# zerohd4869/MM-DFN

Hardware: AMD Instinct MI355X
Metric: utterances/sec (fwd+bwd), IEMOCAP-shaped batch (higher is better)
Workload: dtype f32; 1 GPU; cfg2 (BASELINE configs[1]): B=16 dialogues/GPU, L=110, dims 100/100/512, 2 GCN layers, P=2, dropout 0.50; utterances_per_gpu=1760, parallelism=dp1

## Files before the change

### include/mmdfn_hip.h

```cpp
#ifndef MMDFN_HIP_H
#define MMDFN_HIP_H

#include <stdint.h>

#ifdef __cplusplus
extern "C" {
#endif

int64_t mmdfn_riders_bytes(void);

int mmdfn_abi_version(void);

int mmdfn_propagate(const float* tiles, const float* cross, const float* H, float* out,
                    const int32_t* dia_len, const int32_t* row_start, const int64_t* tile_base,
                    int B, int M, int N, int d, int ldh, int ldo, int max_len, int transpose,
                    void* stream);

int mmdfn_tile_outer(const float* X, const float* Y, float* dtiles, float* dcross,
                     const int32_t* dia_len, const int32_t* row_start, const int64_t* tile_base,
                     int B, int M, int N, int d, int ldx, int ldy, int max_len, int accumulate,
                     void* stream);

int mmdfn_adj_build(const float* feats, float* unit, float* norm, float* cosg, float* cdot,
                    float* rdeg, float* tiles, float* cross,
                    const int32_t* dia_len, const int32_t* row_start, const int64_t* tile_base,
                    int B, int M, int N, int D, int max_len, float modal_weight, void* stream);

int mmdfn_adj_build_bwd(const float* dtiles, const float* dcross,
                        const float* unit, const float* norm, const float* cosg, const float* cdot,
                        const float* rdeg, const float* tiles, const float* cross,
                        float* wsym, float* etile, float* ecross, float* ddeg, float* dunit,
                        float* dfeats, const float* addend,
                        const int32_t* dia_len, const int32_t* row_start, const int64_t* tile_base,
                        int B, int M, int N, int D, int max_len, float modal_weight, void* stream);

int mmdfn_gru_seq_fwd(int ngroups, const float* const* gi, const float* const* w_hh,
                      const float* const* b_hh, float* const* y, float* const* gates,
                      const int* rows, const int* T, int H, void* riders, void* stream);

int mmdfn_gru_seq_bwd(int ngroups, const float* const* dy, const float* const* y,
                      const float* const* gates, const float* const* w_hh,
                      float* const* dgi, float* const* dgh,
                      const int* rows, const int* T, int H, void* riders, void* stream);

int mmdfn_gru_seq_fwd_seg(int ngroups, const float* const* gi, const float* const* w_hh,
                          const float* const* b_hh, float* const* y, float* const* gates,
                          const int* rows, const int* T, int H, const int32_t* const* rank, const int* P,
                          const int* BP, const int* tdir, const float* const* ytab, void* stream);
int mmdfn_gru_seq_bwd_seg(int ngroups, const float* const* dy, const float* const* y,
                          const float* const* gates, const float* const* w_hh,
                          float* const* dgi, float* const* dgh, const int* rows, const int* T, int H,
                          const int32_t* const* rank, const int* P, const int* BP, const int* tdir,
                          float* const* dhinit, int32_t* const* kout, void* stream);
int mmdfn_gru_tab_reduce(const float* dy, const int32_t* kout, const float* dhinit, float* dyt, int rows, int T,
                         int H, int dir, void* stream);

int mmdfn_lstm_pointwise_fwd(const float* G, const float* c_prev, float* h_out, float* c_out,
                             int64_t R, int H, void* stream);
int mmdfn_lstm_pointwise_bwd(const float* G, const float* c_prev, const float* c_new,
                             const float* dh, const float* dc_next, float* dG, float* dc_prev,
                             int64_t R, int H, void* stream);

int mmdfn_gcnii_combine_fwd(const float* P, const float* S2, const float* q, const float* mask,
                            float* out, float theta, float alpha, int64_t R, int d, void* stream);
int mmdfn_gcnii_combine_bwd(const float* P, const float* S2, const float* mask, const float* dout,
                            float* dP, float* dS2, float theta, float alpha, int64_t R, int d,
                            void* stream);

int mmdfn_party_gather(int Mn, const float* const* X, const float* qmask, const float* bias, float* S,
                       int32_t* rank, int L, int B, int P, int H, void* stream);
int mmdfn_party_gather_bwd(int Mn, const float* dS, const int32_t* rank, float* const* dX,
                           const float* const* addend, int L, int B, int P, int H, void* stream);
int mmdfn_party_gather_bwd_colsum(int Mn, const float* dS, const int32_t* rank, float* const* dX,
                                  const float* const* addend, int L, int B, int P, int H, float* workspace, void* stream);

int mmdfn_keep_flags(float* out, int64_t n, float keep, void* state, void* stream);
int mmdfn_keep_flags_stage(float* out, int64_t n, float keep, void* state, void* riders, void* stream);
int mmdfn_keep_flags_flush(void* riders, void* stream);
int mmdfn_gru_seq_fwd_takes_flags(int ngroups, const int* rows);
int64_t mmdfn_colsum_workspace(int H);
int mmdfn_colsum(const float* A, int64_t R, int H, int lda, float* out, float* workspace, void* stream);
int mmdfn_colsum_partial(const float* A, int64_t R, int H, int lda, float* workspace, void* stream);
int mmdfn_party_combine(int Mn, const float* const* base, const float* E, const int32_t* rank,
                        const int64_t* flat_idx, float* out, const float* weights,
                        int L, int B, int P, int N, int H, void* stream);
int mmdfn_party_combine_bwd(int Mn, const float* dout, const int32_t* rank, const int64_t* flat_idx,
                            float* const* dbase, float* dE, const float* weights,
                            int L, int B, int P, int N, int H, void* stream);
int mmdfn_party_combine_bwd_dst(int Mn, const float* dout, const int32_t* rank, const int64_t* inv, float* const* dbase,
                                float* dE, const float* weights, int L, int B, int P, int N, int H, void* stream);


int mmdfn_mask_scale(int ngroups, const float* const* x, const float* const* mask, float* const* out,
                     const int64_t* n, float scale, void* stream);

int mmdfn_linear(const float* X, const float* W, const float* bias, float* Y, int R, int K, int N,
                 int ldx, int ldy, int act, int accumulate, void* stream);
int mmdfn_linear2(const float* X, const float* W, const float* W2, int N1, const float* bias, const float* bias2,
                  float* Y, int R, int K, int N, int ldx, int ldy, int act, int accumulate, void* stream);

int64_t mmdfn_weight_planes_workspace(int N, int K);
int mmdfn_cut_weight_planes(int n, const float* const* w1, const float* const* w2, const int* n1, const int* ld,
                            const int* N, const int* K, const int* mode, void* const* planes, void* stream);
int mmdfn_linear_planes(const float* X, const void* planes, const float* bias, const float* bias2, int n1, float* Y, int R,
                        int K, int N, int ldx, int ldy, int act, int accumulate, void* stream);
int mmdfn_linear_planes_group(int n, const float* const* X, const void* const* planes, const float* const* bias,
                              const float* const* bias2, const int* n1, float* const* Y, const int* R, const int* K,
                              const int* N, const int* ldx, const int* ldy, int act, int accumulate,
                              const float* const* mask, float mask_scale, void* stream);
int mmdfn_linear_planes_group_in(int n, const float* const* X, const void* const* planes, const float* const* bias,
                                 const float* const* bias2, const int* n1, float* const* Y, const int* R, const int* K,
                                 const int* N, const int* ldx, const int* ldy, int act, int accumulate,
                                 const float* const* mask, float mask_scale, const float* const* xmask,
                                 float* const* xdrop, float xscale, void* stream);
int mmdfn_linear_planes_group_party(int n, const float* const* X, const void* const* planes, const float* const* bias,
                                    const float* const* bias2, const int* n1, float* const* Y, const int* R, const int* K,
                                    const int* N, const int* ldx, const int* ldy, int act, int accumulate,
                                    const float* const* mask, float mask_scale, const float* const* xmask,
                                    float* const* xdrop, float xscale, const int* party, const float* qmask, float* S,
                                    int32_t* rank, int L, int B, int P, int Mn, void* stream);

int mmdfn_linear_group_supported(int R, int K, int N);
int mmdfn_linear_group(int n, const float* const* X, const float* const* W, const float* const* W2, const int* N1,
                       const float* const* bias, const float* const* bias2, float* const* Y, const int* R,
                       const int* K, const int* N, const int* ldx, const int* ldw, const int* ldy,
                       const int* kmajor, const int* accumulate, int act, void* stream);
int mmdfn_linear_group_addend(int n, const float* const* X, const float* const* W, const float* const* W2, const int* N1,
                              const float* const* bias, const float* const* bias2, float* const* Y, const float* const* Z,
                              const int* ldz, const int* R, const int* K, const int* N, const int* ldx, const int* ldw,
                              const int* ldy, const int* kmajor, const int* accumulate, int act, void* stream);
int mmdfn_linear_group_seg2(int n, const float* const* X, const float* const* W, const float* const* W2, const int* N1,
                            const float* const* bias, const float* const* bias2, float* const* Y, const float* const* Z,
                            const int* ldz, const int* R, const int* K, const int* N, const int* ldx, const int* ldw,
                            const int* ldy, const int* kmajor, const int* accumulate, const float* const* X2,
                            const float* const* Wk2, const int* K2, const int* ldx2, const int* ldw2, int act, void* stream);

int mmdfn_softmax_scale_fwd(const float* z, const float* c, float* att, float* out, int R, int W, void* stream);
int mmdfn_softmax_scale_bwd(const float* att, const float* c, const float* dout, float* dz, float* dc, int R, int W,
                            void* stream);
int mmdfn_mfn_mem_fwd(const float* u, const float* v1, const float* v2, const float* mem, float* out, float* saved,
                      int64_t n, void* stream);
int mmdfn_mfn_mem_bwd(const float* saved, const float* mem, const float* dout, float* du, float* dv1, float* dv2,
                      float* dmem, int64_t n, void* stream);
int mmdfn_gated_pair_fwd(const float* xm, const float* xn, const float* w, const float* b, const float* pm,
                         const float* pn, float* out, float* zs, int R, int D, int C, void* stream);
int mmdfn_gated_pair_bwd(const float* xm, const float* xn, const float* w, const float* pm, const float* pn,
                         const float* zs, const float* dout, float* dxm, float* dxn, float* dpm, float* dpn,
                         float* dpre, int R, int D, int C, void* stream);
int mmdfn_rowscale_colsum(const float* s, const float* xm, const float* xn, float* out, int R, int D, void* stream);

int mmdfn_gemm_tn_splits(int R, int M, int N);
int mmdfn_gemm_tn(const float* A, const float* B, float* C, float* colsum, float* workspace,
                  int R, int M, int N, int lda, int ldb, int ldc, int splits, void* stream);

int64_t mmdfn_gemm_tn_grouped_workspace(int n, const int* R, const int* M, const int* N);
int mmdfn_gemm_tn_grouped(int n, const float* const* A, const float* const* B, float* const* C, float* const* colsum,
                          const int* R, const int* M, const int* N, const int* lda, const int* ldb, const int* ldc,
                          const int* bshift, float* workspace, void* stream);

int mmdfn_gcn_input_fwd(const float* x, const float* mx, const float* W0, const float* b0, const float* m0, float* xd,
                        float* h0, float* cur0, int R, int F, int H, int ldxd, float mscale, void* stream);
int mmdfn_gcn_input_bwd(const float* dcur0, const float* m0, const float* dh0, const float* h0, const float* W0,
                        const float* dxd, const float* mx, float* dpre, float* dx, int R, int F, int H, int lddxd,
                        float mscale, void* stream);
int mmdfn_lstm_gate_fwd(const float* q, const float* h, const float* c, const float* Wih, const float* Whh,
                        const float* bsum, const float* bsum2, float* gates, float* h_out, float* c_out, int R, int H,
                        void* stream);
int mmdfn_lstm_gate_fwd_ld(const float* q, const float* h, const float* c, const float* Wih, const float* Whh,
                           const float* bsum, const float* bsum2, float* gates, float* h_out, float* c_out, int R, int H,
                           int ldh, void* stream);
int64_t mmdfn_lstm_gate_planes_workspace(int H);
int mmdfn_lstm_gate_cut_weights(const float* Wih, const float* Whh, float* planes, int H, void* stream);
int mmdfn_lstm_gate_takes_planes(int R, int H);
int mmdfn_lstm_gate_fwd_pre(const float* q, const float* h, const float* c, const float* Wih, const float* Whh,
                            const float* bsum, const float* bsum2, float* gates, float* h_out, float* c_out, int R, int H,
                            int ldh, const float* planes, void* stream);
int mmdfn_lstm_gate_bwd(const float* gates, const float* c_prev, const float* c_new, const float* dh_a, const float* dh_b,
                        const float* dc_next, const float* Wih, const float* Whh, const float* dres, float* dG,
                        float* dc_prev, float* dq, float* dh_prev, int R, int H, int has_h, int lddres, void* stream);
int mmdfn_gcnii_layer_fwd(const float* hi, const float* h0, const float* W, const float* q, const float* m, float* out,
                          float* gmask, float theta, float alpha, int R, int H, int ldo, float mscale, void* stream);

int mmdfn_prop_layer_fwd(const float* tiles, const float* cross, const float* zin, int ldz, const int32_t* dia_len,
                         const int32_t* row_start, const int64_t* tile_base, int B, int M, int N, int max_len,
                         const float* h0, const float* W, const float* q, const float* m, float* hi, float* out,
                         float* gmask, float theta, float alpha, int H, int ldo, float mscale, void* stream);
int mmdfn_gcnii_layer_bwd(const float* dout, const float* gmask, const float* W, float* dP, float* dhi, float* dh0,
                          float theta, float alpha, int R, int H, int lddo, int acc_h0, void* stream);
int mmdfn_gcnii_layer_bwd_ld(const float* dout, const float* gmask, const float* W, float* dP, float* dhi, float* dh0,
                             float theta, float alpha, int R, int H, int lddo, int acc_h0, int lddhi, void* stream);

int64_t mmdfn_gemm_tn_batch_workspace(int nseg, const int* R, const int* out, int nout, const int* M, const int* N);
int mmdfn_gemm_tn_batch(int nseg, const float* const* A, const float* const* B, const int* R, const int* lda,
                        const int* ldb, const int* bshift, const int* out, int nout, float* const* C,
                        float* const* colsum, float* const* colsum2, const int* M, const int* N, const int* ldc,
                        const int* accumulate, float* workspace, void* riders, void* stream);
int mmdfn_gemm_tn_batch_ext(int nseg, const float* const* A, const float* const* B, const int* R, const int* lda,
                            const int* ldb, const int* bshift, const int* out, int nout, float* const* C,
                            float* const* colsum, float* const* colsum2, const int* M, const int* N, const int* ldc,
                            const int* accumulate, float* workspace, int next, const float* const* ext_part,
                            const float* const* ext_colpart, float* const* ext_C, float* const* ext_colsum, const int* ext_M,
                            const int* ext_N, const int* ext_ldc, const int* ext_splits, const int* ext_accumulate,
                            void* riders, void* stream);

int mmdfn_wgrad_riders_stage(int nseg, const float* const* A, const float* const* B, const int* R, const int* lda,
                             const int* ldb, const int* bshift, const int* out, int nout, float* const* C,
                             float* const* colsum, float* const* colsum2, const int* M, const int* N, const int* ldc,
                             const int* accumulate, float* workspace, void* riders, void* stream);
int mmdfn_wgrad_riders_staged(void* riders);
int mmdfn_gru_seq_bwd_idle_cus(int ngroups, const int* rows);
int mmdfn_gru_seq_bwd_step_ns(int ngroups, const int* rows);
int mmdfn_wgrad_riders_flush(void* riders, void* stream);
int mmdfn_wgrad_riders_drain(void* riders, void* stream, int discard);

int mmdfn_adam_step(float* p, const float* g, float* m, float* v, int64_t n, float lr, float beta1,
                    float beta2, float eps, float weight_decay, int step, void* stream);

int mmdfn_head_fwd(const float* F, const float* mask, const float* W, const float* bias, float* logp, int64_t N, int Wd,
                   int C, int ldf, int split, float mscale, void* stream);
int64_t mmdfn_head_bwd_workspace(int Wd, int C);
int mmdfn_head_bwd(const float* dlogp, const float* logp, const float* F, const float* mask, const float* W, float* dF,
                   float* dW, float* db, float* workspace, int64_t N, int Wd, int C, int ldf, int lddf, int split,
                   float mscale, void* stream);
int mmdfn_head_bwd_groups(void);
int mmdfn_head_bwd_partial(const float* dlogp, const float* logp, const float* F, const float* mask, const float* W, float* dF,
                           float* workspace, int64_t N, int Wd, int C, int ldf, int lddf, int split, float mscale,
                           void* stream);
int mmdfn_head_fwd_act(const float* F, const float* mask, const float* W, const float* bias, float* logp, int64_t N, int Wd,
                       int C, int ldf, int split, float mscale, int relu, void* stream);
int mmdfn_head_bwd_act(const float* dlogp, const float* logp, const float* F, const float* mask, const float* W, float* dF,
                       float* dW, float* db, float* workspace, int64_t N, int Wd, int C, int ldf, int lddf, int split,
                       float mscale, int relu, void* stream);
int mmdfn_head_bwd_partial_act(const float* dlogp, const float* logp, const float* F, const float* mask, const float* W,
                               float* dF, float* workspace, int64_t N, int Wd, int C, int ldf, int lddf, int split, float mscale,
                               int relu, void* stream);

int mmdfn_lmf_bwd_width(int O, int R);
int mmdfn_lmf_fwd(float* P, const float* factor_a, const float* factor_v, const float* factor_t, int64_t rank_stride_a,
                  int64_t rank_stride_v, int64_t rank_stride_t, const float* w, const float* bias, float* out, int64_t N, int O,
                  int R, int ldp, int ldo, void* stream);
int mmdfn_lmf_bwd(const float* g, const float* P, const float* w, float* D, int64_t N, int O, int R, int ldg, int ldp, int ldd,
                  void* stream);

int64_t mmdfn_tfn_workspace(int64_t N, int Ha, int Hv, int Ht, int O, int which);
int mmdfn_tfn_fwd(const float* ha, const float* hv, const float* ht, int ldha, int ldhv, int ldht, const float* W1, int64_t ldw,
                  const float* b1, void* state, void* used, int64_t counters, float keep, float scale, float* out,
                  float* workspace, int64_t N, int Ha, int Hv, int Ht, int O, int relu, void* stream);
int mmdfn_tfn_bwd_input(const float* dy, const float* y1, int relu, const float* W1, int64_t ldw, const float* ha,
                        const float* hv, const float* ht, int ldha, int ldhv, int ldht, void* used, float keep, float scale,
                        float* dpre, float* dha, float* dhv, float* dht, float* workspace, int64_t N, int Ha, int Hv, int Ht,
                        int O, void* stream);
int mmdfn_tfn_bwd_weight(const float* dpre, const float* ha, const float* hv, const float* ht, int ldha, int ldhv, int ldht,
                         void* used, float keep, float scale, float* dW1, int64_t N, int Ha, int Hv, int Ht, int O,
                         void* stream);
int mmdfn_tfn_keep_flags(void* used, float keep, float* out, int64_t N, int64_t K, int64_t row0, int64_t rows, void* stream);

int mmdfn_focal_loss_fwd(const float* logp, const int64_t* target, const float* alpha, float* loss, float* coef,
                         int64_t N, int C, float gamma, int size_average, void* stream);
int mmdfn_focal_loss_fwd_grad(const float* logp, const int64_t* target, const float* alpha, float* loss, float* coef,
                              float* dlogp_unit, int64_t N, int C, float gamma, int size_average, void* stream);
int mmdfn_focal_loss_bwd(const float* coef, const int64_t* target, const float* dloss, float* dlogp, int64_t N, int C,
                         void* stream);
int mmdfn_focal_loss_fwd_ignore(const float* logp, const int64_t* target, const float* alpha, float* loss, float* coef,
                                float* scale_out, int64_t N, int C, float gamma, int size_average, int64_t ignore_index,
                                void* stream);
int mmdfn_focal_loss_bwd_ignore(const float* coef, const int64_t* target, const float* dloss, const float* scale,
                                float* dlogp, int64_t N, int C, int64_t ignore_index, void* stream);

#ifdef __cplusplus
}
#endif
#endif
```

### mm_dfn_amd/_hip.py

```python
import ctypes
import os

import torch

from . import build as _build

_P = ctypes.c_void_p
_I = ctypes.c_int
_F = ctypes.c_float
_L = ctypes.c_int64

SIGNATURES = {
    "mmdfn_abi_version": [],
    "mmdfn_propagate": [_P, _P, _P, _P, _P, _P, _P, _I, _I, _I, _I, _I, _I, _I, _I, _P],
    "mmdfn_tile_outer": [_P, _P, _P, _P, _P, _P, _P, _I, _I, _I, _I, _I, _I, _I, _I, _P],
    "mmdfn_adj_build": [_P] * 8 + [_P, _P, _P] + [_I] * 5 + [_F, _P],
    "mmdfn_adj_build_bwd": [_P] * 16 + [_P, _P, _P] + [_I] * 5 + [_F, _P],
    "mmdfn_riders_bytes": [],
    "mmdfn_gru_seq_fwd": [_I, _P, _P, _P, _P, _P, _P, _P, _I, _P, _P],
    "mmdfn_gru_seq_bwd": [_I, _P, _P, _P, _P, _P, _P, _P, _P, _I, _P, _P],
    "mmdfn_gru_seq_fwd_seg": [_I, _P, _P, _P, _P, _P, _P, _P, _I, _P, _P, _P, _P, _P, _P],
    "mmdfn_gru_seq_bwd_seg": [_I, _P, _P, _P, _P, _P, _P, _P, _P, _I, _P, _P, _P, _P, _P, _P, _P],
    "mmdfn_gru_tab_reduce": [_P, _P, _P, _P, _I, _I, _I, _I, _P],
    "mmdfn_lstm_pointwise_fwd": [_P, _P, _P, _P, _L, _I, _P],
    "mmdfn_lstm_pointwise_bwd": [_P, _P, _P, _P, _P, _P, _P, _L, _I, _P],
    "mmdfn_gcnii_combine_fwd": [_P, _P, _P, _P, _P, _F, _F, _L, _I, _P],
    "mmdfn_gcnii_combine_bwd": [_P, _P, _P, _P, _P, _P, _F, _F, _L, _I, _P],
    "mmdfn_gcn_input_fwd": [_P] * 8 + [_I] * 4 + [_F, _P],
    "mmdfn_gcn_input_bwd": [_P] * 9 + [_I] * 4 + [_F, _P],
    "mmdfn_lstm_gate_fwd": [_P] * 10 + [_I] * 2 + [_P],
    "mmdfn_lstm_gate_fwd_ld": [_P] * 10 + [_I] * 3 + [_P],
    "mmdfn_lstm_gate_fwd_pre": [_P] * 10 + [_I] * 3 + [_P, _P],
    "mmdfn_lstm_gate_planes_workspace": [_I],
    "mmdfn_lstm_gate_cut_weights": [_P, _P, _P, _I, _P],
    "mmdfn_lstm_gate_takes_planes": [_I, _I],
    "mmdfn_lstm_gate_bwd": [_P] * 13 + [_I] * 4 + [_P],
    "mmdfn_gcnii_layer_fwd": [_P] * 7 + [_F, _F, _I, _I, _I, _F, _P],
    "mmdfn_prop_layer_fwd": [_P, _P, _P, _I, _P, _P, _P, _I, _I, _I, _I, _P, _P, _P, _P, _P, _P, _P, _F, _F, _I, _I, _F, _P],
    "mmdfn_gcnii_layer_bwd": [_P] * 6 + [_F, _F, _I, _I, _I, _I, _P],
    "mmdfn_gcnii_layer_bwd_ld": [_P] * 6 + [_F, _F, _I, _I, _I, _I, _I, _P],
    "mmdfn_linear": [_P, _P, _P, _P, _I, _I, _I, _I, _I, _I, _I, _P],
    "mmdfn_linear2": [_P, _P, _P, _I, _P, _P, _P, _I, _I, _I, _I, _I, _I, _I, _P],
    "mmdfn_weight_planes_workspace": [_I, _I],
    "mmdfn_cut_weight_planes": [_I, _P, _P, _P, _P, _P, _P, _P, _P, _P],
    "mmdfn_linear_planes": [_P, _P, _P, _P, _I, _P, _I, _I, _I, _I, _I, _I, _I, _P],
    "mmdfn_linear_planes_group": [_I, _P, _P, _P, _P, _P, _P, _P, _P, _P, _P, _P, _I, _I, _P, _F, _P],
    "mmdfn_linear_planes_group_in": [_I, _P, _P, _P, _P, _P, _P, _P, _P, _P, _P, _P, _I, _I, _P, _F, _P, _P, _F, _P],
    "mmdfn_linear_planes_group_party": [_I, _P, _P, _P, _P, _P, _P, _P, _P, _P, _P, _P, _I, _I, _P, _F, _P, _P, _F,
                                        _P, _P, _P, _P, _I, _I, _I, _I, _P],
    "mmdfn_linear_group_supported": [_I, _I, _I],
    "mmdfn_linear_group": [_I] + [_P] * 15 + [_I, _P],
    "mmdfn_linear_group_addend": [_I] + [_P] * 17 + [_I, _P],
    "mmdfn_linear_group_seg2": [_I] + [_P] * 22 + [_I, _P],
    "mmdfn_softmax_scale_fwd": [_P, _P, _P, _P, _I, _I, _P],
    "mmdfn_softmax_scale_bwd": [_P, _P, _P, _P, _P, _I, _I, _P],
    "mmdfn_mfn_mem_fwd": [_P] * 6 + [_L, _P],
    "mmdfn_mfn_mem_bwd": [_P] * 7 + [_L, _P],
    "mmdfn_gated_pair_fwd": [_P] * 8 + [_I, _I, _I, _P],
    "mmdfn_gated_pair_bwd": [_P] * 12 + [_I, _I, _I, _P],
    "mmdfn_rowscale_colsum": [_P, _P, _P, _P, _I, _I, _P],
    "mmdfn_gemm_tn_splits": [_I, _I, _I],
    "mmdfn_gemm_tn": [_P, _P, _P, _P, _P, _I, _I, _I, _I, _I, _I, _I, _P],
    "mmdfn_gemm_tn_grouped_workspace": [_I, _P, _P, _P],
    "mmdfn_gemm_tn_grouped": [_I, _P, _P, _P, _P, _P, _P, _P, _P, _P, _P, _P, _P, _P],
    "mmdfn_gemm_tn_batch_workspace": [_I, _P, _P, _I, _P, _P],
    "mmdfn_gemm_tn_batch": [_I, _P, _P, _P, _P, _P, _P, _P, _I, _P, _P, _P, _P, _P, _P, _P, _P, _P, _P],
    "mmdfn_wgrad_riders_stage": [_I, _P, _P, _P, _P, _P, _P, _P, _I, _P, _P, _P, _P, _P, _P, _P, _P, _P, _P],
    "mmdfn_wgrad_riders_staged": [_P],
    "mmdfn_wgrad_riders_flush": [_P, _P],
    "mmdfn_wgrad_riders_drain": [_P, _P, _I],
    "mmdfn_gru_seq_bwd_idle_cus": [_I, _P],
    "mmdfn_gru_seq_bwd_step_ns": [_I, _P],
    "mmdfn_gemm_tn_batch_ext": [_I, _P, _P, _P, _P, _P, _P, _P, _I, _P, _P, _P, _P, _P, _P, _P, _P,
                                _I, _P, _P, _P, _P, _P, _P, _P, _P, _P, _P, _P],
    "mmdfn_head_bwd_groups": [],
    "mmdfn_head_bwd_partial": [_P, _P, _P, _P, _P, _P, _P, _L, _I, _I, _I, _I, _I, _F, _P],
    "mmdfn_colsum_partial": [_P, _L, _I, _I, _P, _P],
    "mmdfn_head_fwd": [_P, _P, _P, _P, _P, _L, _I, _I, _I, _I, _F, _P],
    "mmdfn_head_bwd_workspace": [_I, _I],
    "mmdfn_head_bwd": [_P] * 9 + [_L, _I, _I, _I, _I, _I, _F, _P],
    "mmdfn_head_fwd_act": [_P, _P, _P, _P, _P, _L, _I, _I, _I, _I, _F, _I, _P],
    "mmdfn_head_bwd_act": [_P] * 9 + [_L, _I, _I, _I, _I, _I, _F, _I, _P],
    "mmdfn_head_bwd_partial_act": [_P, _P, _P, _P, _P, _P, _P, _L, _I, _I, _I, _I, _I, _F, _I, _P],
    "mmdfn_lmf_bwd_width": [_I, _I],
    "mmdfn_lmf_fwd": [_P, _P, _P, _P, _L, _L, _L, _P, _P, _P, _L, _I, _I, _I, _I, _P],
    "mmdfn_lmf_bwd": [_P, _P, _P, _P, _L, _I, _I, _I, _I, _I, _P],
    "mmdfn_tfn_workspace": [_L, _I, _I, _I, _I, _I],
    "mmdfn_tfn_fwd": [_P, _P, _P, _I, _I, _I, _P, _L, _P, _P, _P, _L, _F, _F, _P, _P, _L, _I, _I, _I, _I, _I, _P],
    "mmdfn_tfn_bwd_input": [_P, _P, _I, _P, _L, _P, _P, _P, _I, _I, _I, _P, _F, _F, _P, _P, _P, _P, _P, _L, _I, _I, _I, _I, _P],
    "mmdfn_tfn_bwd_weight": [_P, _P, _P, _P, _I, _I, _I, _P, _F, _F, _P, _L, _I, _I, _I, _I, _P],
    "mmdfn_tfn_keep_flags": [_P, _F, _P, _L, _L, _L, _L, _P],
    "mmdfn_focal_loss_fwd": [_P, _P, _P, _P, _P, _L, _I, _F, _I, _P],
    "mmdfn_focal_loss_bwd": [_P, _P, _P, _P, _L, _I, _P],
    "mmdfn_focal_loss_fwd_grad": [_P, _P, _P, _P, _P, _P, _L, _I, _F, _I, _P],
    "mmdfn_focal_loss_fwd_ignore": [_P, _P, _P, _P, _P, _P, _L, _I, _F, _I, _L, _P],
    "mmdfn_focal_loss_bwd_ignore": [_P, _P, _P, _P, _P, _L, _I, _L, _P],
    "mmdfn_adam_step": [_P, _P, _P, _P, _L, _F, _F, _F, _F, _F, _I, _P],
    "mmdfn_party_gather": [_I, _P, _P, _P, _P, _P, _I, _I, _I, _I, _P],
    "mmdfn_party_gather_bwd": [_I, _P, _P, _P, _P, _I, _I, _I, _I, _P],
    "mmdfn_party_gather_bwd_colsum": [_I, _P, _P, _P, _P, _I, _I, _I, _I, _P, _P],
    "mmdfn_party_combine": [_I, _P, _P, _P, _P, _P, _P, _I, _I, _I, _I, _I, _P],
    "mmdfn_party_combine_bwd": [_I, _P, _P, _P, _P, _P, _P, _I, _I, _I, _I, _I, _P],
    "mmdfn_party_combine_bwd_dst": [_I, _P, _P, _P, _P, _P, _P, _I, _I, _I, _I, _I, _P],
    "mmdfn_mask_scale": [_I, _P, _P, _P, _P, _F, _P],
    "mmdfn_keep_flags": [_P, _L, _F, _P, _P],
    "mmdfn_keep_flags_stage": [_P, _L, _F, _P, _P, _P],
    "mmdfn_keep_flags_flush": [_P, _P],
    "mmdfn_gru_seq_fwd_takes_flags": [_I, _P],
    "mmdfn_colsum_workspace": [_I],
    "mmdfn_colsum": [_P, _L, _I, _I, _P, _P, _P],
}

ABI_VERSION = 21


class HipLibraryError(RuntimeError):
    pass


_libs = {}
_tuning = os.environ.get("MMDFN_TUNING_LIB", "0") == "1"


def set_tuning(flag):
    global _tuning
    prev, _tuning = _tuning, bool(flag)
    return prev


def lib():
    handle = _libs.get(_tuning)
    if handle is not None:
        return handle
    tuning = _tuning
    path = _build.TUNING_LIBPATH if tuning else _build.LIBPATH
    if _build.is_stale(tuning):
        try:
            _build.build(verbose=False, tuning=tuning)
        except Exception as e:
            raise HipLibraryError(
                "%s is missing or stale (source digest mismatch) and could not be rebuilt (%s): run `python -m "
                "mm_dfn_amd.build` (needs hipcc); the MI355X path has no CPU fallback" % (path, e)) from e
    handle = ctypes.CDLL(path)
    for name, argtypes in SIGNATURES.items():
        try:
            fn = getattr(handle, name)
        except AttributeError as e:
            raise HipLibraryError("%s lacks symbol %s (stale build?)" % (os.path.basename(path), name)) from e
        fn.argtypes = argtypes
        fn.restype = ctypes.c_int64 if name.endswith(("_workspace", "_bytes")) else ctypes.c_int
    if handle.mmdfn_abi_version() != ABI_VERSION:
        raise HipLibraryError("%s ABI version mismatch" % os.path.basename(path))
    _libs[tuning] = handle
    return handle


def riders_context():
    return ctypes.create_string_buffer(int(lib().mmdfn_riders_bytes()))


def ptr(t):
    if t is None:
        return None
    return ctypes.c_void_p(t.data_ptr())


def stream():
    return ctypes.c_void_p(torch.cuda.current_stream().cuda_stream)


def check(rc, what):
    if rc != 0:
        raise HipLibraryError("%s failed with code %d" % (what, rc))


def require_cuda(*tensors):
    for t in tensors:
        if t is not None and not t.is_cuda:
            raise HipLibraryError("the MM-DFN HIP path needs tensors on an MI355X device (got %s); "
                                  "there is no CPU fallback" % t.device)


def ptr_array(tensors):
    return (ctypes.c_void_p * len(tensors))(*[None if t is None else t.data_ptr() for t in tensors])


def int_array(values):
    return (ctypes.c_int * len(values))(*[int(v) for v in values])


def long_array(values):
    return (ctypes.c_int64 * len(values))(*[int(v) for v in values])


def float_array(values):
    return (ctypes.c_float * len(values))(*[float(v) for v in values])


def require_f32(*tensors):
    for t in tensors:
        if t is not None and t.dtype != torch.float32:
            raise HipLibraryError("the MM-DFN HIP kernels are fp32 (got %s)" % t.dtype)
```

### mm_dfn_amd/csrc/gcn_small.hip

```cpp
#include "mmdfn_internal.h"
#include "../../include/mmdfn_hip.h"
#include <stdlib.h>

namespace {

constexpr int GS_SR = 32;
constexpr int GS_NW = 8;
constexpr int GS_MAXL = 128;
constexpr int GS_SA = 132;

#ifdef MMDFN_TUNING
#define GS_STOP(K) do { if (stop == (K)) return; } while (0)
#else
#define GS_STOP(K) do { } while (0)
#endif

__global__ __launch_bounds__(64 * GS_NW) void prop_layer_strip_fwd_kernel(
    const float* __restrict__ tiles, const float* __restrict__ cross, const float* __restrict__ zin, int ldz,
    const int32_t* __restrict__ dia_len, const int32_t* __restrict__ row_start, const int64_t* __restrict__ tile_base,
    int B, int M, int N, int NS, const float* __restrict__ h0, const float* __restrict__ W, const float* __restrict__ q,
    const float* __restrict__ mk, float* __restrict__ hi_out, float* __restrict__ out, float* __restrict__ gmask,
    float theta, float alpha, int H, int ldo, float ms, int S2, int stop) {
    extern __shared__ __attribute__((aligned(16))) float smem[];
    const int bid = blockIdx.x;
    const int yq = bid >> 3;
    const int per = M * NS;
    const int i = (yq / per) * 8 + (bid & 7);
    if (i >= B) return;
    const int rem = yq % per;
    const int m = rem / NS;
    const int st = rem - m * NS;
    const int L = dia_len[i];
    const int r0 = st * GS_SR;
    if (r0 >= L) return;
    GS_STOP(9);
    const int ld = (L + 3) & ~3;
    const int Lp = (L + 15) & ~15;
    const int nt = Lp >> 4;
    const int rs = row_start[i];
    const int64_t toff = tile_base[i] + (int64_t)m * L * ld;
    const int K2 = 2 * H;
    const int nkc2 = (K2 + 15) >> 4;
    const int nct = (H + 15) >> 4;

    float* As = smem;
    float* A2 = As + GS_SR * GS_SA;
    float* cw = A2 + GS_SR * S2;

    const int tid = threadIdx.x;
    const int lane = tid & 63;
    const int w = __builtin_amdgcn_readfirstlane(tid >> 6);
    const int fi = lane & 15, g = lane >> 4;
    const bool tile = w < nct;
    const int col = 16 * w + fi;
    const unsigned colc = col < H ? col : H - 1;

    int o0 = -1, o1 = -1;
    for (int n = 0; n < M; ++n)
        if (n != m) { if (o0 < 0) o0 = n; else o1 = n; }

    const int c4 = lane & 31, sub = lane >> 5;
    float4 ar[2];
#pragma unroll
    for (int it = 0; it < 2; ++it) {
        const int p = r0 + 16 * it + 2 * w + sub;
        const int qc = 4 * c4 < ld ? 4 * c4 : ld - 4;
        ar[it] = *reinterpret_cast<const float4*>(tiles + toff + (unsigned)((p < L ? p : L - 1) * ld + qc));
    }
    const int H4 = H >> 2;
    float4 hr[2];
#pragma unroll
    for (int s2 = 0; s2 < 2; ++s2) {
        const int e = tid + 64 * GS_NW * s2;
        const int r = e / H4, k = (e - r * H4) * 4;
        const int p = r0 + r;
        hr[s2] = make_float4(0.f, 0.f, 0.f, 0.f);
        if (r < GS_SR && p < L) hr[s2] = *reinterpret_cast<const float4*>(h0 + ((int64_t)m * N + rs + p) * H + k);
    }
    float cwv = 0.f;
    if (tid < 2 * GS_SR) {
        const int n = tid >> 5, pl = tid & 31;
        const int o = n == 0 ? o0 : o1;
        const int p = r0 + pl;
        if (o >= 0 && p < L) {
            const int pk = (m < o) ? mmdfn_pair_index(m, o, M) : mmdfn_pair_index(o, m, M);
            cwv = cross[(int64_t)pk * N + rs + p];
        }
    }
    float zo0[2][4], zo1[2][4], qv[2][4], mv[2][4];
    const bool whole = r0 + GS_SR <= L;
    const int64_t row0 = (int64_t)m * N + rs + r0;
    const unsigned lane_z = (unsigned)(4 * g) * (unsigned)ldz + colc, lane_h = (unsigned)(4 * g) * (unsigned)H + colc;
#pragma unroll
    for (int a = 0; a < 2; ++a)
#pragma unroll
        for (int r = 0; r < 4; ++r) {
            zo0[a][r] = zo1[a][r] = qv[a][r] = 0.f;
            mv[a][r] = 1.0f;
        }
    if (tile) {
        const float* z0 = zin + ((int64_t)(o0 >= 0 ? o0 : m) * N + rs + r0) * ldz;
        const float* z1 = zin + ((int64_t)(o1 >= 0 ? o1 : m) * N + rs + r0) * ldz;
        const float* qb = (q ? q : h0) + row0 * H;
        const float* mb = (mk ? mk : h0) + row0 * H;
        if (whole) {
#pragma unroll
            for (int a = 0; a < 2; ++a)
#pragma unroll
                for (int r = 0; r < 4; ++r) {
                    const int rr = 16 * a + r;
                    zo0[a][r] = (z0 + (size_t)rr * ldz)[lane_z];
                    zo1[a][r] = (z1 + (size_t)rr * ldz)[lane_z];
                    qv[a][r] = (qb + (size_t)rr * H)[lane_h];
                    mv[a][r] = (mb + (size_t)rr * H)[lane_h];
                }
        } else {
#pragma unroll
            for (int a = 0; a < 2; ++a)
#pragma unroll
                for (int r = 0; r < 4; ++r) {
                    const int pl = 16 * a + 4 * g + r;
                    const unsigned pc = r0 + pl < L ? pl : L - 1 - r0;
                    zo0[a][r] = z0[pc * (unsigned)ldz + colc];
                    zo1[a][r] = z1[pc * (unsigned)ldz + colc];
                    qv[a][r] = qb[pc * (unsigned)H + colc];
                    mv[a][r] = mb[pc * (unsigned)H + colc];
                }
        }
#pragma unroll
        for (int a = 0; a < 2; ++a)
#pragma unroll
            for (int r = 0; r < 4; ++r) {
                if (!q) qv[a][r] = 0.f;
                mv[a][r] = mk ? mv[a][r] * ms : 1.0f;
            }
    }

    float zfr[32], wfr[64];
#pragma unroll
    for (int kk = 0; kk < 32; ++kk) zfr[kk] = 0.f;
#pragma unroll
    for (int kk = 0; kk < 64; ++kk) wfr[kk] = 0.f;
    if (tile) {
        const float* zm = zin + ((int64_t)m * N + rs) * ldz;
        const int zfull = L >> 4;
#pragma unroll
        for (int kc = 0; kc < 8; ++kc) {
            if (kc < zfull) {
#pragma unroll
                for (int j = 0; j < 4; ++j) zfr[4 * kc + j] = (zm + (size_t)(16 * kc + j) * ldz)[lane_z];
            } else if (kc < nt) {
#pragma unroll
                for (int j = 0; j < 4; ++j) {
                    const int qq = 16 * kc + 4 * g + j;
                    zfr[4 * kc + j] = zm[(unsigned)(qq < L ? qq : L - 1) * (unsigned)ldz + colc];
                }
            }
        }
        const int wfull = K2 >> 4;
#pragma unroll
        for (int kc = 0; kc < 16; ++kc) {
            if (kc < wfull) {
#pragma unroll
                for (int j = 0; j < 4; ++j) wfr[4 * kc + j] = (W + (size_t)(16 * kc + j) * H)[lane_h];
            } else if (kc < nkc2) {
#pragma unroll
                for (int j = 0; j < 4; ++j) {
                    const int k = 16 * kc + 4 * g + j;
                    wfr[4 * kc + j] = W[(unsigned)(k < K2 ? k : K2 - 1) * (unsigned)H + colc];
                }
            }
        }
    }
#pragma unroll
    for (int it = 0; it < 2; ++it) {
        const int pl = 16 * it + 2 * w + sub;
        const int p = r0 + pl;
        const int qq = 4 * c4;
        float4 v = ar[it];
        const bool rowin = p < L;
        v.x = (rowin && qq + 0 < L) ? v.x : 0.f;
        v.y = (rowin && qq + 1 < L) ? v.y : 0.f;
        v.z = (rowin && qq + 2 < L) ? v.z : 0.f;
        v.w = (rowin && qq + 3 < L) ? v.w : 0.f;
        *reinterpret_cast<float4*>(As + pl * GS_SA + qq) = v;
    }
#pragma unroll
    for (int s2 = 0; s2 < 2; ++s2) {
        const int e = tid + 64 * GS_NW * s2;
        const int r = e / H4, k = (e - r * H4) * 4;
        if (r < GS_SR) *reinterpret_cast<float4*>(A2 + r * S2 + H + k) = hr[s2];
    }
    for (int e = tid; e < GS_SR * (S2 - K2); e += 64 * GS_NW) {
        const int r = e / (S2 - K2), k = K2 + (e - r * (S2 - K2));
        A2[r * S2 + k] = 0.f;
    }
    if (tid < 2 * GS_SR) cw[tid] = cwv;
    __syncthreads();
    GS_STOP(1);

    float hv[2][4];
    if (tile) {
#pragma unroll
        for (int a = 0; a < 2; ++a) {
            const float* ea = As + (16 * a + fi) * GS_SA + 4 * g;
            float4 av[8];
#pragma unroll
            for (int kc = 0; kc < 8; ++kc) av[kc] = *reinterpret_cast<const float4*>(ea + 16 * kc);
            f32x4 acc = (f32x4){0.f, 0.f, 0.f, 0.f};
#pragma unroll
            for (int kc = 0; kc < 8; ++kc) {
                if (kc >= nt) continue;
                acc = __builtin_amdgcn_mfma_f32_16x16x4f32(av[kc].x, zfr[4 * kc + 0], acc, 0, 0, 0);
                acc = __builtin_amdgcn_mfma_f32_16x16x4f32(av[kc].y, zfr[4 * kc + 1], acc, 0, 0, 0);
                acc = __builtin_amdgcn_mfma_f32_16x16x4f32(av[kc].z, zfr[4 * kc + 2], acc, 0, 0, 0);
                acc = __builtin_amdgcn_mfma_f32_16x16x4f32(av[kc].w, zfr[4 * kc + 3], acc, 0, 0, 0);
            }
            float* hb = hi_out + (row0 + 16 * a) * H;
#pragma unroll
            for (int r = 0; r < 4; ++r) {
                const int pl = 16 * a + 4 * g + r;
                float v = acc[r];
                if (o0 >= 0) v += cw[pl] * zo0[a][r];
                if (o1 >= 0) v += cw[GS_SR + pl] * zo1[a][r];
                hv[a][r] = v;
                if (col < H) {
                    A2[pl * S2 + col] = v;
                    if (r0 + pl < L) (hb + (size_t)r * H)[lane_h] = v;
                }
            }
        }
    }
    __syncthreads();
    GS_STOP(2);

    if (tile) {
        f32x4 acc0 = (f32x4){0.f, 0.f, 0.f, 0.f}, acc1 = acc0;
        const float* e0 = A2 + fi * S2 + 4 * g;
        const float* e1 = A2 + (16 + fi) * S2 + 4 * g;
#pragma unroll
        for (int kc = 0; kc < 16; ++kc) {
            if (kc >= nkc2) continue;
            const float4 a0 = *reinterpret_cast<const float4*>(e0 + 16 * kc);
            const float4 a1 = *reinterpret_cast<const float4*>(e1 + 16 * kc);
            acc0 = __builtin_amdgcn_mfma_f32_16x16x4f32(a0.x, wfr[4 * kc + 0], acc0, 0, 0, 0);
            acc1 = __builtin_amdgcn_mfma_f32_16x16x4f32(a1.x, wfr[4 * kc + 0], acc1, 0, 0, 0);
            acc0 = __builtin_amdgcn_mfma_f32_16x16x4f32(a0.y, wfr[4 * kc + 1], acc0, 0, 0, 0);
            acc1 = __builtin_amdgcn_mfma_f32_16x16x4f32(a1.y, wfr[4 * kc + 1], acc1, 0, 0, 0);
            acc0 = __builtin_amdgcn_mfma_f32_16x16x4f32(a0.z, wfr[4 * kc + 2], acc0, 0, 0, 0);
            acc1 = __builtin_amdgcn_mfma_f32_16x16x4f32(a1.z, wfr[4 * kc + 2], acc1, 0, 0, 0);
            acc0 = __builtin_amdgcn_mfma_f32_16x16x4f32(a0.w, wfr[4 * kc + 3], acc0, 0, 0, 0);
            acc1 = __builtin_amdgcn_mfma_f32_16x16x4f32(a1.w, wfr[4 * kc + 3], acc1, 0, 0, 0);
        }
        if (col < H) {
            const unsigned lane_o = (unsigned)(4 * g) * (unsigned)ldo + col;
#pragma unroll
            for (int a = 0; a < 2; ++a)
#pragma unroll
                for (int r = 0; r < 4; ++r) {
                    const int pl = 16 * a + 4 * g + r;
                    if (r0 + pl >= L) continue;
                    const float pv = a == 0 ? acc0[r] : acc1[r];
                    const float v0 = A2[pl * S2 + H + col];
                    const float pre = theta * pv + (1.0f - theta) * ((1.0f - alpha) * hv[a][r] + alpha * v0);
                    (out + (row0 + 16 * a + r) * ldo)[lane_o] = fmaxf(pre, 0.f) * mv[a][r] + qv[a][r];
                    (gmask + (row0 + 16 * a + r) * H)[lane_h] = pre > 0.f ? mv[a][r] : 0.f;
                }
        }
    }
}

}

extern "C" int mmdfn_prop_layer_fwd(const float* tiles, const float* cross, const float* zin, int ldz, const int32_t* dia_len,
                                    const int32_t* row_start, const int64_t* tile_base, int B, int M, int N, int max_len,
                                    const float* h0, const float* W, const float* q, const float* m, float* hi, float* out,
                                    float* gmask, float theta, float alpha, int H, int ldo, float mscale, void* stream) {
    if (B <= 0 || M <= 0 || N <= 0 || H <= 0 || max_len <= 0 || !tiles || !zin || !h0 || !W || !hi || !out || !gmask) return -1;
    if (M > 3 || max_len > GS_MAXL || H > 100 || (H & 3) || ldz < H || ldo < H) return -2;
    if (M > 1 && !cross) return -1;
    int stop = 0;
#ifdef MMDFN_TUNING
    if (const char* e = getenv("MMDFN_PROP_LAYER")) if (atoi(e) == 0) return -2;
    if (const char* e = getenv("MMDFN_PROP_LAYER_STOP")) stop = atoi(e);
#endif
    const int NS = (max_len + GS_SR - 1) / GS_SR;
    const int64_t grid = (int64_t)((B + 7) / 8) * 8 * M * NS;
    if (grid > 4096) return -2;
    const int S2 = ((2 * H + 15) & ~15) + 4;
    const size_t lds = ((size_t)GS_SR * GS_SA + (size_t)GS_SR * S2 + 2 * GS_SR) * sizeof(float);
    hipLaunchKernelGGL(prop_layer_strip_fwd_kernel, dim3((unsigned)grid), dim3(64 * GS_NW), lds, (hipStream_t)stream, tiles, cross,
                       zin, ldz, dia_len, row_start, tile_base, B, M, N, NS, h0, W, q, m, hi, out, gmask, theta, alpha, H, ldo,
                       mscale, S2, stop);
    MMDFN_CHECK_LAUNCH();
    return 0;
}
```

### mm_dfn_amd/csrc/gcn_stack.hip

```cpp
#include "mmdfn_internal.h"
#include "../../include/mmdfn_hip.h"
#include <stdlib.h>

namespace {

constexpr int RB = 16;

__device__ __forceinline__ float4 ld4(const float* p) { return *reinterpret_cast<const float4*>(p); }
__device__ __forceinline__ void st4(float* p, float4 v) { *reinterpret_cast<float4*>(p) = v; }
__device__ __forceinline__ float4 zero4() { return make_float4(0.f, 0.f, 0.f, 0.f); }
__device__ __forceinline__ float4 one4() { return make_float4(1.f, 1.f, 1.f, 1.f); }
__device__ __forceinline__ float4 mul4(float4 a, float4 b) { return make_float4(a.x * b.x, a.y * b.y, a.z * b.z, a.w * b.w); }
__device__ __forceinline__ float4 scl4(float4 a, float s) { return make_float4(a.x * s, a.y * s, a.z * s, a.w * s); }
__device__ __forceinline__ float4 add4(float4 a, float4 b) { return make_float4(a.x + b.x, a.y + b.y, a.z + b.z, a.w + b.w); }
__device__ __forceinline__ float4 fma4(float4 a, float s, float4 b) { return make_float4(a.x * s + b.x, a.y * s + b.y, a.z * s + b.z, a.w * s + b.w); }
__device__ __forceinline__ float sigm(float x) { return __builtin_amdgcn_rcpf(1.0f + __expf(-x)); }
__device__ __forceinline__ float tanhf_(float x) { return 1.0f - 2.0f * __builtin_amdgcn_rcpf(1.0f + __expf(2.0f * x)); }

typedef float f32x2_t __attribute__((ext_vector_type(2)));
__device__ __forceinline__ void st4_nt(float* p, float4 v) { __builtin_nontemporal_store((f32x4){v.x, v.y, v.z, v.w}, reinterpret_cast<f32x4*>(p)); }
__device__ __forceinline__ void nt_store2(float* p, float2 v) { __builtin_nontemporal_store((f32x2_t){v.x, v.y}, reinterpret_cast<f32x2_t*>(p)); }
__device__ __forceinline__ int frag_row(int i) { return i < 4 ? 2 * i : (i < 12 ? 2 * (i - 4) + 1 : 2 * (i - 12) + 8); }
__device__ __forceinline__ int frag_unit(int g) { return ((g & 1) << 1) | (g >> 1); }

__host__ __device__ inline int lds_stride(int K) {
    int ld = ((K + 15) & ~15) + 4;
    if (((ld >> 2) & 1) == 0) ld += 4;
    return ld;
}

__device__ __forceinline__ int qdiv(int i, float inv) { return (int)(((float)i + 0.5f) * inv); }

__device__ __forceinline__ void zero_pads(float* base, int nrows, int ld, int K) {
    const int np4 = (ld - K) >> 2;
    const float rnp4 = 1.0f / (float)(np4 > 0 ? np4 : 1);
    for (int i = threadIdx.x; i < nrows * np4; i += 256) {
        const int r = qdiv(i, rnp4), j = i - r * np4;
        st4(base + r * ld + K + 4 * j, zero4());
    }
}

constexpr int NWS = 26;
template <bool KMAJOR>
struct WeightStager {
    float4 v[NWS];
    __device__ __forceinline__ void issue(const float* __restrict__ W, int ldsrc, int n0, int ncols, int K) {
        const int inner = KMAJOR ? (ncols >> 2) : (K >> 2);
        const int total = KMAJOR ? K * inner : ncols * inner;
        const int qa = 256 / inner, qb = 256 - qa * inner;
        int r = threadIdx.x / inner, j = threadIdx.x - r * inner;
#pragma unroll
        for (int e = 0; e < NWS; ++e) {
            const int i = threadIdx.x + 256 * e;
            const float* src = KMAJOR ? W + (int64_t)r * ldsrc + n0 + 4 * j : W + (int64_t)(n0 + r) * ldsrc + 4 * j;
            v[e] = (i < total) ? ld4(src) : zero4();
            r += qa;
            j += qb;
            if (j >= inner) { j -= inner; ++r; }
        }
    }
    __device__ __forceinline__ void commit(float* sW, int ldw, int ncols, int K) const {
        const int inner = KMAJOR ? (ncols >> 2) : (K >> 2);
        const int total = KMAJOR ? K * inner : ncols * inner;
        const int qa = 256 / inner, qb = 256 - qa * inner;
        int r = threadIdx.x / inner, j = threadIdx.x - r * inner;
#pragma unroll
        for (int e = 0; e < NWS; ++e) {
            const int i = threadIdx.x + 256 * e;
            if (i < total) {
                if (KMAJOR) {
                    float* d = sW + (4 * j) * ldw + r;
                    d[0] = v[e].x; d[ldw] = v[e].y; d[2 * ldw] = v[e].z; d[3 * ldw] = v[e].w;
                } else {
                    st4(sW + r * ldw + 4 * j, v[e]);
                }
            }
            r += qa;
            j += qb;
            if (j >= inner) { j -= inner; ++r; }
        }
        zero_pads(sW, ncols, ldw, K);
    }
};

template <int NT>
__device__ __forceinline__ void contract(f32x4 (&acc)[NT], const int (&wrow0)[NT], const float* sA, int lda, const float* sW,
                                         int ldw, int K) {
    const int lane = threadIdx.x & 63, fi = lane & 15, g = lane >> 4;
    const float* ap = sA + frag_row(fi) * lda + 4 * frag_unit(g);
    const float* bp[NT];
#pragma unroll
    for (int t = 0; t < NT; ++t) bp[t] = sW + (wrow0[t] + frag_row(fi)) * ldw + 4 * frag_unit(g);
    const int nk = (K + 15) >> 4;
    float4 a0, a1, b0[NT], b1[NT];
#define CT_LOAD(A_, B_, KC)                                                          \
    do {                                                                             \
        A_ = ld4(ap + 16 * (KC));                                                    \
        _Pragma("unroll") for (int t = 0; t < NT; ++t) B_[t] = ld4(bp[t] + 16 * (KC)); \
    } while (0)
#define CT_MMA(A_, B_)                                                                                         \
    do {                                                                                                       \
        const float av_[4] = {A_.x, A_.y, A_.z, A_.w};                                                         \
        _Pragma("unroll") for (int j = 0; j < 4; ++j)                                                          \
            _Pragma("unroll") for (int t = 0; t < NT; ++t) {                                                   \
                const float bv_ = (j == 0) ? B_[t].x : (j == 1) ? B_[t].y : (j == 2) ? B_[t].z : B_[t].w;     \
                acc[t] = __builtin_amdgcn_mfma_f32_16x16x4f32(av_[j], bv_, acc[t], 0, 0, 0);                   \
            }                                                                                                  \
    } while (0)
    CT_LOAD(a0, b0, 0);
    int kc = 0;
    for (; kc + 2 <= nk; kc += 2) {
        CT_LOAD(a1, b1, kc + 1);
        CT_MMA(a0, b0);
        if (kc + 2 < nk) CT_LOAD(a0, b0, kc + 2);
        CT_MMA(a1, b1);
    }
    if (kc < nk) CT_MMA(a0, b0);
#undef CT_LOAD
#undef CT_MMA
}

template <int NT>
__device__ __forceinline__ int wave_tiles(int (&wrow0)[NT], int ntiles) {
    const int w = threadIdx.x >> 6;
    int nt = 0;
#pragma unroll
    for (int t = 0; t < NT; ++t) {
        const int tile = w + 4 * t;
        wrow0[t] = tile < ntiles ? 16 * tile : 0;
        nt += tile < ntiles ? 1 : 0;
    }
    return nt;
}

template <int NT>
__device__ __forceinline__ void spill_tiles(const f32x4 (&acc)[NT], const int (&wrow0)[NT], int nt, float* sP, int ldp) {
    const int lane = threadIdx.x & 63, fi = lane & 15, g = lane >> 4;
#pragma unroll
    for (int t = 0; t < NT; ++t) {
        if (t < nt) {
#pragma unroll
            for (int r = 0; r < 4; ++r) sP[frag_row(4 * g + r) * ldp + wrow0[t] + frag_row(fi)] = acc[t][r];
        }
    }
}

#define FOR_ROW_BLOCKS(rb, nrb) for (int rb = blockIdx.x; rb < (nrb); rb += gridDim.x)

__global__ __launch_bounds__(256) void gcn_input_fwd_kernel(const float* __restrict__ x, const float* __restrict__ mx,
                                                            const float* __restrict__ W0, const float* __restrict__ b0,
                                                            const float* __restrict__ m0, float* __restrict__ xd,
                                                            float* __restrict__ h0, float* __restrict__ cur0, int R,
                                                            int F, int H, int ldxd, float ms) {
    extern __shared__ __attribute__((aligned(16))) float smem[];
    const int ldw = lds_stride(F), ldp = ((H + 15) & ~15) + 4;
    float* sW = smem;
    float* sA = sW + H * ldw;
    float* sP = sA + 2 * RB * ldw;
    WeightStager<false> wst;
    wst.issue(W0, F, 0, H, F);
    const int nrb = (R + RB - 1) / RB;
    const int F4 = F >> 2, H4 = H >> 2;
    const float rF4 = 1.0f / (float)F4, rH4 = 1.0f / (float)H4;
    int wrow0[2];
    const int nt = wave_tiles<2>(wrow0, (H + 15) >> 4);
    constexpr int NS = 4;
    constexpr int NE = 2;
    float4 rx[NS], rm[NS];
    auto issue = [&](int rb) {
#pragma unroll
        for (int s = 0; s < NS; ++s) {
            const int i = threadIdx.x + 256 * s;
            const int r = qdiv(i, rF4), k = (i - r * F4) * 4, row = rb * RB + r;
            const bool ok = i < RB * F4 && row < R;
            rx[s] = ok ? ld4(x + (int64_t)row * F + k) : zero4();
            rm[s] = (ok && mx) ? ld4(mx + (int64_t)row * F + k) : one4();
        }
    };
    auto park = [&](int rb, float* dst) {
#pragma unroll
        for (int s = 0; s < NS; ++s) {
            const int i = threadIdx.x + 256 * s;
            if (i >= RB * F4) continue;
            const int r = qdiv(i, rF4), k = (i - r * F4) * 4, row = rb * RB + r;
            const float4 v = mul4(rx[s], scl4(rm[s], mx ? ms : 1.0f));
            st4(dst + r * ldw + k, v);
            if (row < R) st4_nt(xd + (int64_t)row * ldxd + k, v);
        }
    };
    const int rb0 = blockIdx.x;
    if (rb0 < nrb) issue(rb0);
    wst.commit(sW, ldw, H, F);
    zero_pads(sA, 2 * RB, ldw, F);
    if (rb0 < nrb) park(rb0, sA);
    __syncthreads();
    int buf = 0;
    FOR_ROW_BLOCKS(rb, nrb) {
        const int nxt = rb + gridDim.x;
        if (nxt < nrb) issue(nxt);
        float4 em[NE], eb[NE];
#pragma unroll
        for (int s = 0; s < NE; ++s) {
            const int i = threadIdx.x + 256 * s;
            const int r = qdiv(i, rH4), n = (i - r * H4) * 4, row = rb * RB + r;
            const bool ok = i < RB * H4 && row < R;
            em[s] = (ok && m0) ? ld4(m0 + (int64_t)row * H + n) : one4();
            eb[s] = (ok && b0) ? ld4(b0 + n) : zero4();
        }
        f32x4 acc[2] = {{0.f, 0.f, 0.f, 0.f}, {0.f, 0.f, 0.f, 0.f}};
        contract<2>(acc, wrow0, sA + buf * RB * ldw, ldw, sW, ldw, F);
        spill_tiles<2>(acc, wrow0, nt, sP, ldp);
        __syncthreads();
#pragma unroll
        for (int s = 0; s < NE; ++s) {
            const int i = threadIdx.x + 256 * s;
            const int r = qdiv(i, rH4), n = (i - r * H4) * 4, row = rb * RB + r;
            if (i >= RB * H4 || row >= R) continue;
            float4 v = add4(ld4(sP + r * ldp + n), eb[s]);
            v.x = fmaxf(v.x, 0.f); v.y = fmaxf(v.y, 0.f); v.z = fmaxf(v.z, 0.f); v.w = fmaxf(v.w, 0.f);
            st4(h0 + (int64_t)row * H + n, v);
            st4(cur0 + (int64_t)row * H + n, mul4(v, scl4(em[s], m0 ? ms : 1.0f)));
        }
        if (nxt < nrb) park(nxt, sA + (buf ^ 1) * RB * ldw);
        __syncthreads();
        buf ^= 1;
    }
}

__global__ __launch_bounds__(256) void gcn_input_bwd_kernel(const float* __restrict__ dcur0, const float* __restrict__ m0,
                                                            const float* __restrict__ dh0, const float* __restrict__ h0,
                                                            const float* __restrict__ W0, const float* __restrict__ dxd,
                                                            const float* __restrict__ mx, float* __restrict__ dpre,
                                                            float* __restrict__ dx, int R, int F, int H, int lddxd, float ms) {
    extern __shared__ __attribute__((aligned(16))) float smem[];
    const int ldw = lds_stride(H), ldp = ((F + 15) & ~15) + 4;
    float* sW = smem;
    float* sA = sW + F * ldw;
    float* sP = sA + 2 * RB * ldw;
    WeightStager<true> wst;
    wst.issue(W0, F, 0, F, H);
    const int nrb = (R + RB - 1) / RB;
    const int H4 = H >> 2, F4 = F >> 2;
    const float rF4 = 1.0f / (float)F4, rH4 = 1.0f / (float)H4;
    int wrow0[4];
    const int nt = wave_tiles<4>(wrow0, (F + 15) >> 4);
    constexpr int NS = 2;
    constexpr int NE = 4;
    float4 rd[NS], rmk[NS], rh0[NS], rdh[NS];
    auto issue = [&](int rb) {
#pragma unroll
        for (int s = 0; s < NS; ++s) {
            const int i = threadIdx.x + 256 * s;
            const int r = qdiv(i, rH4), k = (i - r * H4) * 4, row = rb * RB + r;
            const bool ok = i < RB * H4 && row < R;
            const int64_t o = (int64_t)row * H + k;
            rd[s] = (ok && dcur0) ? ld4(dcur0 + o) : zero4();
            rmk[s] = (ok && m0) ? ld4(m0 + o) : one4();
            rdh[s] = (ok && dh0) ? ld4(dh0 + o) : zero4();
            rh0[s] = ok ? ld4(h0 + o) : zero4();
        }
    };
    auto park = [&](int rb, float* dst) {
#pragma unroll
        for (int s = 0; s < NS; ++s) {
            const int i = threadIdx.x + 256 * s;
            if (i >= RB * H4) continue;
            const int r = qdiv(i, rH4), k = (i - r * H4) * 4, row = rb * RB + r;
            float4 v = add4(mul4(rd[s], scl4(rmk[s], m0 ? ms : 1.0f)), rdh[s]);
            v.x = rh0[s].x > 0.f ? v.x : 0.f; v.y = rh0[s].y > 0.f ? v.y : 0.f;
            v.z = rh0[s].z > 0.f ? v.z : 0.f; v.w = rh0[s].w > 0.f ? v.w : 0.f;
            st4(dst + r * ldw + k, v);
            if (row < R) st4_nt(dpre + (int64_t)row * H + k, v);
        }
    };
    if ((int)blockIdx.x < nrb) issue(blockIdx.x);
    wst.commit(sW, ldw, F, H);
    zero_pads(sA, 2 * RB, ldw, H);
    if ((int)blockIdx.x < nrb) park(blockIdx.x, sA);
    __syncthreads();
    int buf = 0;
    FOR_ROW_BLOCKS(rb, nrb) {
        const int nxt = rb + gridDim.x;
        if (nxt < nrb) issue(nxt);
        float4 ed[NE], em[NE];
#pragma unroll
        for (int s = 0; s < NE; ++s) {
            const int i = threadIdx.x + 256 * s;
            const int r = qdiv(i, rF4), n = (i - r * F4) * 4, row = rb * RB + r;
            const bool ok = i < RB * F4 && row < R;
            ed[s] = (ok && dxd) ? ld4(dxd + (int64_t)row * lddxd + n) : zero4();
            em[s] = (ok && mx) ? ld4(mx + (int64_t)row * F + n) : one4();
        }
        f32x4 acc[4];
#pragma unroll
        for (int t = 0; t < 4; ++t) acc[t] = (f32x4){0.f, 0.f, 0.f, 0.f};
        contract<4>(acc, wrow0, sA + buf * RB * ldw, ldw, sW, ldw, H);
        spill_tiles<4>(acc, wrow0, nt, sP, ldp);
        __syncthreads();
#pragma unroll
        for (int s = 0; s < NE; ++s) {
            const int i = threadIdx.x + 256 * s;
            const int r = qdiv(i, rF4), n = (i - r * F4) * 4, row = rb * RB + r;
            if (i >= RB * F4 || row >= R) continue;
            st4(dx + (int64_t)row * F + n, mul4(add4(ld4(sP + r * ldp + n), ed[s]), scl4(em[s], mx ? ms : 1.0f)));
        }
        if (nxt < nrb) park(nxt, sA + (buf ^ 1) * RB * ldw);
        __syncthreads();
        buf ^= 1;
    }
}

__global__ __launch_bounds__(256) void gcnii_layer_fwd_kernel(const float* __restrict__ hi, const float* __restrict__ h0,
                                                              const float* __restrict__ W, const float* __restrict__ q,
                                                              const float* __restrict__ m, float* __restrict__ out,
                                                              float* __restrict__ gmask, float theta, float alpha, int R,
                                                              int H, int ldo, float ms) {
    extern __shared__ __attribute__((aligned(16))) float smem[];
    const int K = 2 * H;
    const int ldw = lds_stride(K), ldp = ((H + 15) & ~15) + 4;
    float* sW = smem;
    float* sA = sW + H * ldw;
    float* sP = sA + 2 * RB * ldw;
    WeightStager<true> wst;
    wst.issue(W, H, 0, H, K);
    const int nrb = (R + RB - 1) / RB;
    const int H4 = H >> 2;
    const float rH4 = 1.0f / (float)H4;
    int wrow0[2];
    const int nt = wave_tiles<2>(wrow0, (H + 15) >> 4);
    constexpr int NS = 2;
    float4 ra[NS], rb_[NS];
    auto issue = [&](int rb) {
#pragma unroll
        for (int s = 0; s < NS; ++s) {
            const int i = threadIdx.x + 256 * s;
            const int r = qdiv(i, rH4), k = (i - r * H4) * 4, row = rb * RB + r;
            const bool ok = i < RB * H4 && row < R;
            ra[s] = ok ? ld4(hi + (int64_t)row * H + k) : zero4();
            rb_[s] = ok ? ld4(h0 + (int64_t)row * H + k) : zero4();
        }
    };
    auto park = [&](float* dst) {
#pragma unroll
        for (int s = 0; s < NS; ++s) {
            const int i = threadIdx.x + 256 * s;
            if (i >= RB * H4) continue;
            const int r = qdiv(i, rH4), k = (i - r * H4) * 4;
            st4(dst + r * ldw + k, ra[s]);
            st4(dst + r * ldw + H + k, rb_[s]);
        }
    };
    if ((int)blockIdx.x < nrb) issue(blockIdx.x);
    wst.commit(sW, ldw, H, K);
    zero_pads(sA, 2 * RB, ldw, K);
    if ((int)blockIdx.x < nrb) park(sA);
    __syncthreads();
    int buf = 0;
    FOR_ROW_BLOCKS(rb, nrb) {
        const int nxt = rb + gridDim.x;
        if (nxt < nrb) issue(nxt);
        const float* A = sA + buf * RB * ldw;
        float4 eq[NS], em[NS];
#pragma unroll
        for (int s = 0; s < NS; ++s) {
            const int i = threadIdx.x + 256 * s;
            const int r = qdiv(i, rH4), n = (i - r * H4) * 4, row = rb * RB + r;
            const bool ok = i < RB * H4 && row < R;
            eq[s] = (ok && q) ? ld4(q + (int64_t)row * H + n) : zero4();
            em[s] = (ok && m) ? ld4(m + (int64_t)row * H + n) : one4();
        }
        f32x4 acc[2] = {{0.f, 0.f, 0.f, 0.f}, {0.f, 0.f, 0.f, 0.f}};
        contract<2>(acc, wrow0, A, ldw, sW, ldw, K);
        spill_tiles<2>(acc, wrow0, nt, sP, ldp);
        __syncthreads();
#pragma unroll
        for (int s = 0; s < NS; ++s) {
            const int i = threadIdx.x + 256 * s;
            const int r = qdiv(i, rH4), n = (i - r * H4) * 4, row = rb * RB + r;
            if (i >= RB * H4 || row >= R) continue;
            const float4 p = ld4(sP + r * ldp + n), vh = ld4(A + r * ldw + n), v0 = ld4(A + r * ldw + H + n);
            const float4 ems = scl4(em[s], m ? ms : 1.0f);
            float4 o, gm;
#define K7F(F_)                                                                                            \
    {                                                                                                      \
        const float pre = theta * p.F_ + (1.0f - theta) * ((1.0f - alpha) * vh.F_ + alpha * v0.F_);       \
        o.F_ = fmaxf(pre, 0.f) * ems.F_ + eq[s].F_;                                                        \
        gm.F_ = pre > 0.f ? ems.F_ : 0.f;                                                                  \
    }
            K7F(x) K7F(y) K7F(z) K7F(w)
#undef K7F
            st4(out + (int64_t)row * ldo + n, o);
            st4_nt(gmask + (int64_t)row * H + n, gm);
        }
        if (nxt < nrb) park(sA + (buf ^ 1) * RB * ldw);
        __syncthreads();
        buf ^= 1;
    }
}

__global__ __launch_bounds__(256) void gcnii_layer_bwd_kernel(const float* __restrict__ dout, const float* __restrict__ gmask,
                                                              const float* __restrict__ W, float* __restrict__ dP,
                                                              float* __restrict__ dhi, float* __restrict__ dh0,
                                                              float theta, float alpha, int R, int H, int lddo, int acc_h0, int lddhi) {
    extern __shared__ __attribute__((aligned(16))) float smem[];
    const int N = 2 * H;
    const int ldw = lds_stride(H), ldp = ((N + 15) & ~15) + 4;
    float* sW = smem;
    float* sA = sW + N * ldw;
    float* sP = sA + 2 * RB * ldw;
    WeightStager<false> wst;
    wst.issue(W, H, 0, N, H);
    const int nrb = (R + RB - 1) / RB;
    const int H4 = H >> 2;
    const float rH4 = 1.0f / (float)H4;
    int wrow0[4];
    const int nt = wave_tiles<4>(wrow0, (N + 15) >> 4);
    constexpr int NS = 2;
    float4 rd[NS], rg[NS];
    auto issue = [&](int rb) {
#pragma unroll
        for (int s = 0; s < NS; ++s) {
            const int i = threadIdx.x + 256 * s;
            const int r = qdiv(i, rH4), k = (i - r * H4) * 4, row = rb * RB + r;
            const bool ok = i < RB * H4 && row < R;
            rd[s] = ok ? ld4(dout + (int64_t)row * lddo + k) : zero4();
            rg[s] = ok ? ld4(gmask + (int64_t)row * H + k) : zero4();
        }
    };
    auto park = [&](int rb, float* dst) {
#pragma unroll
        for (int s = 0; s < NS; ++s) {
            const int i = threadIdx.x + 256 * s;
            if (i >= RB * H4) continue;
            const int r = qdiv(i, rH4), k = (i - r * H4) * 4, row = rb * RB + r;
            const float4 v = scl4(mul4(rd[s], rg[s]), theta);
            st4(dst + r * ldw + k, v);
            if (row < R) st4_nt(dP + (int64_t)row * H + k, v);
        }
    };
    if ((int)blockIdx.x < nrb) issue(blockIdx.x);
    wst.commit(sW, ldw, N, H);
    zero_pads(sA, 2 * RB, ldw, H);
    if ((int)blockIdx.x < nrb) park(blockIdx.x, sA);
    __syncthreads();
    const float c1 = (1.0f - theta) * (1.0f - alpha) / theta, c2 = (1.0f - theta) * alpha / theta;
    int buf = 0;
    FOR_ROW_BLOCKS(rb, nrb) {
        const int nxt = rb + gridDim.x;
        if (nxt < nrb) issue(nxt);
        const float* A = sA + buf * RB * ldw;
        float4 eo[NS];
#pragma unroll
        for (int s = 0; s < NS; ++s) {
            const int i = threadIdx.x + 256 * s;
            const int r = qdiv(i, rH4), n = (i - r * H4) * 4, row = rb * RB + r;
            eo[s] = (acc_h0 && i < RB * H4 && row < R) ? ld4(dh0 + (int64_t)row * H + n) : zero4();
        }
        f32x4 acc[4];
#pragma unroll
        for (int t = 0; t < 4; ++t) acc[t] = (f32x4){0.f, 0.f, 0.f, 0.f};
        contract<4>(acc, wrow0, A, ldw, sW, ldw, H);
        spill_tiles<4>(acc, wrow0, nt, sP, ldp);
        __syncthreads();
#pragma unroll
        for (int s = 0; s < NS; ++s) {
            const int i = threadIdx.x + 256 * s;
            const int r = qdiv(i, rH4), n = (i - r * H4) * 4, row = rb * RB + r;
            if (i >= RB * H4 || row >= R) continue;
            const float4 dp = ld4(A + r * ldw + n);
            st4(dhi + (int64_t)row * lddhi + n, fma4(dp, c1, ld4(sP + r * ldp + n)));
            st4(dh0 + (int64_t)row * H + n, add4(fma4(dp, c2, ld4(sP + r * ldp + H + n)), eo[s]));
        }
        if (nxt < nrb) park(nxt, sA + (buf ^ 1) * RB * ldw);
        __syncthreads();
        buf ^= 1;
    }
}

__global__ __launch_bounds__(512) void gcnii_layer_fwd_ws_kernel(const float* __restrict__ hi, const float* __restrict__ h0,
                                                                 const float* __restrict__ W, const float* __restrict__ q,
                                                                 const float* __restrict__ m, float* __restrict__ out,
                                                                 float* __restrict__ gmask, float theta, float alpha, int R,
                                                                 int H, int ldo, float ms) {
    extern __shared__ __attribute__((aligned(16))) float smem[];
    const int K = 2 * H;
    const int ldw = lds_stride(K), ldp = ((H + 15) & ~15) + 4;
    float* sW = smem;
    float* sA = sW + H * ldw;
    float* sP = sA + 2 * RB * ldw;
    const int nrb = (R + RB - 1) / RB;
    const int H4 = H >> 2;
    const float rH4 = 1.0f / (float)H4;
    const int tid = threadIdx.x & 255;
    const bool producer = threadIdx.x >= 256;
    const int first = blockIdx.x, stride = gridDim.x;
    constexpr int NS = 2;
    float4 ra[NS], rb_[NS], eq[NS], em[NS];
    auto issue = [&](int rb) {
#pragma unroll
        for (int s = 0; s < NS; ++s) {
            const int i = tid + 256 * s;
            const int r = qdiv(i, rH4), k = (i - r * H4) * 4, row = rb * RB + r;
            const bool ok = i < RB * H4 && row < R;
            ra[s] = ok ? ld4(hi + (int64_t)row * H + k) : zero4();
            rb_[s] = ok ? ld4(h0 + (int64_t)row * H + k) : zero4();
        }
    };
    auto park = [&](float* dst) {
#pragma unroll
        for (int s = 0; s < NS; ++s) {
            const int i = tid + 256 * s;
            if (i >= RB * H4) continue;
            const int r = qdiv(i, rH4), k = (i - r * H4) * 4;
            st4(dst + r * ldw + k, ra[s]);
            st4(dst + r * ldw + H + k, rb_[s]);
        }
    };
    auto issue_epi = [&](int rb) {
#pragma unroll
        for (int s = 0; s < NS; ++s) {
            const int i = tid + 256 * s;
            const int r = qdiv(i, rH4), n = (i - r * H4) * 4, row = rb * RB + r;
            const bool ok = i < RB * H4 && row < R;
            eq[s] = (ok && q) ? ld4(q + (int64_t)row * H + n) : zero4();
            em[s] = (ok && m) ? ld4(m + (int64_t)row * H + n) : one4();
        }
    };
    auto epilogue = [&](int rb, const float* A, const float* P) {
#pragma unroll
        for (int s = 0; s < NS; ++s) {
            const int i = tid + 256 * s;
            const int r = qdiv(i, rH4), n = (i - r * H4) * 4, row = rb * RB + r;
            if (i >= RB * H4 || row >= R) continue;
            const float4 p = ld4(P + r * ldp + n), vh = ld4(A + r * ldw + n), v0 = ld4(A + r * ldw + H + n);
            const float4 ems = scl4(em[s], m ? ms : 1.0f);
            float4 o, gm;
#define K7F(F_)                                                                                            \
    {                                                                                                      \
        const float pre = theta * p.F_ + (1.0f - theta) * ((1.0f - alpha) * vh.F_ + alpha * v0.F_);       \
        o.F_ = fmaxf(pre, 0.f) * ems.F_ + eq[s].F_;                                                        \
        gm.F_ = pre > 0.f ? ems.F_ : 0.f;                                                                  \
    }
            K7F(x) K7F(y) K7F(z) K7F(w)
#undef K7F
            st4(out + (int64_t)row * ldo + n, o);
            st4_nt(gmask + (int64_t)row * H + n, gm);
        }
    };
    if (producer) {
        if (first < nrb) { issue(first); issue_epi(first); }
    } else {
        WeightStager<true> wst;
        wst.issue(W, H, 0, H, K);
        wst.commit(sW, ldw, H, K);
        zero_pads(sA, 2 * RB, ldw, K);
    }
    if (producer) {
        if (first < nrb) park(sA);
        if (first + stride < nrb) issue(first + stride);
    }
    __syncthreads();
    int wrow0[2];
    const int nt = wave_tiles<2>(wrow0, (H + 15) >> 4);
    int buf = 0, prev_rb = -1;
    for (int rb = first; rb < nrb; rb += stride) {
        const int nxt = rb + stride;
        if (producer) {
            if (prev_rb >= 0) epilogue(prev_rb, sA + (buf ^ 1) * RB * ldw, sP + (buf ^ 1) * RB * ldp);
            if (prev_rb >= 0) issue_epi(rb);
            if (nxt < nrb) {
                park(sA + (buf ^ 1) * RB * ldw);
                if (nxt + stride < nrb) issue(nxt + stride);
            }
        } else {
            f32x4 acc[2] = {{0.f, 0.f, 0.f, 0.f}, {0.f, 0.f, 0.f, 0.f}};
            contract<2>(acc, wrow0, sA + buf * RB * ldw, ldw, sW, ldw, K);
            spill_tiles<2>(acc, wrow0, nt, sP + buf * RB * ldp, ldp);
        }
        __syncthreads();
        prev_rb = rb;
        buf ^= 1;
    }
    if (producer && prev_rb >= 0) epilogue(prev_rb, sA + (buf ^ 1) * RB * ldw, sP + (buf ^ 1) * RB * ldp);
}

__global__ __launch_bounds__(512) void gcnii_layer_bwd_ws_kernel(const float* __restrict__ dout, const float* __restrict__ gmask,
                                                                 const float* __restrict__ W, float* __restrict__ dP,
                                                                 float* __restrict__ dhi, float* __restrict__ dh0,
                                                                 float theta, float alpha, int R, int H, int lddo, int acc_h0,
                                                                 int lddhi) {
    extern __shared__ __attribute__((aligned(16))) float smem[];
    const int N = 2 * H;
    const int ldw = lds_stride(H), ldp = ((N + 15) & ~15) + 4;
    float* sW = smem;
    float* sA = sW + N * ldw;
    float* sP = sA + 2 * RB * ldw;
    const int nrb = (R + RB - 1) / RB;
    const int H4 = H >> 2;
    const float rH4 = 1.0f / (float)H4;
    const int tid = threadIdx.x & 255;
    const bool producer = threadIdx.x >= 256;
    const int first = blockIdx.x, stride = gridDim.x;
    constexpr int NS = 2;
    float4 rd[NS], rg[NS], eo[NS];
    auto issue = [&](int rb) {
#pragma unroll
        for (int s = 0; s < NS; ++s) {
            const int i = tid + 256 * s;
            const int r = qdiv(i, rH4), k = (i - r * H4) * 4, row = rb * RB + r;
            const bool ok = i < RB * H4 && row < R;
            rd[s] = ok ? ld4(dout + (int64_t)row * lddo + k) : zero4();
            rg[s] = ok ? ld4(gmask + (int64_t)row * H + k) : zero4();
        }
    };
    auto park = [&](int rb, float* dst) {
#pragma unroll
        for (int s = 0; s < NS; ++s) {
            const int i = tid + 256 * s;
            if (i >= RB * H4) continue;
            const int r = qdiv(i, rH4), k = (i - r * H4) * 4, row = rb * RB + r;
            const float4 v = scl4(mul4(rd[s], rg[s]), theta);
            st4(dst + r * ldw + k, v);
            if (row < R) st4_nt(dP + (int64_t)row * H + k, v);
        }
    };
    auto issue_epi = [&](int rb) {
#pragma unroll
        for (int s = 0; s < NS; ++s) {
            const int i = tid + 256 * s;
            const int r = qdiv(i, rH4), n = (i - r * H4) * 4, row = rb * RB + r;
            eo[s] = (acc_h0 && i < RB * H4 && row < R) ? ld4(dh0 + (int64_t)row * H + n) : zero4();
        }
    };
    const float c1 = (1.0f - theta) * (1.0f - alpha) / theta, c2 = (1.0f - theta) * alpha / theta;
    auto epilogue = [&](int rb, const float* A, const float* P) {
#pragma unroll
        for (int s = 0; s < NS; ++s) {
            const int i = tid + 256 * s;
            const int r = qdiv(i, rH4), n = (i - r * H4) * 4, row = rb * RB + r;
            if (i >= RB * H4 || row >= R) continue;
            const float4 dp = ld4(A + r * ldw + n);
            st4(dhi + (int64_t)row * lddhi + n, fma4(dp, c1, ld4(P + r * ldp + n)));
            st4(dh0 + (int64_t)row * H + n, add4(fma4(dp, c2, ld4(P + r * ldp + H + n)), eo[s]));
        }
    };
    if (producer) {
        if (first < nrb) { issue(first); issue_epi(first); }
    } else {
        WeightStager<false> wst;
        wst.issue(W, H, 0, N, H);
        wst.commit(sW, ldw, N, H);
        zero_pads(sA, 2 * RB, ldw, H);
    }
    if (producer) {
        if (first < nrb) park(first, sA);
        if (first + stride < nrb) issue(first + stride);
    }
    __syncthreads();
    int wrow0[4];
    const int nt = wave_tiles<4>(wrow0, (N + 15) >> 4);
    int buf = 0, prev_rb = -1;
    for (int rb = first; rb < nrb; rb += stride) {
        const int nxt = rb + stride;
        if (producer) {
            if (prev_rb >= 0) epilogue(prev_rb, sA + (buf ^ 1) * RB * ldw, sP + (buf ^ 1) * RB * ldp);
            if (prev_rb >= 0) issue_epi(rb);
            if (nxt < nrb) {
                park(nxt, sA + (buf ^ 1) * RB * ldw);
                if (nxt + stride < nrb) issue(nxt + stride);
            }
        } else {
            f32x4 acc[4];
#pragma unroll
            for (int t = 0; t < 4; ++t) acc[t] = (f32x4){0.f, 0.f, 0.f, 0.f};
            contract<4>(acc, wrow0, sA + buf * RB * ldw, ldw, sW, ldw, H);
            spill_tiles<4>(acc, wrow0, nt, sP + buf * RB * ldp, ldp);
        }
        __syncthreads();
        prev_rb = rb;
        buf ^= 1;
    }
    if (producer && prev_rb >= 0) epilogue(prev_rb, sA + (buf ^ 1) * RB * ldw, sP + (buf ^ 1) * RB * ldp);
}

constexpr int UB = 32;

__global__ __launch_bounds__(256) void lstm_gate_fwd_kernel(const float* __restrict__ q, const float* __restrict__ h,
                                                            const float* __restrict__ c, const float* __restrict__ Wih,
                                                            const float* __restrict__ Whh, const float* __restrict__ bsum, const float* __restrict__ bsum2,
                                                            float* __restrict__ gates, float* __restrict__ h_out,
                                                            float* __restrict__ c_out, int R, int H, int ldh) {
    extern __shared__ __attribute__((aligned(16))) float smem[];
    const int K = h ? 2 * H : H;
    const int ldw = lds_stride(K), lde = UB + 4;
    float* sW = smem;
    float* sA = sW + 4 * UB * ldw;
    float* sE = sA + 2 * RB * ldw;
    const int u0 = blockIdx.y * UB;
    const int nu = min(UB, H - u0);
    const int H4 = H >> 2;
    const float rH4 = 1.0f / (float)H4;
    constexpr int NW1 = 13;
    float4 vi[NW1], vh[NW1];
    {
        const int total = 4 * UB * H4;
#pragma unroll
        for (int e = 0; e < NW1; ++e) {
            const int i = threadIdx.x + 256 * e;
            const int rowl = qdiv(i, rH4), k = (i - rowl * H4) * 4;
            const int gate = rowl / UB, ul = rowl - gate * UB;
            const bool ok = i < total && ul < nu;
            const int64_t src = (int64_t)(gate * H + u0 + ul) * H + k;
            vi[e] = ok ? ld4(Wih + src) : zero4();
            vh[e] = (ok && h) ? ld4(Whh + src) : zero4();
        }
    }
    const int nrb = (R + RB - 1) / RB;
    const int w = threadIdx.x >> 6;
    const int wrow0[2] = {w * UB, w * UB + 16};
    constexpr int NS = 2;
    float4 rq[NS], rh[NS];
    auto issue = [&](int rb) {
#pragma unroll
        for (int s = 0; s < NS; ++s) {
            const int i = threadIdx.x + 256 * s;
            const int r = qdiv(i, rH4), k = (i - r * H4) * 4, row = rb * RB + r;
            const bool ok = i < RB * H4 && row < R;
            rq[s] = ok ? ld4(q + (int64_t)row * H + k) : zero4();
            rh[s] = (ok && h) ? ld4(h + (int64_t)row * ldh + k) : zero4();
        }
    };
    auto park = [&](float* dst) {
#pragma unroll
        for (int s = 0; s < NS; ++s) {
            const int i = threadIdx.x + 256 * s;
            if (i >= RB * H4) continue;
            const int r = qdiv(i, rH4), k = (i - r * H4) * 4;
            st4(dst + r * ldw + k, rq[s]);
            if (h) st4(dst + r * ldw + H + k, rh[s]);
        }
    };
    if ((int)blockIdx.x < nrb) issue(blockIdx.x);
    {
        const int total = 4 * UB * H4;
#pragma unroll
        for (int e = 0; e < NW1; ++e) {
            const int i = threadIdx.x + 256 * e;
            if (i >= total) continue;
            const int rowl = qdiv(i, rH4), k = (i - rowl * H4) * 4;
            st4(sW + rowl * ldw + k, vi[e]);
            if (h) st4(sW + rowl * ldw + H + k, vh[e]);
        }
        zero_pads(sW, 4 * UB, ldw, K);
    }
    zero_pads(sA, 2 * RB, ldw, K);
    if ((int)blockIdx.x < nrb) park(sA);
    const int er = threadIdx.x >> 4, eu = (threadIdx.x & 15) * 2;
    const bool ethread = eu < nu;
    float2 bi = make_float2(0.f, 0.f), bf = bi, bg = bi, bo = bi;
    if (ethread) {
        bi = *reinterpret_cast<const float2*>(bsum + u0 + eu); bf = *reinterpret_cast<const float2*>(bsum + H + u0 + eu);
        bg = *reinterpret_cast<const float2*>(bsum + 2 * H + u0 + eu); bo = *reinterpret_cast<const float2*>(bsum + 3 * H + u0 + eu);
        if (bsum2) {
            const float2 ci = *reinterpret_cast<const float2*>(bsum2 + u0 + eu), cf = *reinterpret_cast<const float2*>(bsum2 + H + u0 + eu);
            const float2 cg = *reinterpret_cast<const float2*>(bsum2 + 2 * H + u0 + eu), co = *reinterpret_cast<const float2*>(bsum2 + 3 * H + u0 + eu);
            bi.x += ci.x; bi.y += ci.y; bf.x += cf.x; bf.y += cf.y; bg.x += cg.x; bg.y += cg.y; bo.x += co.x; bo.y += co.y;
        }
    }
    __syncthreads();
    int buf = 0;
    FOR_ROW_BLOCKS(rb, nrb) {
        const int nxt = rb + gridDim.x;
        if (nxt < nrb) issue(nxt);
        const int erow = rb * RB + er;
        const float2 cp = (c && ethread && erow < R) ? *reinterpret_cast<const float2*>(c + (int64_t)erow * H + u0 + eu)
                                                     : make_float2(0.f, 0.f);
        f32x4 acc[2] = {{0.f, 0.f, 0.f, 0.f}, {0.f, 0.f, 0.f, 0.f}};
        contract<2>(acc, wrow0, sA + buf * RB * ldw, ldw, sW, ldw, K);
        {
            const int lane = threadIdx.x & 63, fi = lane & 15, g = lane >> 4;
#pragma unroll
            for (int t = 0; t < 2; ++t)
#pragma unroll
                for (int r = 0; r < 4; ++r) sE[(w * RB + frag_row(4 * g + r)) * lde + 16 * t + frag_row(fi)] = acc[t][r];
        }
        __syncthreads();
        if (ethread && erow < R) {
            const float2 pi = *reinterpret_cast<const float2*>(sE + (0 * RB + er) * lde + eu);
            const float2 pf = *reinterpret_cast<const float2*>(sE + (1 * RB + er) * lde + eu);
            const float2 pg = *reinterpret_cast<const float2*>(sE + (2 * RB + er) * lde + eu);
            const float2 po = *reinterpret_cast<const float2*>(sE + (3 * RB + er) * lde + eu);
            float2 gi, gf, gg, go, cn, hn;
#define K8F(F_)                                                                 \
    {                                                                           \
        gi.F_ = sigm(pi.F_ + bi.F_); gf.F_ = sigm(pf.F_ + bf.F_); gg.F_ = tanhf_(pg.F_ + bg.F_); go.F_ = sigm(po.F_ + bo.F_); \
        cn.F_ = gf.F_ * cp.F_ + gi.F_ * gg.F_;                                  \
        hn.F_ = go.F_ * tanhf_(cn.F_);                                          \
    }
            K8F(x) K8F(y)
#undef K8F
            float* gr = gates + (int64_t)erow * 4 * H + u0 + eu;
            *reinterpret_cast<float2*>(gr) = gi; *reinterpret_cast<float2*>(gr + H) = gf;
            *reinterpret_cast<float2*>(gr + 2 * H) = gg; *reinterpret_cast<float2*>(gr + 3 * H) = go;
            *reinterpret_cast<float2*>(c_out + (int64_t)erow * H + u0 + eu) = cn;
            *reinterpret_cast<float2*>(h_out + (int64_t)erow * ldh + u0 + eu) = hn;
        }
        if (nxt < nrb) park(sA + (buf ^ 1) * RB * ldw);
        __syncthreads();
        buf ^= 1;
    }
}

constexpr int CBW = 64;
constexpr int GATE_BWD_WIDE_NKC = 26;

__global__ __launch_bounds__(256) void lstm_gate_bwd_kernel(const float* __restrict__ gates, const float* __restrict__ c_prev,
                                                            const float* __restrict__ c_new, const float* __restrict__ dh_a,
                                                            const float* __restrict__ dh_b, const float* __restrict__ dc_next,
                                                            const float* __restrict__ Wih, const float* __restrict__ Whh,
                                                            const float* __restrict__ dres, float* __restrict__ dG,
                                                            float* __restrict__ dc_prev, float* __restrict__ dq,
                                                            float* __restrict__ dh_prev, int R, int H, int has_h,
                                                            int lddres) {
    extern __shared__ __attribute__((aligned(16))) float smem[];
    const int K = 4 * H;
    const int ldw = lds_stride(K), ldp = CBW + 4;
    float* sW = smem;
    float* sA = sW + CBW * ldw;
    const int nb = (H + CBW - 1) / CBW;
    const bool is_dh = (int)blockIdx.y >= nb;
    const int n0 = (is_dh ? blockIdx.y - nb : blockIdx.y) * CBW;
    const int ncols = min(CBW, H - n0);
    WeightStager<true> wst;
    wst.issue(is_dh ? Whh : Wih, H, n0, ncols, K);
    const int nrb = (R + RB - 1) / RB;
    const int w = threadIdx.x >> 6;
    const int wrow0[1] = {16 * w < ncols ? 16 * w : 0};
    const int nt = 16 * w < ncols ? 1 : 0;
    const bool writer = blockIdx.y == 0;
    const int H4 = H >> 2;
    const float rH4 = 1.0f / (float)H4;
    constexpr int NS = 2;
    float4 rgi[NS], rgf[NS], rgg[NS], rgo[NS], rcn[NS], rcp[NS], rdh[NS], rdh2[NS], rdc[NS];
    auto issue = [&](int rb) {
#pragma unroll
        for (int s_ = 0; s_ < NS; ++s_) {
            const int i = threadIdx.x + 256 * s_;
            const int r = qdiv(i, rH4), u = (i - r * H4) * 4, row = rb * RB + r;
            const bool ok = i < RB * H4 && row < R;
            const int64_t o = (int64_t)row * H + u;
            const float* gr = gates + (int64_t)row * 4 * H + u;
            rgi[s_] = ok ? ld4(gr) : zero4();
            rgf[s_] = ok ? ld4(gr + H) : zero4();
            rgg[s_] = ok ? ld4(gr + 2 * H) : zero4();
            rgo[s_] = ok ? ld4(gr + 3 * H) : zero4();
            rcn[s_] = ok ? ld4(c_new + o) : zero4();
            rcp[s_] = (ok && c_prev) ? ld4(c_prev + o) : zero4();
            rdh[s_] = (ok && dh_a) ? ld4(dh_a + o) : zero4();
            rdh2[s_] = (ok && dh_b) ? ld4(dh_b + o) : zero4();
            rdc[s_] = (ok && dc_next) ? ld4(dc_next + o) : zero4();
        }
    };
    auto park = [&](int rb, float* dst) {
#pragma unroll
        for (int s_ = 0; s_ < NS; ++s_) {
            const int i = threadIdx.x + 256 * s_;
            if (i >= RB * H4) continue;
            const int r = qdiv(i, rH4), u = (i - r * H4) * 4, row = rb * RB + r;
            float4 di, df, dg, dO, dcp;
#define GB1(F)                                                                      \
    {                                                                               \
        const float gi = rgi[s_].F, gf = rgf[s_].F, gg = rgg[s_].F, go = rgo[s_].F; \
        const float tc = tanhf_(rcn[s_].F);                                         \
        const float dhv = rdh[s_].F + rdh2[s_].F;                                   \
        const float dc = rdc[s_].F + dhv * go * (1.0f - tc * tc);                   \
        dO.F = dhv * tc * go * (1.0f - go);                                         \
        di.F = dc * gg * gi * (1.0f - gi);                                          \
        df.F = dc * rcp[s_].F * gf * (1.0f - gf);                                   \
        dg.F = dc * gi * (1.0f - gg * gg);                                          \
        dcp.F = dc * gf;                                                            \
    }
            GB1(x) GB1(y) GB1(z) GB1(w)
#undef GB1
            float* sp = dst + r * ldw + u;
            st4(sp, di); st4(sp + H, df); st4(sp + 2 * H, dg); st4(sp + 3 * H, dO);
            if (writer && row < R) {
                float* d = dG + (int64_t)row * 4 * H + u;
                st4(d, di); st4(d + H, df); st4(d + 2 * H, dg); st4(d + 3 * H, dO);
                if (has_h) st4(dc_prev + (int64_t)row * H + u, dcp);
            }
        }
    };
    if ((int)blockIdx.x < nrb) issue(blockIdx.x);
    wst.commit(sW, ldw, ncols, K);
    if (ncols < CBW) {
        for (int i = threadIdx.x; i < (CBW - ncols) * (ldw >> 2); i += 256) st4(sW + ncols * ldw + 4 * i, zero4());
    }
    zero_pads(sA, 2 * RB, ldw, K);
    if ((int)blockIdx.x < nrb) park(blockIdx.x, sA);
    __syncthreads();
    const int er = threadIdx.x >> 4, en = (threadIdx.x & 15) * 4;
    int buf = 0;
    FOR_ROW_BLOCKS(rb, nrb) {
        const int nxt = rb + gridDim.x;
        if (nxt < nrb) issue(nxt);
        const int erow = rb * RB + er;
        const bool eok = en < ncols && erow < R;
        const float4 rv = (!is_dh && dres && eok) ? ld4(dres + (int64_t)erow * lddres + n0 + en) : zero4();
        f32x4 acc[1] = {{0.f, 0.f, 0.f, 0.f}};
        float* Acur = sA + buf * RB * ldw;
        contract<1>(acc, wrow0, Acur, ldw, sW, ldw, K);
        __syncthreads();
        spill_tiles<1>(acc, wrow0, nt, Acur, ldp);
        __syncthreads();
        if (eok) {
            const float4 v = add4(ld4(Acur + er * ldp + en), rv);
            st4((is_dh ? dh_prev : dq) + (int64_t)erow * H + n0 + en, v);
        }
        if (nxt < nrb) park(nxt, sA + (buf ^ 1) * RB * ldw);
        __syncthreads();
        buf ^= 1;
    }
}

template <int ABL, bool WIDE = false>
__global__ __launch_bounds__(512) void lstm_gate_bwd_ws_kernel(const float* __restrict__ gates, const float* __restrict__ c_prev,
                                                               const float* __restrict__ c_new, const float* __restrict__ dh_a,
                                                               const float* __restrict__ dh_b, const float* __restrict__ dc_next,
                                                               const float* __restrict__ Wih, const float* __restrict__ Whh,
                                                               const float* __restrict__ dres, float* __restrict__ dG,
                                                               float* __restrict__ dc_prev, float* __restrict__ dq,
                                                               float* __restrict__ dh_prev, int R, int H, int has_h,
                                                               int lddres) {
    extern __shared__ __attribute__((aligned(16))) float smem[];
    const int K = 4 * H;
    const int ldw = lds_stride(K);
    float* sW = smem;
    float* sA = sW + CBW * ldw;
    const int nb = WIDE ? 1 : (H + CBW - 1) / CBW;
    const bool is_dh = (int)blockIdx.y >= nb;
    const int n0 = WIDE ? 0 : (is_dh ? blockIdx.y - nb : blockIdx.y) * CBW;
    const int ncols = min(CBW, H - n0);
    const int nrb = (R + RB - 1) / RB;
    const int tid = threadIdx.x & 255;
    const bool producer = threadIdx.x >= 256;
    const int nyb = gridDim.y, yb = blockIdx.y;
    const bool wr_i = (0 % nyb) == yb, wr_f = (1 % nyb) == yb, wr_g = (2 % nyb) == yb, wr_o = (3 % nyb) == yb, wr_c = yb == nyb - 1;
    const int H4 = H >> 2;
    const float rH4 = 1.0f / (float)H4;
    {
        const float* Wsrc = is_dh ? Whh : Wih;
        const int inner = ncols >> 2;
        const int total = K * inner;
        constexpr int NW2 = 13;
        float4 v[NW2];
#pragma unroll
        for (int e = 0; e < NW2; ++e) {
            const int i0 = threadIdx.x + 512 * e, i = i0 < total ? i0 : total - 1;
            const int r = i / inner, j = i - r * inner;
            v[e] = ld4(Wsrc + (int64_t)r * H + n0 + 4 * j);
        }
#pragma unroll
        for (int e = 0; e < NW2; ++e) {
            const int i = threadIdx.x + 512 * e;
            if (i >= total) continue;
            const int r = i / inner, j = i - r * inner;
            float* d = sW + (4 * j) * ldw + r;
            d[0] = v[e].x; d[ldw] = v[e].y; d[2 * ldw] = v[e].z; d[3 * ldw] = v[e].w;
        }
        const int np4 = (ldw - K) >> 2;
        const float rnp4 = 1.0f / (float)(np4 > 0 ? np4 : 1);
        for (int i = threadIdx.x; i < ncols * np4; i += 512) { const int r = qdiv(i, rnp4), j = i - r * np4; st4(sW + r * ldw + K + 4 * j, zero4()); }
        for (int i = threadIdx.x; i < (CBW - ncols) * (ldw >> 2); i += 512) st4(sW + ncols * ldw + 4 * i, zero4());
        for (int i = threadIdx.x; i < 2 * RB * np4; i += 512) { const int r = qdiv(i, rnp4), j = i - r * np4; st4(sA + r * ldw + K + 4 * j, zero4()); }
    }
    constexpr int NS = 2;
    float4 rgi[NS], rgf[NS], rgg[NS], rgo[NS], rcn[NS], rcp[NS], rdh[NS], rdh2[NS], rdc[NS];
    auto issue = [&](int rb) {
#pragma unroll
        for (int s_ = 0; s_ < NS; ++s_) {
            const int i = tid + 256 * s_;
            const int r = qdiv(i, rH4), u = (i - r * H4) * 4, row = rb * RB + r;
            const bool ok = !(ABL & 2) && i < RB * H4 && row < R;
            const int64_t o = (int64_t)row * H + u;
            const float* gr = gates + (int64_t)row * 4 * H + u;
            rgi[s_] = ok ? ld4(gr) : zero4();
            rgf[s_] = ok ? ld4(gr + H) : zero4();
            rgg[s_] = ok ? ld4(gr + 2 * H) : zero4();
            rgo[s_] = ok ? ld4(gr + 3 * H) : zero4();
            rcn[s_] = ok ? ld4(c_new + o) : zero4();
            rcp[s_] = (ok && c_prev) ? ld4(c_prev + o) : zero4();
            rdh[s_] = (ok && dh_a) ? ld4(dh_a + o) : zero4();
            rdh2[s_] = (ok && dh_b) ? ld4(dh_b + o) : zero4();
            rdc[s_] = (ok && dc_next) ? ld4(dc_next + o) : zero4();
        }
    };
    float4 odi[NS], odf[NS], odg[NS], odo[NS], odc[NS];
    auto park = [&](float* dst) {
#pragma unroll
        for (int s_ = 0; s_ < NS; ++s_) {
            const int i = tid + 256 * s_;
            float4 di, df, dg, dO, dcp;
#define GB1(F)                                                                      \
    {                                                                               \
        const float gi = rgi[s_].F, gf = rgf[s_].F, gg = rgg[s_].F, go = rgo[s_].F; \
        const float tc = tanhf_(rcn[s_].F);                                         \
        const float dhv = rdh[s_].F + rdh2[s_].F;                                   \
        const float dc = rdc[s_].F + dhv * go * (1.0f - tc * tc);                   \
        dO.F = dhv * tc * go * (1.0f - go);                                         \
        di.F = dc * gg * gi * (1.0f - gi);                                          \
        df.F = dc * rcp[s_].F * gf * (1.0f - gf);                                   \
        dg.F = dc * gi * (1.0f - gg * gg);                                          \
        dcp.F = dc * gf;                                                            \
    }
            if (ABL & 4) { di = rgi[s_]; df = rgf[s_]; dg = rgg[s_]; dO = rgo[s_]; dcp = rcn[s_]; }
            else { GB1(x) GB1(y) GB1(z) GB1(w) }
#undef GB1
            odi[s_] = di; odf[s_] = df; odg[s_] = dg; odo[s_] = dO; odc[s_] = dcp;
            if (i >= RB * H4) continue;
            const int r = qdiv(i, rH4), u = (i - r * H4) * 4;
            float* sp = dst + r * ldw + u;
            st4(sp, di); st4(sp + H, df); st4(sp + 2 * H, dg); st4(sp + 3 * H, dO);
        }
    };
    auto flush = [&](int rb) {
        if (ABL & 8) return;
#pragma unroll
        for (int s_ = 0; s_ < NS; ++s_) {
            const int i = tid + 256 * s_;
            if (i >= RB * H4) continue;
            const int r = qdiv(i, rH4), u = (i - r * H4) * 4, row = rb * RB + r;
            if (row >= R) continue;
            float* d = dG + (int64_t)row * 4 * H + u;
            if (wr_i) st4_nt(d, odi[s_]);
            if (wr_f) st4_nt(d + H, odf[s_]);
            if (wr_g) st4_nt(d + 2 * H, odg[s_]);
            if (wr_o) st4_nt(d + 3 * H, odo[s_]);
            if (has_h && wr_c) st4(dc_prev + (int64_t)row * H + u, odc[s_]);
        }
    };
    const int first = blockIdx.x, stride = gridDim.x;
    if (producer) {
        if (first < nrb) { issue(first); park(sA); }
        if (first + stride < nrb) issue(first + stride);
        if (first < nrb) flush(first);
    }
    __syncthreads();
    const int w = tid >> 6, lane = tid & 63, fi = lane & 15, g = lane >> 4;
    const int wrow0[1] = {16 * w < ncols ? 16 * w : 0};
    const int ecol = n0 + 16 * w + frag_row(fi);
    const bool ecol_ok = (16 * w + frag_row(fi)) < ncols;
    float* const outp = is_dh ? dh_prev : dq;
    constexpr int NKC = WIDE ? GATE_BWD_WIDE_NKC : 1;
    const int ecol2 = CBW + 16 * w + frag_row(fi);
    const bool ecol2_ok = WIDE && ecol2 < H;
    const bool tile2 = WIDE && (CBW + 16 * w) < H;
    float4 wreg[NKC];
    if (WIDE && !producer) {
        const float* Wsrc = is_dh ? Whh : Wih;
        const int cc = ecol2_ok ? ecol2 : 0;
#pragma unroll
        for (int kc = 0; kc < NKC; ++kc) {
            const int k0 = 16 * kc + 4 * frag_unit(g);
            float v[4];
#pragma unroll
            for (int j = 0; j < 4; ++j) v[j] = (ecol2_ok && k0 + j < K) ? Wsrc[(int64_t)(k0 + j) * H + cc] : 0.f;
            wreg[kc] = make_float4(v[0], v[1], v[2], v[3]);
        }
    }
    int buf = 0;
    if (producer) {
        for (int rb = first; rb < nrb; rb += stride) {
            const int nxt = rb + stride;
            if (nxt < nrb) {
                park(sA + (buf ^ 1) * RB * ldw);
                if (nxt + stride < nrb) issue(nxt + stride);
                flush(nxt);
            }
            __syncthreads();
            buf ^= 1;
        }
        return;
    }
    for (int rb = first; rb < nrb; rb += stride) {
        {
            float rv[4];
#pragma unroll
            for (int r = 0; r < 4; ++r) {
                const int erow = rb * RB + frag_row(4 * g + r);
                rv[r] = (!is_dh && dres && ecol_ok && erow < R) ? dres[(int64_t)erow * lddres + ecol] : 0.f;
            }
            f32x4 acc[1] = {{0.f, 0.f, 0.f, 0.f}};
            if constexpr (WIDE) {
                float rv2[4];
#pragma unroll
                for (int r = 0; r < 4; ++r) {
                    const int erow = rb * RB + frag_row(4 * g + r);
                    rv2[r] = (!is_dh && dres && ecol2_ok && erow < R) ? dres[(int64_t)erow * lddres + ecol2] : 0.f;
                }
                f32x4 acc2 = {0.f, 0.f, 0.f, 0.f};
                const float* ap = sA + buf * RB * ldw + frag_row(fi) * ldw + 4 * frag_unit(g);
                const float* bp = sW + (wrow0[0] + frag_row(fi)) * ldw + 4 * frag_unit(g);
                const int nk = (K + 15) >> 4;
                float4 a_n = ld4(ap), b_n = ld4(bp);
#pragma unroll
                for (int kc = 0; kc < NKC; ++kc) {
                    if (kc < nk) {
                        const float4 a_c = a_n, b_c = b_n;
                        if (kc + 1 < nk) { a_n = ld4(ap + 16 * (kc + 1)); b_n = ld4(bp + 16 * (kc + 1)); }
                        const float av[4] = {a_c.x, a_c.y, a_c.z, a_c.w}, bv[4] = {b_c.x, b_c.y, b_c.z, b_c.w};
                        const float cv[4] = {wreg[kc].x, wreg[kc].y, wreg[kc].z, wreg[kc].w};
#pragma unroll
                        for (int j = 0; j < 4; ++j) {
                            acc[0] = __builtin_amdgcn_mfma_f32_16x16x4f32(av[j], bv[j], acc[0], 0, 0, 0);
                            if (tile2) acc2 = __builtin_amdgcn_mfma_f32_16x16x4f32(av[j], cv[j], acc2, 0, 0, 0);
                        }
                    }
                }
                if (ecol2_ok && !(ABL & 8)) {
#pragma unroll
                    for (int r = 0; r < 4; ++r) {
                        const int erow = rb * RB + frag_row(4 * g + r);
                        if (erow < R) outp[(int64_t)erow * H + ecol2] = acc2[r] + rv2[r];
                    }
                }
            } else {
                if (!(ABL & 1)) contract<1>(acc, wrow0, sA + buf * RB * ldw, ldw, sW, ldw, K);
                else acc[0][0] = sA[buf * RB * ldw + fi * ldw + g];
            }
            if (ecol_ok && !(ABL & 8)) {
#pragma unroll
                for (int r = 0; r < 4; ++r) {
                    const int erow = rb * RB + frag_row(4 * g + r);
                    if (erow < R) outp[(int64_t)erow * H + ecol] = acc[0][r] + rv[r];
                }
            }
        }
        __syncthreads();
        buf ^= 1;
    }
}

__global__ __launch_bounds__(512) void lstm_gate_fwd_ws_kernel(const float* __restrict__ q, const float* __restrict__ h,
                                                               const float* __restrict__ c, const float* __restrict__ Wih,
                                                               const float* __restrict__ Whh, const float* __restrict__ bsum, const float* __restrict__ bsum2,
                                                               float* __restrict__ gates, float* __restrict__ h_out,
                                                               float* __restrict__ c_out, int R, int H, int ldh) {
    extern __shared__ __attribute__((aligned(16))) float smem[];
    const int K = h ? 2 * H : H;
    const int ldw = lds_stride(K), lde = UB + 4;
    float* sW = smem;
    float* sA = sW + 4 * UB * ldw;
    float* sE = sA + 2 * RB * ldw;
    const int u0 = blockIdx.y * UB;
    const int nu = min(UB, H - u0);
    const int H4 = H >> 2;
    const float rH4 = 1.0f / (float)H4;
    const int tid = threadIdx.x & 255;
    const bool producer = threadIdx.x >= 256;
    {
        const int total = 4 * UB * H4;
        constexpr int NW2 = 7;
        float4 vi[NW2], vh[NW2];
#pragma unroll
        for (int e = 0; e < NW2; ++e) {
            const int i0 = threadIdx.x + 512 * e, i = i0 < total ? i0 : total - 1;
            const int rowl = qdiv(i, rH4), k = (i - rowl * H4) * 4;
            const int gate = rowl / UB, ul = rowl - gate * UB;
            const int64_t src = (int64_t)(gate * H + u0 + (ul < nu ? ul : nu - 1)) * H + k;
            vi[e] = ld4(Wih + src);
            vh[e] = h ? ld4(Whh + src) : zero4();
        }
#pragma unroll
        for (int e = 0; e < NW2; ++e) {
            const int i = threadIdx.x + 512 * e;
            if (i >= total) continue;
            const int rowl = qdiv(i, rH4), k = (i - rowl * H4) * 4;
            const int ul = rowl - (rowl / UB) * UB;
            st4(sW + rowl * ldw + k, ul < nu ? vi[e] : zero4());
            if (h) st4(sW + rowl * ldw + H + k, ul < nu ? vh[e] : zero4());
        }
        const int np4 = (ldw - K) >> 2;
        const float rnp4 = 1.0f / (float)(np4 > 0 ? np4 : 1);
        for (int i = threadIdx.x; i < 4 * UB * np4; i += 512) { const int r = qdiv(i, rnp4), j = i - r * np4; st4(sW + r * ldw + K + 4 * j, zero4()); }
        for (int i = threadIdx.x; i < 2 * RB * np4; i += 512) { const int r = qdiv(i, rnp4), j = i - r * np4; st4(sA + r * ldw + K + 4 * j, zero4()); }
    }
    const int nrb = (R + RB - 1) / RB;
    constexpr int NS = 2;
    float4 rq[NS], rh[NS];
    auto issue = [&](int rb) {
#pragma unroll
        for (int s = 0; s < NS; ++s) {
            const int i = tid + 256 * s;
            const int r = qdiv(i, rH4), k = (i - r * H4) * 4, row = rb * RB + r;
            const bool ok = i < RB * H4 && row < R;
            rq[s] = ok ? ld4(q + (int64_t)row * H + k) : zero4();
            rh[s] = (ok && h) ? ld4(h + (int64_t)row * ldh + k) : zero4();
        }
    };
    auto park = [&](float* dst) {
#pragma unroll
        for (int s = 0; s < NS; ++s) {
            const int i = tid + 256 * s;
            if (i >= RB * H4) continue;
            const int r = qdiv(i, rH4), k = (i - r * H4) * 4;
            st4(dst + r * ldw + k, rq[s]);
            if (h) st4(dst + r * ldw + H + k, rh[s]);
        }
    };
    const int er = tid >> 4, eu = (tid & 15) * 2;
    const bool ethread = eu < nu;
    float2 bi = make_float2(0.f, 0.f), bf = bi, bg = bi, bo = bi;
    if (producer && ethread) {
        bi = *reinterpret_cast<const float2*>(bsum + u0 + eu); bf = *reinterpret_cast<const float2*>(bsum + H + u0 + eu);
        bg = *reinterpret_cast<const float2*>(bsum + 2 * H + u0 + eu); bo = *reinterpret_cast<const float2*>(bsum + 3 * H + u0 + eu);
        if (bsum2) {
            const float2 ci = *reinterpret_cast<const float2*>(bsum2 + u0 + eu), cf = *reinterpret_cast<const float2*>(bsum2 + H + u0 + eu);
            const float2 cg = *reinterpret_cast<const float2*>(bsum2 + 2 * H + u0 + eu), co = *reinterpret_cast<const float2*>(bsum2 + 3 * H + u0 + eu);
            bi.x += ci.x; bi.y += ci.y; bf.x += cf.x; bf.y += cf.y; bg.x += cg.x; bg.y += cg.y; bo.x += co.x; bo.y += co.y;
        }
    }
    auto cell = [&](int rb, const float* E, float2 cp) {
        const int erow = rb * RB + er;
        if (!(ethread && erow < R)) return;
        const float2 pi = *reinterpret_cast<const float2*>(E + (0 * RB + er) * lde + eu);
        const float2 pf = *reinterpret_cast<const float2*>(E + (1 * RB + er) * lde + eu);
        const float2 pg = *reinterpret_cast<const float2*>(E + (2 * RB + er) * lde + eu);
        const float2 po = *reinterpret_cast<const float2*>(E + (3 * RB + er) * lde + eu);
        float2 gi, gf, gg, go, cn, hn;
#define K8F(F_)                                                                 \
    {                                                                           \
        gi.F_ = sigm(pi.F_ + bi.F_); gf.F_ = sigm(pf.F_ + bf.F_); gg.F_ = tanhf_(pg.F_ + bg.F_); go.F_ = sigm(po.F_ + bo.F_); \
        cn.F_ = gf.F_ * cp.F_ + gi.F_ * gg.F_;                                  \
        hn.F_ = go.F_ * tanhf_(cn.F_);                                          \
    }
        K8F(x) K8F(y)
#undef K8F
        float* gr = gates + (int64_t)erow * 4 * H + u0 + eu;
        nt_store2(gr, gi); nt_store2(gr + H, gf); nt_store2(gr + 2 * H, gg); nt_store2(gr + 3 * H, go);
        *reinterpret_cast<float2*>(c_out + (int64_t)erow * H + u0 + eu) = cn;
        *reinterpret_cast<float2*>(h_out + (int64_t)erow * ldh + u0 + eu) = hn;
    };
    auto load_c = [&](int rb) {
        const int erow = rb * RB + er;
        return (c && ethread && erow < R) ? *reinterpret_cast<const float2*>(c + (int64_t)erow * H + u0 + eu) : make_float2(0.f, 0.f);
    };
    const int first = blockIdx.x, stride = gridDim.x;
    float2 cp_prev = make_float2(0.f, 0.f);
    if (producer) {
        if (first < nrb) { issue(first); park(sA); cp_prev = load_c(first); }
        if (first + stride < nrb) issue(first + stride);
    }
    __syncthreads();
    const int w = tid >> 6;
    const int wrow0[2] = {w * UB, w * UB + 16};
    int buf = 0, prev_rb = -1;
    for (int rb = first; rb < nrb; rb += stride) {
        const int nxt = rb + stride;
        if (producer) {
            if (prev_rb >= 0) cell(prev_rb, sE + (buf ^ 1) * 4 * RB * lde, cp_prev);
            cp_prev = load_c(rb);
            if (nxt < nrb) {
                park(sA + (buf ^ 1) * RB * ldw);
                if (nxt + stride < nrb) issue(nxt + stride);
            }
        } else {
            f32x4 acc[2] = {{0.f, 0.f, 0.f, 0.f}, {0.f, 0.f, 0.f, 0.f}};
            contract<2>(acc, wrow0, sA + buf * RB * ldw, ldw, sW, ldw, K);
            const int lane = tid & 63, fi = lane & 15, g = lane >> 4;
            float* E = sE + buf * 4 * RB * lde;
#pragma unroll
            for (int t = 0; t < 2; ++t)
#pragma unroll
                for (int r = 0; r < 4; ++r) E[(w * RB + frag_row(4 * g + r)) * lde + 16 * t + frag_row(fi)] = acc[t][r];
        }
        __syncthreads();
        prev_rb = rb;
        buf ^= 1;
    }
    if (producer && prev_rb >= 0) cell(prev_rb, sE + (buf ^ 1) * 4 * RB * lde, cp_prev);
}

inline bool bad_dims(int64_t R, int H) { return R <= 0 || H < 4 || (H & 3) || H > 100 || R > (int64_t)1 << 30; }

inline bool gate_ws(int R) {
#ifdef MMDFN_TUNING
    if (const char* e = getenv("MMDFN_GATE_WS")) return atoi(e) != 0;
#endif
    return R >= 64;
}

constexpr int LAYER_WS_ROWS = 64;
inline bool layer_ws(int R) {
#ifdef MMDFN_TUNING
    if (const char* e = getenv("MMDFN_LAYER_WS")) return atoi(e) != 0;
#endif
    return R >= LAYER_WS_ROWS;
}

constexpr int GATE_SPLIT_ROWS = 16384;
constexpr int GATE_BWD_WIDE_ROWS = 16384;
inline bool gate_split(int R, int H) {
#ifdef MMDFN_TUNING
    if (const char* e = getenv("MMDFN_GATE_SPLIT")) return atoi(e) != 0;
#endif
    return R >= GATE_SPLIT_ROWS && H >= 32;
}

inline int row_groups(int R, int column_blocks) {
    const int nrb = (R + RB - 1) / RB;
    int gq = (256 + column_blocks - 1) / column_blocks;
    if (gq > nrb) gq = nrb;
    const int per = (nrb + gq - 1) / gq;
    gq = (nrb + per - 1) / per;
    return gq < 1 ? 1 : gq;
}

#define LAUNCH_BIG_LDS(kern, grid, lds, stream, ...)                                  \
    do {                                                                              \
        if ((lds) > 156 * 1024) return -1;                                            \
        if (int e_ = mmdfn_allow_big_lds(kern)) return e_;                            \
        hipLaunchKernelGGL(kern, grid, dim3(256), lds, (hipStream_t)(stream), __VA_ARGS__); \
        MMDFN_CHECK_LAUNCH();                                                         \
    } while (0)

}

extern "C" int mmdfn_gcn_input_fwd(const float* x, const float* mx, const float* W0, const float* b0, const float* m0,
                                   float* xd, float* h0, float* cur0, int R, int F, int H, int ldxd, float mscale,
                                   void* stream) {
    if (bad_dims(R, H) || F < 4 || (F & 3) || F > 256 || ldxd < F || (ldxd & 3)) return -1;
    const size_t lds = ((size_t)(H + 2 * RB) * lds_stride(F) + RB * (((H + 15) & ~15) + 4)) * sizeof(float);
    LAUNCH_BIG_LDS(gcn_input_fwd_kernel, dim3(row_groups(R, 1)), lds, stream, x, mx, W0, b0, m0, xd, h0, cur0, R, F, H, ldxd,
                   mscale);
    return 0;
}

extern "C" int mmdfn_gcn_input_bwd(const float* dcur0, const float* m0, const float* dh0, const float* h0, const float* W0,
                                   const float* dxd, const float* mx, float* dpre, float* dx, int R, int F, int H, int lddxd,
                                   float mscale, void* stream) {
    if (bad_dims(R, H) || F < 4 || (F & 3) || F > 256 || (dxd && (lddxd < F || (lddxd & 3)))) return -1;
    const size_t lds = ((size_t)(F + 2 * RB) * lds_stride(H) + RB * (((F + 15) & ~15) + 4)) * sizeof(float);
    LAUNCH_BIG_LDS(gcn_input_bwd_kernel, dim3(row_groups(R, 1)), lds, stream, dcur0, m0, dh0, h0, W0, dxd, mx, dpre, dx, R, F, H,
                   lddxd, mscale);
    return 0;
}

static int lstm_gate_fwd_impl(const float* q, const float* h, const float* c, const float* Wih, const float* Whh,
                              const float* bsum, const float* bsum2, float* gates, float* h_out, float* c_out, int R, int H,
                              int ldh, const void* planes, void* stream);

extern "C" int mmdfn_lstm_gate_fwd_ld(const float* q, const float* h, const float* c, const float* Wih, const float* Whh,
                                      const float* bsum, const float* bsum2, float* gates, float* h_out, float* c_out, int R, int H,
                                      int ldh, void* stream) {
    return lstm_gate_fwd_impl(q, h, c, Wih, Whh, bsum, bsum2, gates, h_out, c_out, R, H, ldh, nullptr, stream);
}

extern "C" int64_t mmdfn_lstm_gate_planes_workspace(int H) { return (H < 8 || (H & 3)) ? -1 : mmdfn_lstm_gate_planes_floats(H); }
extern "C" int mmdfn_lstm_gate_cut_weights(const float* Wih, const float* Whh, float* planes, int H, void* stream) {
    return mmdfn_launch_lstm_gate_cut(Wih, Whh, planes, H, (hipStream_t)stream);
}
extern "C" int mmdfn_lstm_gate_fwd_pre(const float* q, const float* h, const float* c, const float* Wih, const float* Whh,
                                       const float* bsum, const float* bsum2, float* gates, float* h_out, float* c_out, int R,
                                       int H, int ldh, const float* planes, void* stream) {
    return lstm_gate_fwd_impl(q, h, c, Wih, Whh, bsum, bsum2, gates, h_out, c_out, R, H, ldh, planes, stream);
}
extern "C" int mmdfn_lstm_gate_takes_planes(int R, int H) { return (!bad_dims(R, H) && gate_split(R, H)) ? 1 : 0; }

static int lstm_gate_fwd_impl(const float* q, const float* h, const float* c, const float* Wih, const float* Whh,
                              const float* bsum, const float* bsum2, float* gates, float* h_out, float* c_out, int R, int H,
                              int ldh, const void* planes, void* stream) {
    if (bad_dims(R, H) || (h == nullptr) != (c == nullptr) || ldh < H || (ldh & 3)) return -1;
    if (gate_split(R, H)) {
        const int rc = mmdfn_launch_lstm_gate_fwd_split(q, h, c, Wih, Whh, bsum, bsum2, gates, h_out, c_out, R, H,
                                                        ldh, planes, (hipStream_t)stream);
        if (rc != -2) return rc;
    }
    const int ncb = (H + UB - 1) / UB;
    if (gate_ws(R)) {
        const size_t ldsw = ((size_t)(4 * UB + 2 * RB) * lds_stride(h ? 2 * H : H) + 2 * 4 * RB * (UB + 4)) * sizeof(float);
        if (ldsw > 156 * 1024) return -1;
        if (int e_ = mmdfn_allow_big_lds(lstm_gate_fwd_ws_kernel)) return e_;
        hipLaunchKernelGGL(lstm_gate_fwd_ws_kernel, dim3(row_groups(R, ncb), ncb), dim3(512), ldsw, (hipStream_t)stream, q, h, c, Wih,
                           Whh, bsum, bsum2, gates, h_out, c_out, R, H, ldh);
        MMDFN_CHECK_LAUNCH();
        return 0;
    }
    const size_t lds = ((size_t)(4 * UB + 2 * RB) * lds_stride(h ? 2 * H : H) + 4 * RB * (UB + 4)) * sizeof(float);
    LAUNCH_BIG_LDS(lstm_gate_fwd_kernel, dim3(row_groups(R, ncb), ncb), lds, stream, q, h, c, Wih, Whh, bsum, bsum2, gates,
                   h_out, c_out, R, H, ldh);
    return 0;
}

extern "C" int mmdfn_lstm_gate_fwd(const float* q, const float* h, const float* c, const float* Wih, const float* Whh,
                                   const float* bsum, const float* bsum2, float* gates, float* h_out, float* c_out, int R, int H,
                                   void* stream) {
    return mmdfn_lstm_gate_fwd_ld(q, h, c, Wih, Whh, bsum, bsum2, gates, h_out, c_out, R, H, H, stream);
}

extern "C" int mmdfn_lstm_gate_bwd(const float* gates, const float* c_prev, const float* c_new, const float* dh_a,
                                   const float* dh_b, const float* dc_next, const float* Wih, const float* Whh,
                                   const float* dres, float* dG, float* dc_prev, float* dq, float* dh_prev, int R, int H,
                                   int has_h, int lddres, void* stream) {
    if (bad_dims(R, H) || (has_h && (dc_prev == nullptr || dh_prev == nullptr || c_prev == nullptr))) return -1;
    if (dres != nullptr && (lddres < H || (lddres & 3))) return -1;
    const int nb = (H + CBW - 1) / CBW;
    const int ncb = has_h ? 2 * nb : nb;
    if (gate_ws(R)) {
        const size_t ldsw = (size_t)(CBW + 2 * RB) * lds_stride(4 * H) * sizeof(float);
        if (ldsw > 156 * 1024) return -1;
#ifdef MMDFN_TUNING
#define GBWS_ABL(A_)                                                                                                         \
    case A_:                                                                                                                 \
        if (int e_ = mmdfn_allow_big_lds(lstm_gate_bwd_ws_kernel<A_>)) return e_;                                            \
        hipLaunchKernelGGL(lstm_gate_bwd_ws_kernel<A_>, dim3(row_groups(R, ncb), ncb), dim3(512), ldsw, (hipStream_t)stream, \
                           gates, c_prev, c_new, dh_a, dh_b, dc_next, Wih, Whh, dres, dG, dc_prev, dq, dh_prev, R, H, has_h, \
                           lddres);                                                                                          \
        MMDFN_CHECK_LAUNCH();                                                                                                \
        return 0;
        if (const char* e = getenv("MMDFN_GATE_ABL")) {
            switch (atoi(e)) {
                GBWS_ABL(1) GBWS_ABL(2) GBWS_ABL(4) GBWS_ABL(8) GBWS_ABL(3) GBWS_ABL(6) GBWS_ABL(7) GBWS_ABL(15) GBWS_ABL(12) GBWS_ABL(14)
                default: break;
            }
        }
#undef GBWS_ABL
#endif
        bool wide = H > CBW && 4 * H <= 16 * GATE_BWD_WIDE_NKC && R >= GATE_BWD_WIDE_ROWS;
#ifdef MMDFN_TUNING
        if (const char* e = getenv("MMDFN_GATE_BWD_WIDE")) wide = H > CBW && 4 * H <= 16 * GATE_BWD_WIDE_NKC && atoi(e) != 0;
#endif
        if (wide) {
            const int ncw = has_h ? 2 : 1;
            if (int e_ = mmdfn_allow_big_lds(lstm_gate_bwd_ws_kernel<0, true>)) return e_;
            hipLaunchKernelGGL((lstm_gate_bwd_ws_kernel<0, true>), dim3(row_groups(R, ncw), ncw), dim3(512), ldsw, (hipStream_t)stream,
                               gates, c_prev, c_new, dh_a, dh_b, dc_next, Wih, Whh, dres, dG, dc_prev, dq, dh_prev, R, H, has_h, lddres);
            MMDFN_CHECK_LAUNCH();
            return 0;
        }
        if (int e_ = mmdfn_allow_big_lds(lstm_gate_bwd_ws_kernel<0>)) return e_;
        hipLaunchKernelGGL(lstm_gate_bwd_ws_kernel<0>, dim3(row_groups(R, ncb), ncb), dim3(512), ldsw, (hipStream_t)stream, gates,
                           c_prev, c_new, dh_a, dh_b, dc_next, Wih, Whh, dres, dG, dc_prev, dq, dh_prev, R, H, has_h, lddres);
        MMDFN_CHECK_LAUNCH();
        return 0;
    }
    const size_t lds = (size_t)(CBW + 2 * RB) * lds_stride(4 * H) * sizeof(float);
    LAUNCH_BIG_LDS(lstm_gate_bwd_kernel, dim3(row_groups(R, ncb), ncb), lds, stream, gates, c_prev, c_new, dh_a, dh_b, dc_next,
                   Wih, Whh, dres, dG, dc_prev, dq, dh_prev, R, H, has_h, lddres);
    return 0;
}

extern "C" int mmdfn_gcnii_layer_fwd(const float* hi, const float* h0, const float* W, const float* q, const float* m,
                                     float* out, float* gmask, float theta, float alpha, int R, int H, int ldo, float mscale,
                                     void* stream) {
    if (bad_dims(R, H) || ldo < H || (ldo & 3)) return -1;
    if (layer_ws(R)) {
        const size_t ldsw = ((size_t)(H + 2 * RB) * lds_stride(2 * H) + 2 * RB * (((H + 15) & ~15) + 4)) * sizeof(float);
        if (ldsw > 156 * 1024) return -1;
        if (int e_ = mmdfn_allow_big_lds(gcnii_layer_fwd_ws_kernel)) return e_;
        hipLaunchKernelGGL(gcnii_layer_fwd_ws_kernel, dim3(row_groups(R, 1)), dim3(512), ldsw, (hipStream_t)stream, hi, h0, W, q, m,
                           out, gmask, theta, alpha, R, H, ldo, mscale);
        MMDFN_CHECK_LAUNCH();
        return 0;
    }
    const size_t lds = ((size_t)(H + 2 * RB) * lds_stride(2 * H) + RB * (((H + 15) & ~15) + 4)) * sizeof(float);
    LAUNCH_BIG_LDS(gcnii_layer_fwd_kernel, dim3(row_groups(R, 1)), lds, stream, hi, h0, W, q, m, out, gmask, theta, alpha, R, H,
                   ldo, mscale);
    return 0;
}

extern "C" int mmdfn_gcnii_layer_bwd_ld(const float* dout, const float* gmask, const float* W, float* dP, float* dhi, float* dh0,
                                        float theta, float alpha, int R, int H, int lddo, int acc_h0, int lddhi, void* stream) {
    if (bad_dims(R, H) || lddo < H || (lddo & 3) || lddhi < H || (lddhi & 3) || !(theta > 0.f)) return -1;
    if (layer_ws(R)) {
        const size_t ldsw = ((size_t)(2 * H + 2 * RB) * lds_stride(H) + 2 * RB * (((2 * H + 15) & ~15) + 4)) * sizeof(float);
        if (ldsw > 156 * 1024) return -1;
        if (int e_ = mmdfn_allow_big_lds(gcnii_layer_bwd_ws_kernel)) return e_;
        hipLaunchKernelGGL(gcnii_layer_bwd_ws_kernel, dim3(row_groups(R, 1)), dim3(512), ldsw, (hipStream_t)stream, dout, gmask, W,
                           dP, dhi, dh0, theta, alpha, R, H, lddo, acc_h0, lddhi);
        MMDFN_CHECK_LAUNCH();
        return 0;
    }
    const size_t lds = ((size_t)(2 * H + 2 * RB) * lds_stride(H) + RB * (((2 * H + 15) & ~15) + 4)) * sizeof(float);
    LAUNCH_BIG_LDS(gcnii_layer_bwd_kernel, dim3(row_groups(R, 1)), lds, stream, dout, gmask, W, dP, dhi, dh0, theta, alpha, R, H,
                   lddo, acc_h0, lddhi);
    return 0;
}

extern "C" int mmdfn_gcnii_layer_bwd(const float* dout, const float* gmask, const float* W, float* dP, float* dhi, float* dh0,
                                     float theta, float alpha, int R, int H, int lddo, int acc_h0, void* stream) {
    return mmdfn_gcnii_layer_bwd_ld(dout, gmask, W, dP, dhi, dh0, theta, alpha, R, H, lddo, acc_h0, H, stream);
}
```

### mm_dfn_amd/csrc/propagate.hip

```cpp
#include "mmdfn_internal.h"
#include "../../include/mmdfn_hip.h"
#include <stdlib.h>

namespace {

constexpr int BK = 32;

template <int NW, int NCT, bool TRANS>
__global__ __launch_bounds__(64 * NW) void propagate_kernel(
    const float* __restrict__ tiles, const float* __restrict__ cross, const float* __restrict__ H,
    float* __restrict__ out, const int32_t* __restrict__ dia_len, const int32_t* __restrict__ row_start,
    const int64_t* __restrict__ tile_base, int M, int N, int d, int ldh, int ldo, int max_rb) {
    constexpr int BM = 16 * NW;
    constexpr int CB = 16 * NCT;
    constexpr int LDH = CB + 2;
    constexpr int LDT = BM + 2;
    __shared__ float Hs[BK * LDH];
    __shared__ float Ts[TRANS ? BK * LDT : 1];

    const int i = blockIdx.x / max_rb;
    const int rb = blockIdx.x % max_rb;
    const int m = blockIdx.y;
    const int c0 = blockIdx.z * CB;
    const int L = dia_len[i];
    const int r0 = rb * BM;
    if (r0 >= L) return;
    const int ld = (L + 3) & ~3;
    const int rs = row_start[i];
    const float* T = tiles + tile_base[i] + (int64_t)m * L * ld;
    const float* Hm = H + ((int64_t)m * N + rs) * ldh;

    const int tid = threadIdx.x;
    const int lane = tid & 63;
    const int w = tid >> 6;
    const int frow = lane & 15;
    const int g = lane >> 4;
    const int arow = r0 + 16 * w + frow;

    f32x4 acc[NCT];
#pragma unroll
    for (int ct = 0; ct < NCT; ++ct) acc[ct] = (f32x4){0.f, 0.f, 0.f, 0.f};

    for (int k0 = 0; k0 < L; k0 += BK) {
        __syncthreads();
        for (int idx = tid; idx < BK * (CB / 4); idx += 64 * NW) {
            const int kk = idx / (CB / 4);
            const int c4 = idx - kk * (CB / 4);
            const int k = k0 + kk;
            const int c = c0 + 4 * c4;
            float4 v = make_float4(0.f, 0.f, 0.f, 0.f);
            if (k < L && c < d) v = *reinterpret_cast<const float4*>(Hm + (int64_t)k * ldh + c);
            float2* dst = reinterpret_cast<float2*>(&Hs[kk * LDH + 4 * c4]);
            dst[0] = make_float2(v.x, v.y);
            dst[1] = make_float2(v.z, v.w);
        }
        float a[8];
        if (TRANS) {
            for (int idx = tid; idx < BK * BM; idx += 64 * NW) {
                const int kk = idx / BM;
                const int qq = idx - kk * BM;
                const int k = k0 + kk;
                const int q = r0 + qq;
                Ts[kk * LDT + qq] = (k < L && q < L) ? T[(int64_t)k * ld + q] : 0.f;
            }
        } else {
            const int kbase = k0 + 8 * g;
            float4 v0 = make_float4(0.f, 0.f, 0.f, 0.f), v1 = v0;
            if (arow < L) {
                const float* p = T + (int64_t)arow * ld + kbase;
                if (kbase < ld) v0 = *reinterpret_cast<const float4*>(p);
                if (kbase + 4 < ld) v1 = *reinterpret_cast<const float4*>(p + 4);
            }
            a[0] = v0.x; a[1] = v0.y; a[2] = v0.z; a[3] = v0.w;
            a[4] = v1.x; a[5] = v1.y; a[6] = v1.z; a[7] = v1.w;
#pragma unroll
            for (int j = 0; j < 8; ++j) a[j] = (kbase + j < L) ? a[j] : 0.f;
        }
        __syncthreads();
#pragma unroll
        for (int j = 0; j < 8; ++j) {
            const int kk = 8 * g + j;
            const float av = TRANS ? Ts[kk * LDT + 16 * w + frow] : a[j];
#pragma unroll
            for (int ct = 0; ct < NCT; ++ct) {
                const float bv = Hs[kk * LDH + ct * 16 + frow];
                acc[ct] = __builtin_amdgcn_mfma_f32_16x16x4f32(av, bv, acc[ct], 0, 0, 0);
            }
        }
    }

#pragma unroll
    for (int r = 0; r < 4; ++r) {
        const int row = r0 + 16 * w + 4 * g + r;
        if (row >= L) continue;
        const int64_t grow = rs + row;
        float cw[8];
        int cn[8];
        int nc = 0;
        for (int n = 0; n < M && nc < 8; ++n) {
            if (n == m) continue;
            const int pk = (m < n) ? mmdfn_pair_index(m, n, M) : mmdfn_pair_index(n, m, M);
            cw[nc] = cross[(int64_t)pk * N + grow];
            cn[nc] = n;
            ++nc;
        }
#pragma unroll
        for (int ct = 0; ct < NCT; ++ct) {
            const int col = c0 + ct * 16 + frow;
            if (col >= d) continue;
            float v = acc[ct][r];
            for (int e = 0; e < nc; ++e) v += cw[e] * H[((int64_t)cn[e] * N + grow) * ldh + col];
            out[((int64_t)m * N + grow) * ldo + col] = v;
        }
    }
}


template <int NWR, int NWC, int NCTW, int BKT, int RPW>
__global__ __launch_bounds__(64 * NWR * NWC, (RPW >= 4 ? 2 : 4)) void propagate_v2_kernel(
    const float* __restrict__ tiles, const float* __restrict__ cross, const float* __restrict__ H,
    float* __restrict__ out, const int32_t* __restrict__ dia_len, const int32_t* __restrict__ row_start,
    const int64_t* __restrict__ tile_base, int B, int M, int N, int d, int ldh, int ldo, int max_rb, int ncb, int abl_arg) {
#ifndef MMDFN_TUNING
    constexpr int abl = 0;
    (void)abl_arg;
#else
    const int abl = abl_arg;
#endif
    constexpr int NT = 64 * NWR * NWC;
    constexpr int WROWS = 16 * RPW;
    constexpr int BM = WROWS * NWR;
    constexpr int CB = 16 * NCTW * NWC;
    constexpr int LDH = CB + 4;
    constexpr int NSUB = BKT / 16;
    constexpr int OROWS = (2 * BKT < BM) ? 2 * BKT : BM;
    constexpr int NH4 = (BKT * (CB / 4) + NT - 1) / NT;
    constexpr int HROWS = (NH4 * NT + CB / 4 - 1) / (CB / 4);
    constexpr int HBUF = HROWS * LDH;
    __shared__ __attribute__((aligned(16))) float lds[2 * HBUF];

    const int Rt = max_rb * ncb;
    const int Rd = M * Rt;
    const int bid = blockIdx.x;
    const int yq = bid >> 3;
    const int i = (yq / Rd) * 8 + (bid & 7);
    if (i >= B) return;
    const int rho = yq % Rd;
    const int m = rho / Rt;
    const int rb = (rho - m * Rt) / ncb;
    const int c0 = (rho - m * Rt - rb * ncb) * CB;
    const int L = dia_len[i];
    const int r0 = rb * BM;
    if (r0 >= L) return;
    const int ld = (L + 3) & ~3;
    const int rs = row_start[i];
    const float* T = tiles + tile_base[i] + (int64_t)m * L * ld;
    const float* Hm = H + ((int64_t)m * N + rs) * ldh;

    const int tid = threadIdx.x;
    const int lane = tid & 63;
    const int w = tid >> 6;
    const int wr = w % NWR;
    const int wc = w / NWR;
    const int frow = lane & 15;
    const int g = lane >> 4;
    const int wrow0 = r0 + WROWS * wr;
    const bool wave_active = (c0 + 16 * wc * NCTW < d) && (wrow0 < L);

    f32x4 acc[RPW][NCTW];
#pragma unroll
    for (int rp = 0; rp < RPW; ++rp)
#pragma unroll
        for (int ct = 0; ct < NCTW; ++ct) acc[rp][ct] = (f32x4){0.f, 0.f, 0.f, 0.f};

    int s_kk[NH4], s_lds[NH4];
    bool s_cok[NH4];
    const float* s_ptr[NH4];
#pragma unroll
    for (int e = 0; e < NH4; ++e) {
        const int idx = tid + e * NT;
        const int kk = idx / (CB / 4);
        const int c4 = idx - kk * (CB / 4);
        const int c = c0 + 4 * c4;
        s_kk[e] = kk;
        s_lds[e] = kk * LDH + 4 * c4;
        s_cok[e] = (c < d) && !(abl & 4);
        s_ptr[e] = Hm + (c < d ? c : 0);
    }
    const float* a_ptr[RPW];
    bool a_ok[RPW];
#pragma unroll
    for (int rp = 0; rp < RPW; ++rp) {
        const int arow = wrow0 + 16 * rp + frow;
        a_ok[rp] = (arow < L) && !(abl & 8);
        a_ptr[rp] = T + (int64_t)(arow < L ? arow : L - 1) * ld;
    }
    float4 hset[2][NH4] = {};
    float4 aset[2][RPW][NSUB] = {};
    const int nchunks = (L + BKT - 1) / BKT;

#define MMDFN_ISSUE(SET, K0)                                                                              \
    do {                                                                                                  \
        if (!(abl & 4)) {                                                                                 \
            _Pragma("unroll") for (int e = 0; e < NH4; ++e) {                                             \
                const int k_ = (K0) + s_kk[e];                                                            \
                hset[SET][e] = *reinterpret_cast<const float4*>(s_ptr[e] + (int64_t)(k_ < L ? k_ : L - 1) * ldh); \
            }                                                                                             \
        }                                                                                                 \
        if (!(abl & 8)) {                                                                                 \
            _Pragma("unroll") for (int rp = 0; rp < RPW; ++rp)                                            \
                _Pragma("unroll") for (int h = 0; h < NSUB; ++h) {                                        \
                    const int ka_ = (K0) + 16 * h + 4 * g;                                                \
                    aset[SET][rp][h] = *reinterpret_cast<const float4*>(a_ptr[rp] + (ka_ < ld ? ka_ : ld - 4)); \
                }                                                                                         \
        }                                                                                                 \
    } while (0)

#define MMDFN_CHUNK(SET, C)                                                                               \
    do {                                                                                                  \
        float* Hs = lds + ((C) & 1) * HBUF;                                                               \
        const int kc0 = (C) * BKT;                                                                        \
        _Pragma("unroll") for (int e = 0; e < NH4; ++e) {                                                 \
            const bool ok = s_cok[e] && (kc0 + s_kk[e] < L);                                              \
            const float4 v = hset[SET][e];                                                                \
            *reinterpret_cast<float4*>(&Hs[s_lds[e]]) =                                                   \
                make_float4(ok ? v.x : 0.f, ok ? v.y : 0.f, ok ? v.z : 0.f, ok ? v.w : 0.f);              \
        }                                                                                                 \
        float av[RPW][4 * NSUB];                                                                          \
        _Pragma("unroll") for (int rp = 0; rp < RPW; ++rp)                                                \
            _Pragma("unroll") for (int h = 0; h < NSUB; ++h) {                                            \
                      \
                const int ka_ = kc0 + 16 * h + 4 * g;                                                     \
                const float4 v = aset[SET][rp][h];                                                        \
                av[rp][4 * h + 0] = (a_ok[rp] && ka_ + 0 < L) ? v.x : 0.f;                                \
                av[rp][4 * h + 1] = (a_ok[rp] && ka_ + 1 < L) ? v.y : 0.f;                                \
                av[rp][4 * h + 2] = (a_ok[rp] && ka_ + 2 < L) ? v.z : 0.f;                                \
                av[rp][4 * h + 3] = (a_ok[rp] && ka_ + 3 < L) ? v.w : 0.f;                                \
            }                                                                                             \
        __syncthreads();                                                                                  \
        if ((C) + 2 < nchunks) MMDFN_ISSUE(SET, ((C) + 2) * BKT);                                         \
        if (wave_active && !(abl & 2)) {                                                                  \
            __builtin_amdgcn_s_setprio(3);        \
            const float* hbase = &Hs[16 * wc * NCTW + frow];                                              \
            float bq[2][NCTW];                                                                            \
            _Pragma("unroll") for (int ct = 0; ct < NCTW; ++ct) bq[0][ct] = hbase[(4 * g) * LDH + 16 * ct]; \
            _Pragma("unroll") for (int j = 0; j < 4 * NSUB; ++j) {                                        \
                if (j + 1 < 4 * NSUB) {                                                                   \
                    const int kn = 16 * ((j + 1) >> 2) + 4 * g + ((j + 1) & 3);                           \
                    _Pragma("unroll") for (int ct = 0; ct < NCTW; ++ct)                                   \
                        bq[(j + 1) & 1][ct] = hbase[kn * LDH + 16 * ct];                                  \
                }                                                                                         \
                __builtin_amdgcn_sched_barrier(0);            \
                _Pragma("unroll") for (int rp = 0; rp < RPW; ++rp)                                        \
                    _Pragma("unroll") for (int ct = 0; ct < NCTW; ++ct)                                   \
                        acc[rp][ct] = __builtin_amdgcn_mfma_f32_16x16x4f32(av[rp][j], bq[j & 1][ct],      \
                                                                           acc[rp][ct], 0, 0, 0);         \
                __builtin_amdgcn_sched_barrier(0);                                                        \
            }                                                                                             \
        }                                                                                                 \
        __builtin_amdgcn_s_setprio(0);                                                                    \
        __builtin_amdgcn_sched_barrier(0);                                                                \
    } while (0)

    MMDFN_ISSUE(0, 0);
    if (nchunks > 1) MMDFN_ISSUE(1, BKT);
    for (int c = 0; c < nchunks; c += 2) {
        MMDFN_CHUNK(0, c);
        if (c + 1 < nchunks) MMDFN_CHUNK(1, c + 1);
    }
#undef MMDFN_ISSUE
#undef MMDFN_CHUNK

    float* Os = lds;
    const int cw4 = ((d - c0 < CB) ? (d - c0) : CB) / 4;
#pragma unroll
    for (int pass = 0; pass < BM / OROWS; ++pass) {
        __syncthreads();
#pragma unroll
        for (int rp = 0; rp < RPW; ++rp) {
            const int lrow0 = WROWS * wr + 16 * rp;
            if (lrow0 >= pass * OROWS && lrow0 < (pass + 1) * OROWS) {
#pragma unroll
                for (int ct = 0; ct < NCTW; ++ct)
#pragma unroll
                    for (int r = 0; r < 4; ++r)
                        Os[(lrow0 - pass * OROWS + 4 * g + r) * LDH + 16 * (wc * NCTW + ct) + frow] = acc[rp][ct][r];
            }
        }
        __syncthreads();
        for (int idx = tid; idx < OROWS * cw4; idx += NT) {
            const int rr = idx / cw4;
            const int c4 = idx - rr * cw4;
            const int row = r0 + pass * OROWS + rr;
            if (row >= L) continue;
            const int64_t grow = rs + row;
            float4 v = *reinterpret_cast<const float4*>(&Os[rr * LDH + 4 * c4]);
            const int nq = (abl & 1) ? 0 : M - 1;
#pragma unroll 5
            for (int q = 0; q < nq; ++q) {
                const int n = q + (q >= m ? 1 : 0);
                const int pk = (m < n) ? mmdfn_pair_index(m, n, M) : mmdfn_pair_index(n, m, M);
                const float cwt = cross[(int64_t)pk * N + grow];
                const float4 h = *reinterpret_cast<const float4*>(H + ((int64_t)n * N + grow) * ldh + c0 + 4 * c4);
                v.x = fmaf(cwt, h.x, v.x);
                v.y = fmaf(cwt, h.y, v.y);
                v.z = fmaf(cwt, h.z, v.z);
                v.w = fmaf(cwt, h.w, v.w);
            }
            *reinterpret_cast<float4*>(out + ((int64_t)m * N + grow) * ldo + c0 + 4 * c4) = v;
        }
    }
}

#ifdef MMDFN_TUNING
int ablation() {
    const char* e = getenv("MMDFN_PROP_ABL");
    return e ? atoi(e) : 0;
}
#else
constexpr int ablation() { return 0; }
#endif

template <int NWR, int NWC, int NCTW, int BKT, int RPW>
int launch_v2(const float* tiles, const float* cross, const float* H, float* out, const int32_t* dia_len,
              const int32_t* row_start, const int64_t* tile_base, int B, int M, int N, int d, int ldh, int ldo,
              int max_len, hipStream_t s) {
    const int BM = 16 * NWR * RPW;
    const int CB = 16 * NCTW * NWC;
    const int max_rb = (max_len + BM - 1) / BM;
    const int ncb = (d + CB - 1) / CB;
    dim3 grid(((B + 7) / 8) * 8 * M * max_rb * ncb);
    dim3 block(64 * NWR * NWC);
    hipLaunchKernelGGL((propagate_v2_kernel<NWR, NWC, NCTW, BKT, RPW>), grid, block, 0, s, tiles, cross, H, out, dia_len,
                       row_start, tile_base, B, M, N, d, ldh, ldo, max_rb, ncb, ablation());
    MMDFN_CHECK_LAUNCH();
    return 0;
}

#ifdef MMDFN_TUNING
int tuning_override() {
    const char* e = getenv("MMDFN_PROP_CFG");
    return e ? atoi(e) : -1;
}
#else
constexpr int tuning_override() { return -1; }
#endif

template <int NW, int NCT>
int launch(const float* tiles, const float* cross, const float* H, float* out, const int32_t* dia_len,
           const int32_t* row_start, const int64_t* tile_base, int B, int M, int N, int d, int ldh, int ldo,
           int max_len, int transpose, hipStream_t s) {
    const int BM = 16 * NW;
    const int max_rb = (max_len + BM - 1) / BM;
    dim3 grid(B * max_rb, M, (d + 16 * NCT - 1) / (16 * NCT));
    dim3 block(64 * NW);
    if (transpose)
        hipLaunchKernelGGL((propagate_kernel<NW, NCT, true>), grid, block, 0, s, tiles, cross, H, out, dia_len,
                           row_start, tile_base, M, N, d, ldh, ldo, max_rb);
    else
        hipLaunchKernelGGL((propagate_kernel<NW, NCT, false>), grid, block, 0, s, tiles, cross, H, out, dia_len,
                           row_start, tile_base, M, N, d, ldh, ldo, max_rb);
    MMDFN_CHECK_LAUNCH();
    return 0;
}

}

#define V2(NWR, NWC, NCTW, BKT, RPW) \
    launch_v2<NWR, NWC, NCTW, BKT, RPW>(tiles, cross, H, out, dia_len, row_start, tile_base, B, M, N, d, ldh, ldo, max_len, s)

int mmdfn_launch_propagate(const float* tiles, const float* cross, const float* H, float* out,
                           const int32_t* dia_len, const int32_t* row_start, const int64_t* tile_base,
                           int B, int M, int N, int d, int ldh, int ldo, int max_len, int transpose, hipStream_t s) {
    if (B <= 0 || M <= 0 || M > 9 || N <= 0 || d <= 0 || (d & 3) || max_len <= 0) return -1;
    if (ldh < d || ldo < d || (ldh & 3) || (ldo & 3)) return -1;
    if (transpose) {
        const bool small_rows = max_len <= 48;
        if (d <= 112)
            return small_rows ? launch<2, 7>(tiles, cross, H, out, dia_len, row_start, tile_base, B, M, N, d, ldh, ldo, max_len, 1, s)
                              : launch<4, 7>(tiles, cross, H, out, dia_len, row_start, tile_base, B, M, N, d, ldh, ldo, max_len, 1, s);
        if (d <= 208)
            return small_rows ? launch<2, 13>(tiles, cross, H, out, dia_len, row_start, tile_base, B, M, N, d, ldh, ldo, max_len, 1, s)
                              : launch<4, 13>(tiles, cross, H, out, dia_len, row_start, tile_base, B, M, N, d, ldh, ldo, max_len, 1, s);
        return small_rows ? launch<2, 8>(tiles, cross, H, out, dia_len, row_start, tile_base, B, M, N, d, ldh, ldo, max_len, 1, s)
                          : launch<4, 8>(tiles, cross, H, out, dia_len, row_start, tile_base, B, M, N, d, ldh, ldo, max_len, 1, s);
    }
    const int ov = tuning_override();
    if (ov >= 0) {
        switch (ov) {
            case 0: return V2(4, 1, 7, 16, 1);
            case 1: return V2(8, 1, 7, 16, 1);
            case 2: return V2(2, 4, 2, 16, 1);
            case 3: return V2(2, 4, 2, 32, 1);
            case 4: return V2(2, 2, 4, 16, 1);
            case 5: return V2(4, 2, 4, 16, 1);
            case 6: return V2(4, 1, 7, 16, 2);
            case 7: return V2(4, 2, 7, 16, 1);
            case 8: {
                const int rc = mmdfn_launch_propagate_split(tiles, cross, H, out, dia_len, row_start, tile_base, B, M, N, d,
                                                            ldh, ldo, max_len, s);
                if (rc != -2) return rc;
                break;
            }
            default: break;
        }
    }
    if (ov == 9) {
        if (d <= 112) return ((long)B * M * max_len <= 32768L) ? V2(2, 4, 2, 16, 1) : V2(8, 1, 7, 16, 1);
        if (d <= 224) return V2(4, 2, 7, 16, 1);
        return V2(4, 2, 4, 16, 1);
    }
    const long approx_rows = (long)B * M * max_len;
    const long split_wgs = (long)B * M * ((max_len + 127) / 128) * ((d + 127) / 128);
    if (max_len >= 128 && split_wgs >= 48) {
        const int rc = mmdfn_launch_propagate_split(tiles, cross, H, out, dia_len, row_start, tile_base, B, M, N, d, ldh,
                                                    ldo, max_len, s);
        if (rc != -2) return rc;
    }
    if (d <= 112) {
        if (approx_rows <= 32768L) return V2(2, 4, 2, 16, 1);
        return V2(8, 1, 7, 16, 1);
    }
    if (d <= 224) return V2(4, 2, 7, 16, 1);
    return V2(4, 2, 4, 16, 1);
}
#undef V2

extern "C" int mmdfn_abi_version(void) { return 21; }

extern "C" int mmdfn_propagate(const float* tiles, const float* cross, const float* H, float* out,
                               const int32_t* dia_len, const int32_t* row_start, const int64_t* tile_base,
                               int B, int M, int N, int d, int ldh, int ldo, int max_len, int transpose,
                               void* stream) {
    return mmdfn_launch_propagate(tiles, cross, H, out, dia_len, row_start, tile_base, B, M, N, d, ldh, ldo, max_len,
                                  transpose, (hipStream_t)stream);
}
```

### mm_dfn_amd/gcn_stack.py

```python
import math

PRECUT = __import__("os").environ.get("MMDFN_GATE_PRECUT", "1") == "1"
FUSE_PROP_LAYER = __import__("os").environ.get("MMDFN_FUSE_PROP_LAYER", "1") == "1"

import torch

from . import _hip, ops
from .ops_pad import _lay_args

ROW_LIMIT = 131072
TAP = None


def eligible(x, nfeat, nhidden, nlayers, params, lamda=1.0):
    return (x.is_cuda and x.dtype == torch.float32 and x.shape[0] <= ROW_LIMIT and nlayers >= 1 and lamda > 0
            and nhidden % 4 == 0 and 4 <= nhidden <= 100 and nfeat % 4 == 0 and 4 <= nfeat <= 256
            and (not torch.is_grad_enabled() or all(ops._leaf(p) for p in params)))


class _GcnStack(torch.autograd.Function):
    @staticmethod
    def forward(ctx, x, tiles, cross, masks, mscale, lay, symmetric, lamda, alpha, reason, use_residue, W0, b0, w_ih, w_hh,
                b_ih, b_hh, *convW):
        lib = _hip.lib()
        P, st = _hip.ptr, _hip.stream()
        x = x.contiguous()
        R, F = x.shape
        H = W0.shape[0]
        nl = len(convW)
        dev = x.device
        new = lambda *shape: torch.empty(*shape, dtype=torch.float32, device=dev)
        mx = m0 = None
        ml = [None] * nl
        if masks is not None:
            mx = masks[:R * F].view(R, F)
            m0 = masks[R * F:R * (F + H)].view(R, H)
            ml = [masks[R * (F + H) + i * R * H: R * (F + H) + (i + 1) * R * H].view(R, H) for i in range(nl)]
        out = new(R, F + H) if use_residue else new(R, H)
        xd = out if use_residue else new(R, F)
        ldxd = F + H if use_residue else F
        h0, cur = new(R, H), new(R, H)
        _hip.check(lib.mmdfn_gcn_input_fwd(P(x), P(mx), P(W0), P(b0), P(m0), P(xd), P(h0), P(cur), R, F, H, ldxd, mscale, st),
                   "mmdfn_gcn_input_fwd")
        h = c = None
        layers = []
        zin_all = new(R, nl * H) if reason else None
        planes = None
        if PRECUT and reason and nl > 1 and lib.mmdfn_lstm_gate_takes_planes(R, H):
            planes = new(int(lib.mmdfn_lstm_gate_planes_workspace(H)))
            _hip.check(lib.mmdfn_lstm_gate_cut_weights(P(w_ih), P(w_hh), P(planes), H, st), "mmdfn_lstm_gate_cut_weights")
        for i in range(nl):
            q = cur
            rec = dict(q=q, h_prev=h, c_prev=c)
            if reason:
                gates, h_new, c_new = new(R, 4 * H), zin_all[:, i * H:(i + 1) * H], new(R, H)
                _hip.check(lib.mmdfn_lstm_gate_fwd_pre(P(q), P(h), P(c), P(w_ih), P(w_hh), P(b_ih), P(b_hh), P(gates), P(h_new),
                                                       P(c_new), R, H, nl * H, P(planes), st), "mmdfn_lstm_gate_fwd_pre")
                rec.update(gates=gates, c_new=c_new)
                h, c = h_new, c_new
                zin = h_new
            else:
                zin = q
            last = i == nl - 1
            if last and use_residue:
                dst, ldo = out[:, F:], F + H
            elif last:
                dst, ldo = out, H
            else:
                dst, ldo = new(R, H), H
            gmask = new(R, H)
            theta = math.log(lamda / (i + 1) + 1)
            hi = new(R, H)
            rc = lib.mmdfn_prop_layer_fwd(P(tiles), P(cross), P(zin), zin.stride(0), *_lay_args(lay), lay.B, lay.M, lay.N,
                                          lay.max_len, P(h0), P(convW[i]), P(q if reason else None), P(ml[i]), P(hi), P(dst),
                                          P(gmask), theta, alpha, H, ldo, mscale, st) if FUSE_PROP_LAYER else -2
            if rc == -2:
                hi = ops.propagate_raw(tiles, cross, zin, lay, out=hi)
                _hip.check(lib.mmdfn_gcnii_layer_fwd(P(hi), P(h0), P(convW[i]), P(q if reason else None), P(ml[i]), P(dst),
                                                     P(gmask), theta, alpha, R, H, ldo, mscale, st), "mmdfn_gcnii_layer_fwd")
            else:
                _hip.check(rc, "mmdfn_prop_layer_fwd")
            rec.update(zin=zin, hi=hi, gmask=gmask, theta=theta)
            layers.append(rec)
            cur = dst
        if TAP is not None:
            TAP.append(dict(h0=h0, gmask=[rec["gmask"] for rec in layers], out=out.detach()))
        ctx.layers = layers
        ctx.misc = dict(lay=lay, symmetric=symmetric, alpha=alpha, reason=reason, use_residue=use_residue, R=R, F=F, H=H,
                        mx=mx, m0=m0, xd=xd.detach(), h0=h0, tiles=tiles, cross=cross, mscale=mscale, zin_all=zin_all)
        ctx.params = (W0, b0, w_ih, w_hh, b_ih, b_hh, convW)
        return out

    @staticmethod
    def backward(ctx, dout):
        lib = _hip.lib()
        P, st = _hip.ptr, _hip.stream()
        m = ctx.misc
        R, F, H = m["R"], m["F"], m["H"]
        W0, b0, w_ih, w_hh, b_ih, b_hh, convW = ctx.params
        lay, tiles, cross = m["lay"], m["tiles"], m["cross"]
        dev = dout.device
        new = lambda *shape: torch.empty(*shape, dtype=torch.float32, device=dev)
        dout = dout.contiguous()
        if m["use_residue"]:
            dcur, lddo, dxd, lddxd = dout[:, F:], F + H, dout, F + H
        else:
            dcur, lddo, dxd, lddxd = dout, H, None, 0
        want_adj = ctx.needs_input_grad[1] or ctx.needs_input_grad[2]
        plist = [p for p in (W0, b0, w_ih, w_hh, b_ih, b_hh) if p is not None] + list(convW)
        batched = ops.wgrad_batching() and not any(ops._hooked(p) for p in plist)
        inline = {}

        def wgrad(A, B, weight, biases=(), rows=None):
            if batched:
                ops.queue_wgrad(A, B, weight, biases, rows=rows)
                return
            dw, db = ops._wgrad_inline(A, B, bool(biases))
            if rows is not None:
                g = inline.get(id(weight))
                if g is None:
                    g = inline[id(weight)] = torch.zeros_like(weight)
                g[rows[0]:rows[1]] += dw
            else:
                inline[id(weight)] = dw if id(weight) not in inline else inline[id(weight)] + dw
            for b in biases:
                inline[id(b)] = db if id(b) not in inline else inline[id(b)] + db

        dh0 = new(R, H)
        acc_h0 = 0
        dtiles = dcross = None
        dh_carry = dc_carry = None
        nl = len(ctx.layers)
        one_outer = want_adj and m["zin_all"] is not None
        dhi_all = new(R, nl * H) if one_outer else None
        for i in reversed(range(nl)):
            L = ctx.layers[i]
            dP = new(R, H)
            dhi = dhi_all[:, i * H:(i + 1) * H] if one_outer else new(R, H)
            _hip.check(lib.mmdfn_gcnii_layer_bwd_ld(P(dcur), P(L["gmask"]), P(convW[i]), P(dP), P(dhi), P(dh0), L["theta"],
                                                    m["alpha"], R, H, lddo, acc_h0, dhi.stride(0), st), "mmdfn_gcnii_layer_bwd_ld")
            acc_h0 = 1
            wgrad(L["hi"], dP, convW[i], rows=(0, H))
            wgrad(m["h0"], dP, convW[i], rows=(H, 2 * H))
            dz = ops.propagate_raw(tiles, cross, dhi, lay, transpose=not m["symmetric"])
            if want_adj and not one_outer:
                dtiles, dcross = ops.tile_outer_raw(dhi, L["zin"], lay, dtiles, dcross)
            if m["reason"]:
                has_h = L["h_prev"] is not None
                dG, dq = new(R, 4 * H), new(R, H)
                dh_prev = new(R, H) if has_h else None
                dc_prev = new(R, H) if has_h else None
                _hip.check(lib.mmdfn_lstm_gate_bwd(P(L["gates"]), P(L["c_prev"]), P(L["c_new"]), P(dz), P(dh_carry),
                                                   P(dc_carry), P(w_ih), P(w_hh), P(dcur), P(dG), P(dc_prev), P(dq),
                                                   P(dh_prev), R, H, 1 if has_h else 0, lddo, st), "mmdfn_lstm_gate_bwd")
                wgrad(dG, L["q"], w_ih, [b_ih, b_hh])
                if has_h:
                    wgrad(dG, L["h_prev"], w_hh)
                dcur, lddo = dq, H
                dh_carry, dc_carry = dh_prev, dc_prev
            else:
                dcur, lddo = dz, H
        if one_outer:
            dtiles, dcross = ops.tile_outer_raw(dhi_all, m["zin_all"], lay)
        dpre, dx = new(R, H), new(R, F)
        _hip.check(lib.mmdfn_gcn_input_bwd(P(dcur), P(m["m0"]), P(dh0), P(m["h0"]), P(W0), P(dxd), P(m["mx"]), P(dpre), P(dx), R,
                                           F, H, lddxd, m["mscale"], st), "mmdfn_gcn_input_bwd")
        xd = m["xd"][:, :F] if m["use_residue"] else m["xd"]
        wgrad(dpre, xd, W0, [b0] if b0 is not None else [])
        pg = [None if p is None else inline.get(id(p)) for p in (W0, b0, w_ih, w_hh, b_ih, b_hh)]
        return (dx, dtiles, dcross) + (None,) * 8 + tuple(pg) + tuple(inline.get(id(w)) for w in convW)


def gcn_stack(x, adj, masks, mscale, lamda, alpha, reason_flag, use_residue, W0, b0, lstm, convs):
    w_ih = w_hh = b_ih = b_hh = None
    if reason_flag:
        w_ih, w_hh, b_ih, b_hh = lstm.weight_ih_l0, lstm.weight_hh_l0, lstm.bias_ih_l0, lstm.bias_hh_l0
    return _GcnStack.apply(x, adj.tiles, adj.cross, masks, float(mscale), adj.layout, adj.symmetric, float(lamda), float(alpha),
                           bool(reason_flag), bool(use_residue), W0, b0, w_ih, w_hh, b_ih, b_hh, *convs)
```

Baseline: 2.180 million utterances/s.

## Fuse LSTM gate computation into GCN input and propagation layer kernels

Adds a shared gate_tail device helper that computes the LSTM gate GEMM (via MFMA) plus the cell pointwise update at the end of the GCN input kernel and of the fused propagation-layer kernel, using rows already resident in LDS. The Python stack then skips the separate lstm_gate_fwd_pre launch whenever the row count is too small for the pre-cut weight-plane path. This removes one kernel launch and one round trip of q/h through global memory per layer, at the cost of extra LDS, registers and tail work in the fused kernels, which may reduce their occupancy.

```diff
diff --git a/include/mmdfn_hip.h b/include/mmdfn_hip.h
--- a/include/mmdfn_hip.h
+++ b/include/mmdfn_hip.h
@@ -185,6 +185,16 @@
                          const int32_t* row_start, const int64_t* tile_base, int B, int M, int N, int max_len,
                          const float* h0, const float* W, const float* q, const float* m, float* hi, float* out,
                          float* gmask, float theta, float alpha, int H, int ldo, float mscale, void* stream);
+int mmdfn_gcn_input_gate_fwd(const float* x, const float* mx, const float* W0, const float* b0, const float* m0, float* xd,
+                             float* h0, float* cur0, int R, int F, int H, int ldxd, float mscale, const float* Wih,
+                             const float* bsum, const float* bsum2, float* gates, float* h_out, float* c_out, int ldh,
+                             void* stream);
+int mmdfn_prop_layer_gate_fwd(const float* tiles, const float* cross, const float* zin, int ldz, const int32_t* dia_len,
+                              const int32_t* row_start, const int64_t* tile_base, int B, int M, int N, int max_len,
+                              const float* h0, const float* W, const float* q, const float* m, float* hi, float* out,
+                              float* gmask, float theta, float alpha, int H, int ldo, float mscale, const float* h,
+                              const float* c, const float* Wih, const float* Whh, const float* bsum, const float* bsum2,
+                              float* gates, float* h_out, float* c_out, int ldh, void* stream);
 int mmdfn_gcnii_layer_bwd(const float* dout, const float* gmask, const float* W, float* dP, float* dhi, float* dh0,
                           float theta, float alpha, int R, int H, int lddo, int acc_h0, void* stream);
 int mmdfn_gcnii_layer_bwd_ld(const float* dout, const float* gmask, const float* W, float* dP, float* dhi, float* dh0,
diff --git a/mm_dfn_amd/_hip.py b/mm_dfn_amd/_hip.py
--- a/mm_dfn_amd/_hip.py
+++ b/mm_dfn_amd/_hip.py
@@ -37,6 +37,9 @@
     "mmdfn_lstm_gate_bwd": [_P] * 13 + [_I] * 4 + [_P],
     "mmdfn_gcnii_layer_fwd": [_P] * 7 + [_F, _F, _I, _I, _I, _F, _P],
     "mmdfn_prop_layer_fwd": [_P, _P, _P, _I, _P, _P, _P, _I, _I, _I, _I, _P, _P, _P, _P, _P, _P, _P, _F, _F, _I, _I, _F, _P],
+    "mmdfn_gcn_input_gate_fwd": [_P, _P, _P, _P, _P, _P, _P, _P, _I, _I, _I, _I, _F, _P, _P, _P, _P, _P, _P, _I, _P],
+    "mmdfn_prop_layer_gate_fwd": [_P, _P, _P, _I, _P, _P, _P, _I, _I, _I, _I, _P, _P, _P, _P, _P, _P, _P, _F, _F, _I, _I, _F,
+                                  _P, _P, _P, _P, _P, _P, _P, _P, _P, _I, _P],
     "mmdfn_gcnii_layer_bwd": [_P] * 6 + [_F, _F, _I, _I, _I, _I, _P],
     "mmdfn_gcnii_layer_bwd_ld": [_P] * 6 + [_F, _F, _I, _I, _I, _I, _I, _P],
     "mmdfn_linear": [_P, _P, _P, _P, _I, _I, _I, _I, _I, _I, _I, _P],
@@ -111,7 +114,7 @@
     "mmdfn_colsum": [_P, _L, _I, _I, _P, _P, _P],
 }
 
-ABI_VERSION = 21
+ABI_VERSION = 22
 
 
 class HipLibraryError(RuntimeError):
diff --git a/mm_dfn_amd/csrc/gate_tail.h b/mm_dfn_amd/csrc/gate_tail.h
--- /dev/null
+++ b/mm_dfn_amd/csrc/gate_tail.h
@@ -0,0 +1,156 @@
+#pragma once
+#include "mmdfn_internal.h"
+
+namespace gate_tail {
+
+constexpr int GT_ROWS = 32;
+constexpr int GT_RING = 3;
+
+__device__ __forceinline__ float sigm(float x) { return __builtin_amdgcn_rcpf(1.0f + __expf(-x)); }
+__device__ __forceinline__ float tanhf_(float x) { return 1.0f - 2.0f * __builtin_amdgcn_rcpf(1.0f + __expf(2.0f * x)); }
+__device__ __forceinline__ int frag_unit(int g) { return ((g & 1) << 1) | (g >> 1); }
+
+__device__ __forceinline__ void cell(float pi, float pf, float pg, float po, float cp, float& gi, float& gf, float& gg, float& go,
+                                     float& cn, float& hn) {
+    gi = sigm(pi); gf = sigm(pf); gg = tanhf_(pg); go = sigm(po);
+    cn = __builtin_fmaf(gf, cp, gi * gg);
+    hn = go * tanhf_(cn);
+}
+
+struct Args {
+    const float* h;
+    const float* c;
+    const float* Wih;
+    const float* Whh;
+    const float* bsum;
+    const float* bsum2;
+    float* gates;
+    float* h_out;
+    float* c_out;
+    int ldh;
+};
+
+__host__ __device__ inline int lds_stride(int K) {
+    int ld = ((K + 15) & ~15) + 4;
+    if (((ld >> 2) & 1) == 0) ld += 4;
+    return ld;
+}
+
+struct Wave {
+    float4 f[GT_RING][4];
+    float cp[2][4];
+    float b[4];
+    const float* wl;
+    const float* wh;
+    int H, K, nk, u;
+    bool active;
+
+    __device__ __forceinline__ void request(int kc, int slot) {
+        const int g = (threadIdx.x & 63) >> 4;
+        int k = 16 * kc + 4 * frag_unit(g);
+        k = k < K ? k : K - 4;
+        const float* p = k < H ? wl + k : wh + (k - H);
+        const unsigned gs = (unsigned)H * (unsigned)H;
+#pragma unroll
+        for (int t = 0; t < 4; ++t) f[slot][t] = *reinterpret_cast<const float4*>(p + t * gs);
+    }
+
+    __device__ __forceinline__ void request_first(const Args& ga, int H_, int w, int nct, int64_t row0, int nrows) {
+        const int lane = threadIdx.x & 63, fi = lane & 15, g = lane >> 4;
+        H = H_;
+        K = ga.h ? 2 * H : H;
+        nk = (K + 15) >> 4;
+        active = w < nct;
+        u = 16 * w + fi;
+        const unsigned uc = u < H ? u : H - 1;
+#pragma unroll
+        for (int a = 0; a < 2; ++a)
+#pragma unroll
+            for (int r = 0; r < 4; ++r) cp[a][r] = 0.f;
+#pragma unroll
+        for (int t = 0; t < 4; ++t) b[t] = 0.f;
+        if (!active) return;
+        wl = ga.Wih + uc * (unsigned)H;
+        wh = (ga.h ? ga.Whh : ga.Wih) + uc * (unsigned)H;
+        if (ga.c) {
+            const float* cb = ga.c + row0 * H;
+#pragma unroll
+            for (int a = 0; a < 2; ++a)
+#pragma unroll
+                for (int r = 0; r < 4; ++r) {
+                    const int pl = 16 * a + 4 * g + r;
+                    cp[a][r] = cb[(unsigned)(pl < nrows ? pl : nrows - 1) * (unsigned)H + uc];
+                }
+        }
+#pragma unroll
+        for (int t = 0; t < 4; ++t) {
+            b[t] = ga.bsum[t * H + uc];
+            if (ga.bsum2) b[t] += ga.bsum2[t * H + uc];
+        }
+        request(0, 0);
+        request(nk > 1 ? 1 : 0, 1);
+    }
+
+    __device__ __forceinline__ void run(const Args& ga, const float* A3, int S3, int64_t row0, int nrows) {
+        if (!active) return;
+        const int lane = threadIdx.x & 63, fi = lane & 15, g = lane >> 4;
+        f32x4 acc[4][2];
+#pragma unroll
+        for (int t = 0; t < 4; ++t) acc[t][0] = acc[t][1] = (f32x4){0.f, 0.f, 0.f, 0.f};
+        const float* e0 = A3 + fi * S3 + 4 * frag_unit(g);
+        const float* e1 = e0 + 16 * S3;
+        auto mma = [&](int kc, const float4(&fr)[4]) {
+            const float4 a0 = *reinterpret_cast<const float4*>(e0 + 16 * kc);
+            const float4 a1 = *reinterpret_cast<const float4*>(e1 + 16 * kc);
+#pragma unroll
+            for (int j = 0; j < 4; ++j)
+#pragma unroll
+                for (int t = 0; t < 4; ++t) {
+                    const float x0 = j == 0 ? a0.x : j == 1 ? a0.y : j == 2 ? a0.z : a0.w;
+                    const float x1 = j == 0 ? a1.x : j == 1 ? a1.y : j == 2 ? a1.z : a1.w;
+                    const float bw = j == 0 ? fr[t].x : j == 1 ? fr[t].y : j == 2 ? fr[t].z : fr[t].w;
+                    acc[t][0] = __builtin_amdgcn_mfma_f32_16x16x4f32(x0, bw, acc[t][0], 0, 0, 0);
+                    acc[t][1] = __builtin_amdgcn_mfma_f32_16x16x4f32(x1, bw, acc[t][1], 0, 0, 0);
+                }
+        };
+        const int last = nk - 1;
+        int kc = 0;
+#pragma unroll 1
+        for (; kc + GT_RING <= nk; kc += GT_RING) {
+            request(kc + 2 < last ? kc + 2 : last, 2);
+            __builtin_amdgcn_sched_barrier(0);
+            mma(kc, f[0]);
+            __builtin_amdgcn_sched_barrier(0);
+            request(kc + 3 < last ? kc + 3 : last, 0);
+            __builtin_amdgcn_sched_barrier(0);
+            mma(kc + 1, f[1]);
+            __builtin_amdgcn_sched_barrier(0);
+            request(kc + 4 < last ? kc + 4 : last, 1);
+            __builtin_amdgcn_sched_barrier(0);
+            mma(kc + 2, f[2]);
+            __builtin_amdgcn_sched_barrier(0);
+        }
+        if (kc < nk) mma(kc, f[0]);
+        if (kc + 1 < nk) mma(kc + 1, f[1]);
+        if (u >= H) return;
+        const unsigned lane_g = (unsigned)(4 * g) * (unsigned)(4 * H) + u, lane_c = (unsigned)(4 * g) * (unsigned)H + u;
+        const unsigned lane_h = (unsigned)(4 * g) * (unsigned)ga.ldh + u;
+#pragma unroll
+        for (int a = 0; a < 2; ++a)
+#pragma unroll
+            for (int r = 0; r < 4; ++r) {
+                if (16 * a + 4 * g + r >= nrows) continue;
+                float gi, gf, gg, go, cn, hn;
+                cell(acc[0][a][r] + b[0], acc[1][a][r] + b[1], acc[2][a][r] + b[2], acc[3][a][r] + b[3], cp[a][r], gi, gf, gg, go, cn, hn);
+                float* gr = ga.gates + (row0 + 16 * a + r) * (4 * H) + lane_g;
+                __builtin_nontemporal_store(gi, gr);
+                __builtin_nontemporal_store(gf, gr + H);
+                __builtin_nontemporal_store(gg, gr + 2 * H);
+                __builtin_nontemporal_store(go, gr + 3 * H);
+                (ga.c_out + (row0 + 16 * a + r) * H)[lane_c] = cn;
+                (ga.h_out + (row0 + 16 * a + r) * ga.ldh)[lane_h] = hn;
+            }
+    }
+};
+
+}
diff --git a/mm_dfn_amd/csrc/gcn_small.hip b/mm_dfn_amd/csrc/gcn_small.hip
--- a/mm_dfn_amd/csrc/gcn_small.hip
+++ b/mm_dfn_amd/csrc/gcn_small.hip
@@ -1,5 +1,6 @@
 #include "mmdfn_internal.h"
 #include "../../include/mmdfn_hip.h"
+#include "gate_tail.h"
 #include <stdlib.h>
 
 namespace {
@@ -15,12 +16,13 @@
 #define GS_STOP(K) do { } while (0)
 #endif
 
+template <bool GATE>
 __global__ __launch_bounds__(64 * GS_NW) void prop_layer_strip_fwd_kernel(
     const float* __restrict__ tiles, const float* __restrict__ cross, const float* __restrict__ zin, int ldz,
     const int32_t* __restrict__ dia_len, const int32_t* __restrict__ row_start, const int64_t* __restrict__ tile_base,
     int B, int M, int N, int NS, const float* __restrict__ h0, const float* __restrict__ W, const float* __restrict__ q,
     const float* __restrict__ mk, float* __restrict__ hi_out, float* __restrict__ out, float* __restrict__ gmask,
-    float theta, float alpha, int H, int ldo, float ms, int S2, int stop) {
+    float theta, float alpha, int H, int ldo, float ms, int S2, int stop, gate_tail::Args ga) {
     extern __shared__ __attribute__((aligned(16))) float smem[];
     const int bid = blockIdx.x;
     const int yq = bid >> 3;
@@ -77,6 +79,17 @@
         hr[s2] = make_float4(0.f, 0.f, 0.f, 0.f);
         if (r < GS_SR && p < L) hr[s2] = *reinterpret_cast<const float4*>(h0 + ((int64_t)m * N + rs + p) * H + k);
     }
+    float4 hg[2];
+    if (GATE) {
+#pragma unroll
+        for (int s2 = 0; s2 < 2; ++s2) {
+            const int e = tid + 64 * GS_NW * s2;
+            const int r = e / H4, k = (e - r * H4) * 4;
+            const int p = r0 + r;
+            hg[s2] = make_float4(0.f, 0.f, 0.f, 0.f);
+            if (r < GS_SR && p < L) hg[s2] = *reinterpret_cast<const float4*>(ga.h + ((int64_t)m * N + rs + p) * ga.ldh + k);
+        }
+    }
     float cwv = 0.f;
     if (tid < 2 * GS_SR) {
         const int n = tid >> 5, pl = tid & 31;
@@ -234,6 +247,8 @@
     __syncthreads();
     GS_STOP(2);
 
+    gate_tail::Wave gt;
+    float qn[2][4];
     if (tile) {
         f32x4 acc0 = (f32x4){0.f, 0.f, 0.f, 0.f}, acc1 = acc0;
         const float* e0 = A2 + fi * S2 + 4 * g;
@@ -252,6 +267,11 @@
             acc0 = __builtin_amdgcn_mfma_f32_16x16x4f32(a0.w, wfr[4 * kc + 3], acc0, 0, 0, 0);
             acc1 = __builtin_amdgcn_mfma_f32_16x16x4f32(a1.w, wfr[4 * kc + 3], acc1, 0, 0, 0);
         }
+        if (GATE) gt.request_first(ga, H, w, nct, row0, L - r0 < GS_SR ? L - r0 : GS_SR);
+#pragma unroll
+        for (int a = 0; a < 2; ++a)
+#pragma unroll
+            for (int r = 0; r < 4; ++r) qn[a][r] = 0.f;
         if (col < H) {
             const unsigned lane_o = (unsigned)(4 * g) * (unsigned)ldo + col;
 #pragma unroll
@@ -263,19 +283,45 @@
                     const float pv = a == 0 ? acc0[r] : acc1[r];
                     const float v0 = A2[pl * S2 + H + col];
                     const float pre = theta * pv + (1.0f - theta) * ((1.0f - alpha) * hv[a][r] + alpha * v0);
-                    (out + (row0 + 16 * a + r) * ldo)[lane_o] = fmaxf(pre, 0.f) * mv[a][r] + qv[a][r];
+                    const float ov = fmaxf(pre, 0.f) * mv[a][r] + qv[a][r];
+                    (out + (row0 + 16 * a + r) * ldo)[lane_o] = ov;
+                    qn[a][r] = ov;
                     (gmask + (row0 + 16 * a + r) * H)[lane_h] = pre > 0.f ? mv[a][r] : 0.f;
                 }
         }
     }
-}
-
-}
-
-extern "C" int mmdfn_prop_layer_fwd(const float* tiles, const float* cross, const float* zin, int ldz, const int32_t* dia_len,
-                                    const int32_t* row_start, const int64_t* tile_base, int B, int M, int N, int max_len,
-                                    const float* h0, const float* W, const float* q, const float* m, float* hi, float* out,
-                                    float* gmask, float theta, float alpha, int H, int ldo, float mscale, void* stream) {
+    if (!GATE) return;
+    GS_STOP(3);
+    __syncthreads();
+    const int S3 = gate_tail::lds_stride(K2);
+    float* A3 = smem;
+    if (tile && col < H) {
+#pragma unroll
+        for (int a = 0; a < 2; ++a)
+#pragma unroll
+            for (int r = 0; r < 4; ++r) A3[(16 * a + 4 * g + r) * S3 + col] = qn[a][r];
+    }
+#pragma unroll
+    for (int s2 = 0; s2 < 2; ++s2) {
+        const int e = tid + 64 * GS_NW * s2;
+        const int r = e / H4, k = (e - r * H4) * 4;
+        if (r < GS_SR) *reinterpret_cast<float4*>(A3 + r * S3 + H + k) = hg[s2];
+    }
+    for (int e = tid; e < GS_SR * (S3 - K2); e += 64 * GS_NW) {
+        const int r = e / (S3 - K2), k = K2 + (e - r * (S3 - K2));
+        A3[r * S3 + k] = 0.f;
+    }
+    __syncthreads();
+    if (tile) gt.run(ga, A3, S3, row0, L - r0 < GS_SR ? L - r0 : GS_SR);
+}
+
+}
+
+static int prop_layer_launch(const float* tiles, const float* cross, const float* zin, int ldz, const int32_t* dia_len,
+                             const int32_t* row_start, const int64_t* tile_base, int B, int M, int N, int max_len,
+                             const float* h0, const float* W, const float* q, const float* m, float* hi, float* out,
+                             float* gmask, float theta, float alpha, int H, int ldo, float mscale, const gate_tail::Args* gate,
+                             void* stream) {
     if (B <= 0 || M <= 0 || N <= 0 || H <= 0 || max_len <= 0 || !tiles || !zin || !h0 || !W || !hi || !out || !gmask) return -1;
     if (M > 3 || max_len > GS_MAXL || H > 100 || (H & 3) || ldz < H || ldo < H) return -2;
     if (M > 1 && !cross) return -1;
@@ -289,9 +335,34 @@
     if (grid > 4096) return -2;
     const int S2 = ((2 * H + 15) & ~15) + 4;
     const size_t lds = ((size_t)GS_SR * GS_SA + (size_t)GS_SR * S2 + 2 * GS_SR) * sizeof(float);
-    hipLaunchKernelGGL(prop_layer_strip_fwd_kernel, dim3((unsigned)grid), dim3(64 * GS_NW), lds, (hipStream_t)stream, tiles, cross,
-                       zin, ldz, dia_len, row_start, tile_base, B, M, N, NS, h0, W, q, m, hi, out, gmask, theta, alpha, H, ldo,
-                       mscale, S2, stop);
+    if (gate)
+        hipLaunchKernelGGL(prop_layer_strip_fwd_kernel<true>, dim3((unsigned)grid), dim3(64 * GS_NW), lds, (hipStream_t)stream, tiles,
+                           cross, zin, ldz, dia_len, row_start, tile_base, B, M, N, NS, h0, W, q, m, hi, out, gmask, theta, alpha, H,
+                           ldo, mscale, S2, stop, *gate);
+    else
+        hipLaunchKernelGGL(prop_layer_strip_fwd_kernel<false>, dim3((unsigned)grid), dim3(64 * GS_NW), lds, (hipStream_t)stream, tiles,
+                           cross, zin, ldz, dia_len, row_start, tile_base, B, M, N, NS, h0, W, q, m, hi, out, gmask, theta, alpha, H,
+                           ldo, mscale, S2, stop, gate_tail::Args{});
     MMDFN_CHECK_LAUNCH();
     return 0;
 }
+
+extern "C" int mmdfn_prop_layer_fwd(const float* tiles, const float* cross, const float* zin, int ldz, const int32_t* dia_len,
+                                    const int32_t* row_start, const int64_t* tile_base, int B, int M, int N, int max_len,
+                                    const float* h0, const float* W, const float* q, const float* m, float* hi, float* out,
+                                    float* gmask, float theta, float alpha, int H, int ldo, float mscale, void* stream) {
+    return prop_layer_launch(tiles, cross, zin, ldz, dia_len, row_start, tile_base, B, M, N, max_len, h0, W, q, m, hi, out, gmask,
+                             theta, alpha, H, ldo, mscale, nullptr, stream);
+}
+
+extern "C" int mmdfn_prop_layer_gate_fwd(const float* tiles, const float* cross, const float* zin, int ldz, const int32_t* dia_len,
+                                         const int32_t* row_start, const int64_t* tile_base, int B, int M, int N, int max_len,
+                                         const float* h0, const float* W, const float* q, const float* m, float* hi, float* out,
+                                         float* gmask, float theta, float alpha, int H, int ldo, float mscale, const float* h,
+                                         const float* c, const float* Wih, const float* Whh, const float* bsum,
+                                         const float* bsum2, float* gates, float* h_out, float* c_out, int ldh, void* stream) {
+    if (!h || !c || !Wih || !Whh || !bsum || !gates || !h_out || !c_out || ldh < H || (ldh & 3)) return -1;
+    const gate_tail::Args ga = {h, c, Wih, Whh, bsum, bsum2, gates, h_out, c_out, ldh};
+    return prop_layer_launch(tiles, cross, zin, ldz, dia_len, row_start, tile_base, B, M, N, max_len, h0, W, q, m, hi, out, gmask,
+                             theta, alpha, H, ldo, mscale, &ga, stream);
+}
diff --git a/mm_dfn_amd/csrc/gcn_stack.hip b/mm_dfn_amd/csrc/gcn_stack.hip
--- a/mm_dfn_amd/csrc/gcn_stack.hip
+++ b/mm_dfn_amd/csrc/gcn_stack.hip
@@ -1,5 +1,6 @@
 #include "mmdfn_internal.h"
 #include "../../include/mmdfn_hip.h"
+#include "gate_tail.h"
 #include <stdlib.h>
 
 namespace {
@@ -14,20 +15,15 @@
 __device__ __forceinline__ float4 scl4(float4 a, float s) { return make_float4(a.x * s, a.y * s, a.z * s, a.w * s); }
 __device__ __forceinline__ float4 add4(float4 a, float4 b) { return make_float4(a.x + b.x, a.y + b.y, a.z + b.z, a.w + b.w); }
 __device__ __forceinline__ float4 fma4(float4 a, float s, float4 b) { return make_float4(a.x * s + b.x, a.y * s + b.y, a.z * s + b.z, a.w * s + b.w); }
-__device__ __forceinline__ float sigm(float x) { return __builtin_amdgcn_rcpf(1.0f + __expf(-x)); }
-__device__ __forceinline__ float tanhf_(float x) { return 1.0f - 2.0f * __builtin_amdgcn_rcpf(1.0f + __expf(2.0f * x)); }
+using gate_tail::sigm;
+using gate_tail::tanhf_;
+using gate_tail::frag_unit;
+using gate_tail::lds_stride;
 
 typedef float f32x2_t __attribute__((ext_vector_type(2)));
 __device__ __forceinline__ void st4_nt(float* p, float4 v) { __builtin_nontemporal_store((f32x4){v.x, v.y, v.z, v.w}, reinterpret_cast<f32x4*>(p)); }
 __device__ __forceinline__ void nt_store2(float* p, float2 v) { __builtin_nontemporal_store((f32x2_t){v.x, v.y}, reinterpret_cast<f32x2_t*>(p)); }
 __device__ __forceinline__ int frag_row(int i) { return i < 4 ? 2 * i : (i < 12 ? 2 * (i - 4) + 1 : 2 * (i - 12) + 8); }
-__device__ __forceinline__ int frag_unit(int g) { return ((g & 1) << 1) | (g >> 1); }
-
-__host__ __device__ inline int lds_stride(int K) {
-    int ld = ((K + 15) & ~15) + 4;
-    if (((ld >> 2) & 1) == 0) ld += 4;
-    return ld;
-}
 
 __device__ __forceinline__ int qdiv(int i, float inv) { return (int)(((float)i + 0.5f) * inv); }
 
@@ -227,6 +223,131 @@
     }
 }
 
+constexpr int IG_SR = gate_tail::GT_ROWS;
+constexpr int IG_NW = 8;
+constexpr int IG_MAXKC = 16;
+__global__ __launch_bounds__(64 * IG_NW) void gcn_input_gate_fwd_kernel(const float* __restrict__ x, const float* __restrict__ mx,
+                                                                        const float* __restrict__ W0, const float* __restrict__ b0,
+                                                                        const float* __restrict__ m0, float* __restrict__ xd,
+                                                                        float* __restrict__ h0, float* __restrict__ cur0, int R,
+                                                                        int F, int H, int ldxd, float ms, gate_tail::Args ga) {
+    extern __shared__ __attribute__((aligned(16))) float smem[];
+    const int lda = lds_stride(F);
+    float* sA = smem;
+    const int64_t row0 = (int64_t)blockIdx.x * IG_SR;
+    const int nrows = R - row0 < IG_SR ? (int)(R - row0) : IG_SR;
+    const int tid = threadIdx.x, lane = tid & 63, fi = lane & 15, g = lane >> 4;
+    const int w = __builtin_amdgcn_readfirstlane(tid >> 6);
+    const int nct = (H + 15) >> 4;
+    const bool tile = w < nct;
+    const int u = 16 * w + fi;
+    const unsigned uc = u < H ? u : H - 1;
+    const int F4 = F >> 2, nkF = (F + 15) >> 4;
+    const float rF4 = 1.0f / (float)F4;
+    constexpr int NS = 4;
+    float4 rx[NS], rm[NS];
+#pragma unroll
+    for (int s = 0; s < NS; ++s) {
+        const int e = tid + 64 * IG_NW * s;
+        const int r = qdiv(e, rF4), k = (e - r * F4) * 4;
+        const bool ok = r < nrows;
+        rx[s] = ok ? ld4(x + (row0 + r) * F + k) : zero4();
+        rm[s] = (ok && mx) ? ld4(mx + (row0 + r) * F + k) : one4();
+    }
+    float4 wfr[IG_MAXKC];
+    float bv = 0.f, mv[2][4];
+#pragma unroll
+    for (int kc = 0; kc < IG_MAXKC; ++kc) wfr[kc] = zero4();
+#pragma unroll
+    for (int a = 0; a < 2; ++a)
+#pragma unroll
+        for (int r = 0; r < 4; ++r) mv[a][r] = 1.0f;
+    if (tile) {
+        const float* wl = W0 + uc * (unsigned)F;
+#pragma unroll
+        for (int kc = 0; kc < IG_MAXKC; ++kc) {
+            if (kc >= nkF) continue;
+            const int k = 16 * kc + 4 * frag_unit(g);
+            wfr[kc] = ld4(wl + (k < F ? k : F - 4));
+        }
+        if (b0) bv = b0[uc];
+        if (m0) {
+            const float* mb = m0 + row0 * H;
+#pragma unroll
+            for (int a = 0; a < 2; ++a)
+#pragma unroll
+                for (int r = 0; r < 4; ++r) {
+                    const int pl = 16 * a + 4 * g + r;
+                    mv[a][r] = mb[(unsigned)(pl < nrows ? pl : nrows - 1) * (unsigned)H + uc];
+                }
+        }
+    }
+    gate_tail::Wave gt;
+    gt.request_first(ga, H, w, nct, row0, nrows);
+#pragma unroll
+    for (int s = 0; s < NS; ++s) {
+        const int e = tid + 64 * IG_NW * s;
+        const int r = qdiv(e, rF4), k = (e - r * F4) * 4;
+        if (r >= IG_SR) continue;
+        const float4 v = mul4(rx[s], scl4(rm[s], mx ? ms : 1.0f));
+        st4(sA + r * lda + k, v);
+        if (r < nrows) st4_nt(xd + (row0 + r) * ldxd + k, v);
+    }
+    {
+        const int np4 = (lda - F) >> 2;
+        const float rnp4 = 1.0f / (float)np4;
+        for (int i = tid; i < IG_SR * np4; i += 64 * IG_NW) { const int r = qdiv(i, rnp4), j = i - r * np4; st4(sA + r * lda + F + 4 * j, zero4()); }
+    }
+    __syncthreads();
+    float qn[2][4];
+    if (tile) {
+        f32x4 acc0 = (f32x4){0.f, 0.f, 0.f, 0.f}, acc1 = acc0;
+        const float* e0 = sA + fi * lda + 4 * frag_unit(g);
+        const float* e1 = e0 + 16 * lda;
+#pragma unroll
+        for (int kc = 0; kc < IG_MAXKC; ++kc) {
+            if (kc >= nkF) continue;
+            const float4 a0 = ld4(e0 + 16 * kc), a1 = ld4(e1 + 16 * kc);
+            acc0 = __builtin_amdgcn_mfma_f32_16x16x4f32(a0.x, wfr[kc].x, acc0, 0, 0, 0);
+            acc1 = __builtin_amdgcn_mfma_f32_16x16x4f32(a1.x, wfr[kc].x, acc1, 0, 0, 0);
+            acc0 = __builtin_amdgcn_mfma_f32_16x16x4f32(a0.y, wfr[kc].y, acc0, 0, 0, 0);
+            acc1 = __builtin_amdgcn_mfma_f32_16x16x4f32(a1.y, wfr[kc].y, acc1, 0, 0, 0);
+            acc0 = __builtin_amdgcn_mfma_f32_16x16x4f32(a0.z, wfr[kc].z, acc0, 0, 0, 0);
+            acc1 = __builtin_amdgcn_mfma_f32_16x16x4f32(a1.z, wfr[kc].z, acc1, 0, 0, 0);
+            acc0 = __builtin_amdgcn_mfma_f32_16x16x4f32(a0.w, wfr[kc].w, acc0, 0, 0, 0);
+            acc1 = __builtin_amdgcn_mfma_f32_16x16x4f32(a1.w, wfr[kc].w, acc1, 0, 0, 0);
+        }
+        const unsigned lane_h = (unsigned)(4 * g) * (unsigned)H + u;
+#pragma unroll
+        for (int a = 0; a < 2; ++a)
+#pragma unroll
+            for (int r = 0; r < 4; ++r) {
+                const float v = fmaxf((a == 0 ? acc0[r] : acc1[r]) + bv, 0.f);
+                const float cv = v * (mv[a][r] * (m0 ? ms : 1.0f));
+                const bool in = 16 * a + 4 * g + r < nrows;
+                qn[a][r] = in ? cv : 0.f;
+                if (in && u < H) {
+                    (h0 + (row0 + 16 * a + r) * H)[lane_h] = v;
+                    (cur0 + (row0 + 16 * a + r) * H)[lane_h] = cv;
+                }
+            }
+    }
+    __syncthreads();
+    const int S3 = gate_tail::lds_stride(H);
+    if (tile && u < H) {
+#pragma unroll
+        for (int a = 0; a < 2; ++a)
+#pragma unroll
+            for (int r = 0; r < 4; ++r) sA[(16 * a + 4 * g + r) * S3 + u] = qn[a][r];
+    }
+    for (int e = tid; e < IG_SR * (S3 - H); e += 64 * IG_NW) {
+        const int r = e / (S3 - H), k = H + (e - r * (S3 - H));
+        sA[r * S3 + k] = 0.f;
+    }
+    __syncthreads();
+    gt.run(ga, sA, S3, row0, nrows);
+}
+
 __global__ __launch_bounds__(256) void gcn_input_bwd_kernel(const float* __restrict__ dcur0, const float* __restrict__ m0,
                                                             const float* __restrict__ dh0, const float* __restrict__ h0,
                                                             const float* __restrict__ W0, const float* __restrict__ dxd,
@@ -793,9 +914,7 @@
             float2 gi, gf, gg, go, cn, hn;
 #define K8F(F_)                                                                 \
     {                                                                           \
-        gi.F_ = sigm(pi.F_ + bi.F_); gf.F_ = sigm(pf.F_ + bf.F_); gg.F_ = tanhf_(pg.F_ + bg.F_); go.F_ = sigm(po.F_ + bo.F_); \
-        cn.F_ = gf.F_ * cp.F_ + gi.F_ * gg.F_;                                  \
-        hn.F_ = go.F_ * tanhf_(cn.F_);                                          \
+        gate_tail::cell(pi.F_ + bi.F_, pf.F_ + bf.F_, pg.F_ + bg.F_, po.F_ + bo.F_, cp.F_, gi.F_, gf.F_, gg.F_, go.F_, cn.F_, hn.F_); \
     }
             K8F(x) K8F(y)
 #undef K8F
@@ -1230,9 +1349,7 @@
         float2 gi, gf, gg, go, cn, hn;
 #define K8F(F_)                                                                 \
     {                                                                           \
-        gi.F_ = sigm(pi.F_ + bi.F_); gf.F_ = sigm(pf.F_ + bf.F_); gg.F_ = tanhf_(pg.F_ + bg.F_); go.F_ = sigm(po.F_ + bo.F_); \
-        cn.F_ = gf.F_ * cp.F_ + gi.F_ * gg.F_;                                  \
-        hn.F_ = go.F_ * tanhf_(cn.F_);                                          \
+        gate_tail::cell(pi.F_ + bi.F_, pf.F_ + bf.F_, pg.F_ + bg.F_, po.F_ + bo.F_, cp.F_, gi.F_, gf.F_, gg.F_, go.F_, cn.F_, hn.F_); \
     }
         K8F(x) K8F(y)
 #undef K8F
@@ -1333,6 +1450,22 @@
     const size_t lds = ((size_t)(H + 2 * RB) * lds_stride(F) + RB * (((H + 15) & ~15) + 4)) * sizeof(float);
     LAUNCH_BIG_LDS(gcn_input_fwd_kernel, dim3(row_groups(R, 1)), lds, stream, x, mx, W0, b0, m0, xd, h0, cur0, R, F, H, ldxd,
                    mscale);
+    return 0;
+}
+
+extern "C" int mmdfn_gcn_input_gate_fwd(const float* x, const float* mx, const float* W0, const float* b0, const float* m0,
+                                        float* xd, float* h0, float* cur0, int R, int F, int H, int ldxd, float mscale,
+                                        const float* Wih, const float* bsum, const float* bsum2, float* gates, float* h_out,
+                                        float* c_out, int ldh, void* stream) {
+    if (bad_dims(R, H) || F < 4 || (F & 3) || F > 256 || ldxd < F || (ldxd & 3) || ldh < H || (ldh & 3)) return -1;
+    if (!x || !W0 || !xd || !h0 || !cur0 || !Wih || !bsum || !gates || !h_out || !c_out) return -1;
+    if (gate_split(R, H)) return -2;
+    const gate_tail::Args ga = {nullptr, nullptr, Wih, nullptr, bsum, bsum2, gates, h_out, c_out, ldh};
+    const int lda = lds_stride(F), S3 = gate_tail::lds_stride(H);
+    const size_t lds = (size_t)IG_SR * (lda > S3 ? lda : S3) * sizeof(float);
+    hipLaunchKernelGGL(gcn_input_gate_fwd_kernel, dim3((unsigned)((R + IG_SR - 1) / IG_SR)), dim3(64 * IG_NW), lds,
+                       (hipStream_t)stream, x, mx, W0, b0, m0, xd, h0, cur0, R, F, H, ldxd, mscale, ga);
+    MMDFN_CHECK_LAUNCH();
     return 0;
 }
 
diff --git a/mm_dfn_amd/csrc/propagate.hip b/mm_dfn_amd/csrc/propagate.hip
--- a/mm_dfn_amd/csrc/propagate.hip
+++ b/mm_dfn_amd/csrc/propagate.hip
@@ -426,7 +426,7 @@
 }
 #undef V2
 
-extern "C" int mmdfn_abi_version(void) { return 21; }
+extern "C" int mmdfn_abi_version(void) { return 22; }
 
 extern "C" int mmdfn_propagate(const float* tiles, const float* cross, const float* H, float* out,
                                const int32_t* dia_len, const int32_t* row_start, const int64_t* tile_base,
diff --git a/mm_dfn_amd/gcn_stack.py b/mm_dfn_amd/gcn_stack.py
--- a/mm_dfn_amd/gcn_stack.py
+++ b/mm_dfn_amd/gcn_stack.py
@@ -2,6 +2,8 @@
 
 PRECUT = __import__("os").environ.get("MMDFN_GATE_PRECUT", "1") == "1"
 FUSE_PROP_LAYER = __import__("os").environ.get("MMDFN_FUSE_PROP_LAYER", "1") == "1"
+FUSE_INPUT_GATE = __import__("os").environ.get("MMDFN_FUSE_INPUT_GATE", "1") == "1"
+FUSE_LAYER_GATE = __import__("os").environ.get("MMDFN_FUSE_LAYER_GATE", "1") == "1"
 
 import torch
 
@@ -40,8 +42,6 @@
         xd = out if use_residue else new(R, F)
         ldxd = F + H if use_residue else F
         h0, cur = new(R, H), new(R, H)
-        _hip.check(lib.mmdfn_gcn_input_fwd(P(x), P(mx), P(W0), P(b0), P(m0), P(xd), P(h0), P(cur), R, F, H, ldxd, mscale, st),
-                   "mmdfn_gcn_input_fwd")
         h = c = None
         layers = []
         zin_all = new(R, nl * H) if reason else None
@@ -49,13 +49,29 @@
         if PRECUT and reason and nl > 1 and lib.mmdfn_lstm_gate_takes_planes(R, H):
             planes = new(int(lib.mmdfn_lstm_gate_planes_workspace(H)))
             _hip.check(lib.mmdfn_lstm_gate_cut_weights(P(w_ih), P(w_hh), P(planes), H, st), "mmdfn_lstm_gate_cut_weights")
+        few_rows = reason and not lib.mmdfn_lstm_gate_takes_planes(R, H)
+        tail_ok = few_rows and FUSE_PROP_LAYER and FUSE_LAYER_GATE
+        bufs, done = None, False
+        if few_rows and FUSE_INPUT_GATE:
+            bufs = new(R, 4 * H), new(R, H)
+            rc = lib.mmdfn_gcn_input_gate_fwd(P(x), P(mx), P(W0), P(b0), P(m0), P(xd), P(h0), P(cur), R, F, H, ldxd, mscale, P(w_ih),
+                                              P(b_ih), P(b_hh), P(bufs[0]), P(zin_all), P(bufs[1]), nl * H, st)
+            if rc != -2:
+                _hip.check(rc, "mmdfn_gcn_input_gate_fwd")
+            done = rc == 0
+        if not done:
+            _hip.check(lib.mmdfn_gcn_input_fwd(P(x), P(mx), P(W0), P(b0), P(m0), P(xd), P(h0), P(cur), R, F, H, ldxd, mscale, st),
+                       "mmdfn_gcn_input_fwd")
         for i in range(nl):
             q = cur
             rec = dict(q=q, h_prev=h, c_prev=c)
             if reason:
-                gates, h_new, c_new = new(R, 4 * H), zin_all[:, i * H:(i + 1) * H], new(R, H)
-                _hip.check(lib.mmdfn_lstm_gate_fwd_pre(P(q), P(h), P(c), P(w_ih), P(w_hh), P(b_ih), P(b_hh), P(gates), P(h_new),
-                                                       P(c_new), R, H, nl * H, P(planes), st), "mmdfn_lstm_gate_fwd_pre")
+                h_new = zin_all[:, i * H:(i + 1) * H]
+                gates, c_new = bufs if bufs is not None else (new(R, 4 * H), new(R, H))
+                if not done:
+                    _hip.check(lib.mmdfn_lstm_gate_fwd_pre(P(q), P(h), P(c), P(w_ih), P(w_hh), P(b_ih), P(b_hh), P(gates), P(h_new),
+                                                           P(c_new), R, H, nl * H, P(planes), st), "mmdfn_lstm_gate_fwd_pre")
+                bufs, done = None, False
                 rec.update(gates=gates, c_new=c_new)
                 h, c = h_new, c_new
                 zin = h_new
@@ -71,9 +87,20 @@
             gmask = new(R, H)
             theta = math.log(lamda / (i + 1) + 1)
             hi = new(R, H)
-            rc = lib.mmdfn_prop_layer_fwd(P(tiles), P(cross), P(zin), zin.stride(0), *_lay_args(lay), lay.B, lay.M, lay.N,
-                                          lay.max_len, P(h0), P(convW[i]), P(q if reason else None), P(ml[i]), P(hi), P(dst),
-                                          P(gmask), theta, alpha, H, ldo, mscale, st) if FUSE_PROP_LAYER else -2
+            rc = -2
+            if tail_ok and not last:
+                bufs = new(R, 4 * H), new(R, H)
+                rc = lib.mmdfn_prop_layer_gate_fwd(P(tiles), P(cross), P(zin), zin.stride(0), *_lay_args(lay), lay.B, lay.M, lay.N,
+                                                   lay.max_len, P(h0), P(convW[i]), P(q), P(ml[i]), P(hi), P(dst), P(gmask), theta,
+                                                   alpha, H, ldo, mscale, P(h), P(c), P(w_ih), P(w_hh), P(b_ih), P(b_hh), P(bufs[0]),
+                                                   P(zin_all[:, (i + 1) * H:(i + 2) * H]), P(bufs[1]), nl * H, st)
+                if rc != -2:
+                    _hip.check(rc, "mmdfn_prop_layer_gate_fwd")
+                done = rc == 0
+            if rc == -2:
+                rc = lib.mmdfn_prop_layer_fwd(P(tiles), P(cross), P(zin), zin.stride(0), *_lay_args(lay), lay.B, lay.M, lay.N,
+                                              lay.max_len, P(h0), P(convW[i]), P(q if reason else None), P(ml[i]), P(hi), P(dst),
+                                              P(gmask), theta, alpha, H, ldo, mscale, st) if FUSE_PROP_LAYER else -2
             if rc == -2:
                 hi = ops.propagate_raw(tiles, cross, zin, lay, out=hi)
                 _hip.check(lib.mmdfn_gcnii_layer_fwd(P(hi), P(h0), P(convW[i]), P(q if reason else None), P(ml[i]), P(dst),
```

New measurement: 2.207 million utterances/s, median of 6. 1.2% higher.
